# NoelShin/PixelPick

Hardware: AMD Instinct MI355X
Metric: train_step_throughput (higher is better)
Workload: dtype f32; 1 GPU; BASELINE configs[1]: Cityscapes 256x512, C=19, DeepLabv3+-MobileNetV2; train step per-GPU batch 4 with 20 labelled px/img + Adam; acquisition entropy top-k=20, B=256 images/launch/GPU, NCHW fp32 logits; global_batch=4

## Files before the change

### include/pixelpick_hip.h

```cpp
#ifndef PIXELPICK_HIP_H
#define PIXELPICK_HIP_H

#include <stddef.h>
#include <stdint.h>

#ifdef __cplusplus
extern "C" {
#endif

typedef void* pp_stream_t;

enum {
    PP_OK = 0,
    PP_ERR_BAD_ARG = -1,
    PP_ERR_BAD_K = -2,
    PP_ERR_WORKSPACE = -3,
    PP_ERR_UNSUPPORTED = -4,
    PP_ERR_LAUNCH = -5
};

enum { PP_ACQ_ENTROPY = 0, PP_ACQ_LEAST_CONFIDENCE = 1, PP_ACQ_MARGIN = 2 };
#define PP_ACQ_REFERENCE_ORDER 0x100

#define PP_ACQ_MAX_CLASSES 64
// ... 154 lines not shown

int64_t pp_conv2d_fwd_stats_rows(int B, int H, int W, int Cin, int Cout, int kh, int kw, int stride, int pad, int dil);
int pp_conv2d_fwd_stats(const float* x, int64_t ldx, int B, int H, int W, int Cin, const float* w, const float* bias,
                        int kh, int kw, int stride, int pad, int dil, float* y, int64_t ldy, int Cout, void* workspace,
                        size_t ws_bytes, float* stats, size_t stats_floats, pp_stream_t stream);
int pp_bn_train_fwd_partials(const float* x, int64_t ldx, int64_t M, int C, const float* stats, int64_t stat_rows, const float* gamma,
                             const float* beta, float eps, float momentum, float* running_mean, float* running_var, float* mean,
                             float* invstd, const float* residual, int64_t ldr, int act, float drop_p, uint64_t drop_seed,
                             const uint64_t* drop_seed_dev, float* y, int64_t ldy, pp_stream_t stream);

int pp_dwconv3x3_bn_train_fwd_fused(const float* in, int64_t ld_in, int B, int H, int W, int C, const float* w, int stride, int pad,
                                    int dil, float* x_out, int64_t ldx, const float* gamma, const float* beta, float eps,
                                    float momentum, float* running_mean, float* running_var, float* mean, float* invstd,
                                    const float* residual, int64_t ldr, int act, float* y, int64_t ldy, void* workspace,
                                    size_t ws_bytes, int32_t* sync, size_t sync_ints, pp_stream_t stream);

int pp_bn_bwd_fused(const float* x, int64_t ldx, const float* dy, int64_t lddy, const float* y_act, int64_t ldya, int act,
                    int64_t M, int C, const float* mean, const float* invstd, const float* gamma, float* dgamma,
                    float* dbeta, float* dx, int64_t lddx, float* dres, int64_t lddr, float grad_scale, const float* beta,
                    void* workspace, size_t ws_bytes, int32_t* sync, size_t sync_ints, pp_stream_t stream);

int pp_row_flags(const float* dy, int64_t lddy, int64_t M, int C, unsigned char* flags, pp_stream_t stream);
size_t pp_conv1x1_bwd_weight_sparse_workspace_bytes(int64_t M, int Cin, int Cout);
int pp_conv1x1_bwd_weight_sparse(const float* x, int64_t ldx, int64_t M, int Cin, const float* dy, int64_t lddy, int Cout,
                                 const unsigned char* row_flags, float* dw, float* dbias, void* workspace, size_t ws_bytes, pp_stream_t stream);
int pp_conv1x1_bwd_data_sparse(const float* dy, int64_t lddy, int64_t M, int Cout, const float* w, int Cin, const unsigned char* row_flags,
                             float* dx, int64_t lddx, pp_stream_t stream);
int pp_bn_bwd_fused_sparse(const float* x, int64_t ldx, const float* dy, int64_t lddy, const float* y_act, int64_t ldya, int act,
                         int64_t M, int C, const float* mean, const float* invstd, const float* gamma, float* dgamma,
                         float* dbeta, float* dx, int64_t lddx, float* dres, int64_t lddr, float grad_scale, const float* beta,
                         void* workspace, size_t ws_bytes, int32_t* sync, size_t sync_ints, const unsigned char* row_flags,
                         pp_stream_t stream);

int pp_bn_eval_affine(int C, const float* gamma, const float* beta, const float* running_mean, const float* running_var,
                      float eps, float* scale, float* shift, pp_stream_t stream);

int pp_scale_shift_act(const float* x, int64_t ldx, int64_t M, int C, const float* scale, const float* shift,
                       const float* residual, int64_t ldr, int act, float* y, int64_t ldy, pp_stream_t stream);

int pp_bn_bwd(const float* x, int64_t ldx, const float* dy, int64_t lddy, const float* y_act, int64_t ldya, int act,
              int64_t M, int C, const float* mean, const float* invstd, const float* gamma, float* dgamma, float* dbeta,
              float* dx, int64_t lddx, float* dres, int64_t lddr, void* workspace, size_t ws_bytes, pp_stream_t stream);

int pp_dwconv3x3_fwd(const float* x, int64_t ldx, int B, int H, int W, int C, const float* w, int stride, int pad, int dil,
                     float* y, int64_t ldy, pp_stream_t stream);

int pp_dwconv3x3_fwd_bn_act(const float* x, int64_t ldx, int B, int H, int W, int C, const float* w, int stride, int pad,
                            int dil, const float* gamma, const float* beta, const float* running_mean,
                            const float* running_var, float eps, const float* residual, int64_t ldr, int act, float* y,
                            int64_t ldy, pp_stream_t stream);
int pp_dwconv3x3_bwd_data(const float* dy, int64_t lddy, int B, int H, int W, int C, const float* w, int stride, int pad,
                          int dil, float* dx, int64_t lddx, pp_stream_t stream);
int pp_dwconv3x3_bwd_weight(const float* x, int64_t ldx, int B, int H, int W, int C, const float* dy, int64_t lddy,
                            int stride, int pad, int dil, float* dw, void* workspace, size_t ws_bytes, pp_stream_t stream);

size_t pp_groupnorm_workspace_bytes(int B, int64_t P, int C);
int pp_groupnorm_relu_fwd(const float* x, int64_t ldx, int B, int64_t P, int C, int G, const float* gamma, const float* beta,
                          float eps, int relu, float* y, int64_t ldy, float* mean, float* rstd, void* workspace,
                          size_t ws_bytes, pp_stream_t stream);
int pp_groupnorm_relu_bwd(const float* x, int64_t ldx, const float* dy, int64_t lddy, const float* y, int64_t ldy, int B,
                          int64_t P, int C, int G, const float* mean, const float* rstd, const float* gamma, float* dgamma,
                          float* dbeta, float* dx, int64_t lddx, void* workspace, size_t ws_bytes, pp_stream_t stream);

int pp_maxpool2d_fwd(const float* x, int64_t ldx, int B, int H, int W, int C, int ksize, int stride, int pad, float* y,
                     int64_t ldy, unsigned char* argmax, pp_stream_t stream);
int pp_maxpool2d_bwd(const float* dy, int64_t lddy, const unsigned char* argmax, int B, int H, int W, int C, int ksize, int stride,
// ... 90 lines not shown
```

### pixelpick_amd/_lib.py

```python
import ctypes
import os
import struct

import torch

_HERE = os.path.dirname(os.path.abspath(__file__))
LIB_PATH = os.path.join(_HERE, "libpixelpick_hip.so")
KNOBS_LIB_PATH = os.path.join(_HERE, "libpixelpick_hip_knobs.so")
_use_knobs = [os.environ.get("PIXELPICK_KNOBS_BUILD", "0") not in ("", "0")]


def use_knobs_build(on: bool = True):
    if _lib is not None and _use_knobs[0] != bool(on):
        raise PixelPickHipError("use_knobs_build() after the library was loaded")
    _use_knobs[0] = bool(on)


def knobs_build() -> bool:
    return _use_knobs[0]

_i64, _p, _int, _sz, _f = ctypes.c_int64, ctypes.c_void_p, ctypes.c_int, ctypes.c_size_t, ctypes.c_float
_u64 = ctypes.c_uint64

SIGNATURES = {
# ... 33 lines not shown
                                      _p, _i64, _int, _p, _i64, _int, _p, _sz, _p, _sz, _p]),
    "pp_conv2d_bwd_data_bn_bwd_ok": (_int, [_int] * 10),
    "pp_conv2d_bwd_data_bn_bwd_xchg_bytes": (_sz, [_int] * 10),
    "pp_conv2d_bwd_data_bn_bwd": (_int, [_p, _i64, _int, _int, _int, _int, _p, _int, _int, _int, _int, _int, _int, _int, _int, _p, _i64, _p, _p, _p, _p,
                                         _int, _p, _p, _p, _i64, _p, _i64, _p, _i64, _p, _sz, _p, _sz, _p]),
    "pp_x3_planes_bytes": (_sz, [_i64, _int]),
    "pp_x3_split": (_int, [_p, _i64, _i64, _int, _p, _sz, _p]),
    "pp_conv2d_x3_planes_bytes": (_sz, [_int] * 11),
    "pp_conv2d_fwd_pre": (_int, [_p, _i64, _int, _int, _int, _int, _p, _p, _int, _int, _int, _int, _int, _p, _i64, _int, _p, _sz, _p, _p]),
    "pp_conv2d_bwd_data_multi_workspace_bytes": (_sz, [_int] * 14),
    "pp_conv2d_bwd_data_multi": (_int, [_p, _i64, _int, _int, _int, _int, _int, _p, _int, _int, _p, _int, _int, _p, _int, _int, _p, _int, _int,
                                       _p, _i64, _int, _int, _p, _sz, _p]),
    "pp_conv2d_bwd_data_pre": (_int, [_p, _i64, _int, _int, _int, _int, _p, _int, _int, _int, _int, _int, _p, _i64, _int, _int, _int, _int, _p, _sz, _p, _p]),
    "pp_x3_weight_planes_bytes": (_sz, [_int, _int, _int, _int]),
    "pp_x3_split_weights": (_int, [_p, _int, _int, _int, _int, _p, _sz, _p]),
    "pp_conv2d_fwd_pre2": (_int, [_p, _i64, _int, _int, _int, _int, _p, _p, _int, _int, _int, _int, _int, _p, _i64, _int, _p, _sz, _p, _p, _p]),
    "pp_conv2d_bwd_data_pre2": (_int, [_p, _i64, _int, _int, _int, _int, _p, _int, _int, _int, _int, _int, _p, _i64, _int, _int, _int, _int, _p, _sz, _p, _p, _p]),
    "pp_conv2d_bwd_weight_pre": (_int, [_p, _i64, _int, _int, _int, _int, _p, _i64, _int, _int, _int, _int, _int, _int, _p, _p, _p, _sz, _p, _p, _p]),
    "pp_conv2d_bwd_weight_partials": (_int, [_p, _i64, _int, _int, _int, _int, _p, _i64, _int, _int, _int, _int, _int, _int, _p, _p, _p, _sz, _p, _p]),
    "pp_wgrad_reduce_batch": (_int, [_p, _int, _p]),
    "pp_colreduce_workspace_bytes": (_sz, [_i64, _int]),
    "pp_bn_train_fwd": (_int, [_p, _i64, _i64, _int, _p, _p, _f, _f, _p, _p, _p, _p, _p, _p, _p, _sz, _p]),
    "pp_bn_eval_affine": (_int, [_int, _p, _p, _p, _p, _f, _p, _p, _p]),
    "pp_scale_shift_act": (_int, [_p, _i64, _i64, _int, _p, _p, _p, _i64, _int, _p, _i64, _p]),
    "pp_bn_bwd": (_int, [_p, _i64, _p, _i64, _p, _i64, _int, _i64, _int, _p, _p, _p, _p, _p, _p, _i64, _p, _i64, _p, _sz, _p]),
    "pp_bn_fused_workspace_bytes": (_sz, [_i64, _int]),
    "pp_bn_fused_sync_ints": (_sz, [_int]),
    "pp_bn_fused_rows_cached": (_int, [_i64, _int]),
    "pp_bn_train_fwd_fused": (_int, [_p, _i64, _i64, _int, _p, _p, _f, _f, _p, _p, _p, _p, _p, _i64, _int, _f, _u64, _p, _p, _i64, _p, _sz, _p, _sz, _p]),
    "pp_dwconv3x3_bn_train_fwd_fused": (_int, [_p, _i64, _int, _int, _int, _int, _p, _int, _int, _int, _p, _i64, _p, _p, _f, _f, _p, _p, _p, _p,
                                               _p, _i64, _int, _p, _i64, _p, _sz, _p, _sz, _p]),
    "pp_bn_bwd_fused": (_int, [_p, _i64, _p, _i64, _p, _i64, _int, _i64, _int, _p, _p, _p, _p, _p, _p, _i64, _p, _i64, _f, _p, _p, _sz, _p, _sz, _p]),
    "pp_bn_bwd_fused_sparse": (_int, [_p, _i64, _p, _i64, _p, _i64, _int, _i64, _int, _p, _p, _p, _p, _p, _p, _i64, _p, _i64, _f, _p, _p, _sz, _p, _sz, _p, _p]),
    "pp_row_flags": (_int, [_p, _i64, _i64, _int, _p, _p]),
    "pp_conv1x1_bwd_weight_sparse_workspace_bytes": (_sz, [_i64, _int, _int]),
    "pp_conv1x1_bwd_weight_sparse": (_int, [_p, _i64, _i64, _int, _p, _i64, _int, _p, _p, _p, _p, _sz, _p]),
    "pp_conv1x1_bwd_data_sparse": (_int, [_p, _i64, _i64, _int, _p, _int, _p, _p, _i64, _p]),
    "pp_dwconv3x3_fwd": (_int, [_p, _i64, _int, _int, _int, _int, _p, _int, _int, _int, _p, _i64, _p]),
    "pp_dwconv3x3_bwd_data": (_int, [_p, _i64, _int, _int, _int, _int, _p, _int, _int, _int, _p, _i64, _p]),
    "pp_dwconv3x3_bwd_weight": (_int, [_p, _i64, _int, _int, _int, _int, _p, _i64, _int, _int, _int, _p, _p, _sz, _p]),
    "pp_dwconv3x3_bwd_weight_partials": (_int, [_p, _i64, _int, _int, _int, _int, _p, _i64, _int, _int, _int, _p, _p, _sz, _p, _p]),
    "pp_groupnorm_workspace_bytes": (_sz, [_int, _i64, _int]),
    "pp_groupnorm_relu_fwd": (_int, [_p, _i64, _int, _i64, _int, _int, _p, _p, _f, _int, _p, _i64, _p, _p, _p, _sz, _p]),
    "pp_groupnorm_relu_bwd": (_int, [_p, _i64, _p, _i64, _p, _i64, _int, _i64, _int, _int, _p, _p, _p, _p, _p, _p, _i64, _p, _sz, _p]),
    "pp_maxpool2d_fwd": (_int, [_p, _i64, _int, _int, _int, _int, _int, _int, _int, _p, _i64, _p, _p]),
    "pp_maxpool2d_bwd": (_int, [_p, _i64, _p, _int, _int, _int, _int, _int, _int, _int, _p, _i64, _p]),
    "pp_pad2d": (_int, [_p, _i64, _int, _int, _int, _int, _int, _int, _int, _int, _p, _i64, _p]),
    "pp_crop2d_add": (_int, [_p, _i64, _int, _int, _int, _int, _int, _int, _p, _i64, _p, _i64, _int, _int, _p]),
    "pp_bilinear_fwd": (_int, [_p, _i64, _int, _int, _int, _int, _p, _i64, _int, _int, _int, _f, _f, _int, _p]),
    "pp_bilinear_bwd_workspace_bytes": (_sz, [_int] * 4),
    "pp_bilinear_bwd": (_int, [_p, _i64, _int, _int, _int, _int, _p, _i64, _int, _int, _int, _f, _f, _int, _p, _sz, _p]),
    "pp_image_colsum": (_int, [_p, _i64, _int, _i64, _int, _f, _p, _i64, _p]),
    "pp_image_broadcast": (_int, [_p, _i64, _int, _i64, _int, _f, _p, _i64, _p]),
    "pp_dropout": (_int, [_p, _i64, _p, _i64, _i64, _int, _f, ctypes.c_uint64, _p, _p]),
    "pp_dropout2d": (_int, [_p, _i64, _p, _i64, _int, _i64, _int, _f, ctypes.c_uint64, _p, _p]),
    "pp_aug_resample_h": (_int, [_p, _int, _int, _p, _p, _int, _int, _p, _p]),
    "pp_aug_vcrop": (_int, [_p, _p, _p] + [_int] * 11 + [_p, _p]),
    "pp_aug_labels": (_int, [_p, _p, _int, _p, _p, _p, _p] + [_int] * 8 + [_p, _p, _p]),
    "pp_aug_jitter": (_int, [_p, _i64, _int, _f, _p, _p]),
    "pp_aug_blur": (_int, [_p, _int, _int, _p, _int, _p, _p]),
    "pp_aug_blur_q8": (_int, [_p, _int, _int, _p, _int, _p, _p]),
    "pp_aug_to_tensor": (_int, [_p, _i64, ctypes.POINTER(_f), ctypes.POINTER(_f), _p, _p]),
    "pp_sparse_ce_workspace_bytes": (_sz, []),
    "pp_sparse_ce_fwd_bwd": (_int, [_p, _int, _int, _i64, _i64, _i64, _p, _int, _p, _p, _p, _p, _p, _sz, _p]),
    "pp_sparse_ce_lowres_workspace_bytes": (_sz, []),
    "pp_sparse_ce_lowres_fwd_bwd": (_int, [_p, _i64] + [_int] * 7 + [_p, _int, _p, _p, _p, _p, _i64, _p, _sz, _p]),
# ... 347 lines not shown
```

### pixelpick_amd/csrc/conv_igemm.hip

```cpp
#include <atomic>
#include <type_traits>

#include "pp_common.h"
#include "bn_xchg.h"
#include "conv_types.h"

namespace pp {


static int g_conv_xcd_remap = 1;
static int g_conv_novec = 0;
static int g_conv_lds_pad = 0;
static int g_conv_variant = 0;

typedef float f32x16s __attribute__((ext_vector_type(16)));
constexpr int BK = 16;
struct __attribute__((packed, aligned(4))) StemF4 { float x, y, z, w; };
struct __attribute__((packed, aligned(4))) StemF3 { float x, y, z; };
struct __attribute__((packed, aligned(4))) StemF2 { float x, y; };


template <int TM, int TN, bool A_MK, bool B_NK, int PITCH_A, int PITCH_B, int BKT = BK>
__device__ __forceinline__ void mma_step(const float* As, const float* Bs, int a_row0, int b_col0, f32x16 (&acc)[TM][TN])
{
    const int lane = threadIdx.x & 63;
    const int l31 = lane & 31, h = lane >> 5;
    constexpr int NQ = BKT / 8;
    float a[NQ][TM][4], b[NQ][TN][4];
#pragma unroll
    for (int q = 0; q < NQ; ++q) {
        const int k0 = 8 * q + 4 * h;
#pragma unroll
        for (int tm = 0; tm < TM; ++tm) {
            const int r = a_row0 + tm * 32 + l31;
            if constexpr (A_MK) {
                const float4 v = *reinterpret_cast<const float4*>(As + r * PITCH_A + k0);
                a[q][tm][0] = v.x; a[q][tm][1] = v.y; a[q][tm][2] = v.z; a[q][tm][3] = v.w;
            } else {
// ... 2413 lines not shown
        for (; m + 28 < r1; m += 32) {
            float v[8];
#pragma unroll
            for (int u = 0; u < 8; ++u) v[u] = dy[(m + 4 * u) * ld + c];
#pragma unroll
            for (int u = 0; u < 8; ++u) q[u] += v[u];
        }
        for (; m < r1; m += 4) q[0] += dy[m * ld + c];
        s = ((q[0] + q[1]) + (q[2] + q[3])) + ((q[4] + q[5]) + (q[6] + q[7]));
    }
    sh[ry][threadIdx.x & 63] = s;
    __syncthreads();
    if (ry == 0 && c < C)
        part[(int64_t)blockIdx.y * C + c] = (sh[0][threadIdx.x] + sh[1][threadIdx.x]) + (sh[2][threadIdx.x] + sh[3][threadIdx.x]);
}

__global__ __launch_bounds__(256) void bias_grad_final_kernel(const float* part, int nblk, int C, float* dbias)
{
    __shared__ double sh[256];
    const int t = threadIdx.x, lane = t >> 3;
    const int c = blockIdx.x * 8 + (t & 7);
    double s = 0.0;
    if (c < C)
        for (int b = lane; b < nblk; b += 32) s += (double)part[(int64_t)b * C + c];
    sh[t] = s;
    __syncthreads();
    for (int off = 128; off >= 8; off >>= 1) {
        if (t < off) sh[t] += sh[t + off];
        __syncthreads();
    }
    if (t < 8 && c < C) dbias[c] = (float)sh[t];
}

__device__ __forceinline__ uint16_t f32_to_bf16_rne(float f)
{
    uint32_t u = __float_as_uint(f);
    if ((u & 0x7F800000u) == 0x7F800000u) return (uint16_t)(u >> 16);
    u += 0x7FFFu + ((u >> 16) & 1u);
    return (uint16_t)(u >> 16);
}
__device__ __forceinline__ float bf16_to_f32(uint16_t h) { return __uint_as_float((uint32_t)h << 16); }

__device__ __forceinline__ void x3_split1(float v, uint16_t& hi, uint16_t& mid, uint16_t& lo)
{
    hi = f32_to_bf16_rne(v);
    const float r1 = v - bf16_to_f32(hi);
    mid = f32_to_bf16_rne(r1);
    const float r2 = r1 - bf16_to_f32(mid);
    lo = f32_to_bf16_rne(r2);
}

__global__ __launch_bounds__(256) void x3_split_kernel(const float* x, int64_t ldx, int64_t rows, int C, uint16_t* out, int Kp, int64_t plane)
{
    const int nchunk = Kp / 16;
    const int64_t per_chunk = (rows + 1) * 2;
    const int64_t total = per_chunk * nchunk;
    for (int64_t e = (int64_t)blockIdx.x * 256 + threadIdx.x; e < total; e += (int64_t)gridDim.x * 256) {
        const int ch = (int)(e / per_chunk);
        const int64_t rem = e - (int64_t)ch * per_chunk;
        const int64_t r = rem >> 1;
        const int c0 = ch * 16 + (int)(rem & 1) * 8;
        uint16_t h[8], m[8], l[8];
#pragma unroll
        for (int j = 0; j < 8; ++j) { h[j] = m[j] = l[j] = 0; }
        if (r < rows) {
            if (c0 + 8 <= C && (ldx & 3) == 0) {
                const float4 v0 = *reinterpret_cast<const float4*>(x + r * ldx + c0), v1 = *reinterpret_cast<const float4*>(x + r * ldx + c0 + 4);
                const float v[8] = {v0.x, v0.y, v0.z, v0.w, v1.x, v1.y, v1.z, v1.w};
#pragma unroll
                for (int j = 0; j < 8; ++j) x3_split1(v[j], h[j], m[j], l[j]);
            } else {
#pragma unroll
                for (int j = 0; j < 8; ++j)
                    if (c0 + j < C) x3_split1(x[r * ldx + c0 + j], h[j], m[j], l[j]);
            }
        }
        uint4 ph, pm, pl;
        ph.x = h[0] | ((uint32_t)h[1] << 16); ph.y = h[2] | ((uint32_t)h[3] << 16); ph.z = h[4] | ((uint32_t)h[5] << 16); ph.w = h[6] | ((uint32_t)h[7] << 16);
        pm.x = m[0] | ((uint32_t)m[1] << 16); pm.y = m[2] | ((uint32_t)m[3] << 16); pm.z = m[4] | ((uint32_t)m[5] << 16); pm.w = m[6] | ((uint32_t)m[7] << 16);
        pl.x = l[0] | ((uint32_t)l[1] << 16); pl.y = l[2] | ((uint32_t)l[3] << 16); pl.z = l[4] | ((uint32_t)l[5] << 16); pl.w = l[6] | ((uint32_t)l[7] << 16);
        const int64_t o = e * 8;
        *reinterpret_cast<uint4*>(out + o) = ph;
        *reinterpret_cast<uint4*>(out + plane + o) = pm;
        *reinterpret_cast<uint4*>(out + 2 * plane + o) = pl;
    }
}

__global__ __launch_bounds__(256) void x3_split_w_kernel(const float* w, int taps, int Cin, int Cout, int transpose, uint16_t* out, int Kp,
                                                        int64_t plane)
{
    const int n_rows = transpose ? Cout : Cin, K = transpose ? Cin : Cout;
    const int nchunk = Kp / 16;
    const int64_t rows = (int64_t)taps * n_rows;
    const int64_t per_chunk = (rows + 1) * 2;
    const int64_t total = per_chunk * nchunk;
    for (int64_t e = (int64_t)blockIdx.x * 256 + threadIdx.x; e < total; e += (int64_t)gridDim.x * 256) {
        const int64_t ch2 = e / (rows + 1);
        const int64_t r = e - ch2 * (rows + 1);
        const int ch = (int)(ch2 >> 1);
        const int k0 = ch * 16 + (int)(ch2 & 1) * 8;
        uint16_t h[8], m[8], l[8];
#pragma unroll
        for (int j = 0; j < 8; ++j) {
            h[j] = m[j] = l[j] = 0;
            if (r < rows && k0 + j < K) {
                const int t = (int)(r / n_rows), n = (int)(r - (int64_t)t * n_rows);
                const float v = transpose ? w[((int64_t)t * Cin + (k0 + j)) * Cout + n] : w[((int64_t)t * Cin + n) * Cout + k0 + j];
                x3_split1(v, h[j], m[j], l[j]);
            }
        }
        const int64_t o = ((int64_t)ch * per_chunk + r * 2 + (ch2 & 1)) * 8;
        uint4 ph, pm, pl;
        ph.x = h[0] | ((uint32_t)h[1] << 16); ph.y = h[2] | ((uint32_t)h[3] << 16); ph.z = h[4] | ((uint32_t)h[5] << 16); ph.w = h[6] | ((uint32_t)h[7] << 16);
        pm.x = m[0] | ((uint32_t)m[1] << 16); pm.y = m[2] | ((uint32_t)m[3] << 16); pm.z = m[4] | ((uint32_t)m[5] << 16); pm.w = m[6] | ((uint32_t)m[7] << 16);
// ... 3 lines not shown
        *reinterpret_cast<uint4*>(out + 2 * plane + o) = pl;
    }
}

__device__ __forceinline__ void x3_glds16(uint32_t voff, const void* sbase_in, uint32_t lds_dst_in)
{
    const uint32_t lds_dst = __builtin_amdgcn_readfirstlane(lds_dst_in);
    const uint64_t sb = reinterpret_cast<uint64_t>(sbase_in);
    const uint64_t sbu = ((uint64_t)(uint32_t)__builtin_amdgcn_readfirstlane((uint32_t)(sb >> 32)) << 32) |
                         (uint32_t)__builtin_amdgcn_readfirstlane((uint32_t)sb);
    const void* sbase = reinterpret_cast<const void*>(sbu);
    unsigned keep;
    asm volatile("s_mov_b32 %0, m0\n\ts_mov_b32 m0, %3\n\ts_nop 0\n\tglobal_load_lds_dwordx4 %1, %2\n\ts_mov_b32 m0, %0"
                 : "=&s"(keep) : "v"(voff), "s"(sbase), "s"(lds_dst) : "memory");
}

__device__ __forceinline__ void x3_glds16x3(uint32_t voff, const void* s0, const void* s1, const void* s2, uint32_t lds_dst_in, uint32_t stride_in)
{
    const uint32_t d0 = __builtin_amdgcn_readfirstlane(lds_dst_in);
    const uint32_t st = __builtin_amdgcn_readfirstlane(stride_in);
    auto uni = [](const void* q) -> const void* {
        const uint64_t v = reinterpret_cast<uint64_t>(q);
        return reinterpret_cast<const void*>(((uint64_t)(uint32_t)__builtin_amdgcn_readfirstlane((uint32_t)(v >> 32)) << 32) |
                                             (uint32_t)__builtin_amdgcn_readfirstlane((uint32_t)v));
    };
    const void* b0 = uni(s0); const void* b1 = uni(s1); const void* b2 = uni(s2);
    unsigned keep, t;
    asm volatile("s_mov_b32 %0, m0\n\ts_mov_b32 m0, %6\n\ts_nop 0\n\tglobal_load_lds_dwordx4 %2, %3\n\t"
                 "s_add_u32 %1, %6, %7\n\ts_mov_b32 m0, %1\n\ts_nop 0\n\tglobal_load_lds_dwordx4 %2, %4\n\t"
                 "s_add_u32 %1, %1, %7\n\ts_mov_b32 m0, %1\n\ts_nop 0\n\tglobal_load_lds_dwordx4 %2, %5\n\ts_mov_b32 m0, %0"
                 : "=&s"(keep), "=&s"(t) : "v"(voff), "s"(b0), "s"(b1), "s"(b2), "s"(d0), "s"(st) : "memory", "scc");
}

template <int BM, int BN, int VAR = 0>
__global__ __launch_bounds__(BM * 2, (BM == 128 ? 2 : 2)) void conv_x3_kernel(ConvParams p, X3Operands o)
{
    constexpr int TM = 2, TN = BN / 64, WN = 2, NWAVE = BM / 32;
    constexpr int NSTAGE = VAR == 1 ? 3 : VAR == 2 ? 2 : (BM == 256 && BN == 128) ? 4 : (BM == 256 ? 5 : 3);
    constexpr bool PROD = VAR == 0 && BM == 256 && BN == 128;
    constexpr bool PAIR = PROD || VAR == 8 || VAR == 9;
    constexpr bool LATE_BEGIN = PROD || VAR == 9 || VAR == 10;
    constexpr int PRE = PAIR ? NSTAGE - 1 : NSTAGE;
    constexpr int A_BYTES = BM * 32, B_BYTES = BN * 32;
    constexpr int STAGE_BYTES = 3 * (A_BYTES + B_BYTES);
    constexpr int NBW = BN / 32;
    static_assert(NBW <= NWAVE, "B rows are loaded by the first BN/32 waves");
    __shared__ __attribute__((aligned(1024))) unsigned char smem[NSTAGE * STAGE_BYTES];
    struct Frags { bf16x8_t a[3][TM], b[3][TN]; };

    const int tid = threadIdx.x, lane = tid & 63, l31 = lane & 31, h = lane >> 5;
    const int wave = __builtin_amdgcn_readfirstlane(tid >> 6);
    const int wm = wave / WN, wn = wave % WN;
    int mt, nt;
    {
        const int ntn = p.n_tiles, nblk = gridDim.x, bid = blockIdx.x, per_xcd = nblk / 8;
        if (p.xcd_remap && per_xcd * 8 == nblk) {
            const int lin = (bid & 7) * per_xcd + (bid >> 3);
            mt = lin / ntn; nt = lin - mt * ntn;
        } else {
            mt = bid / ntn; nt = bid - mt * ntn;
        }
    }
    const int64_t m0 = (int64_t)mt * BM;
    const int n0 = o.col_base + nt * BN;
    const uint32_t lds0 = __builtin_amdgcn_readfirstlane((uint32_t)(uintptr_t)smem);

    const int lr = lane >> 1;
    const int lhalf = (lane & 1) ^ ((lr >> 3) & 1);
    uint32_t a_e0 = 0;
    unsigned a_vm = 0u;
    {
        const int64_t m = m0 + wave * 32 + lr;
        if (m < p.M) {
            const unsigned mu = (unsigned)m;
            const unsigned t = mu / (unsigned)p.Wo;
            const int ow = (int)(mu - t * (unsigned)p.Wo);
            const unsigned bb = t / (unsigned)p.Ho;
            const int oh = (int)(t - bb * (unsigned)p.Ho);
            const int ih0 = oh * p.stride, iw0 = ow * p.stride;
// ... 561 lines not shown
        const double t = (double)cdiv(tiles, cus) * tile_us;
        if (t < best_t) { best_t = t; best = f; }
    }
    return best;
}

template <bool BWD>
static int launch_conv_x3(ConvParams& p, const ConvPlan& pl, const X3Plan& x, int kh_kw, void* workspace, hipStream_t st, bool f32path)
{
    const uint16_t* ap = p.a_pre ? p.a_pre : reinterpret_cast<uint16_t*>(workspace);
    uint16_t* bp = reinterpret_cast<uint16_t*>(reinterpret_cast<char*>(workspace) + x.b_off);
    if (!p.a_pre && !f32path) {
        const int64_t ta = (x.rows_a + 1) * (x.Kp / 8);
        hipLaunchKernelGGL(x3_split_kernel, dim3((unsigned)std::min<int64_t>(cdiv(ta, 256), 4096)), dim3(256), 0, st, p.x, p.ldx, x.rows_a, p.Ck,
                           reinterpret_cast<uint16_t*>(workspace), x.Kp, x.a_plane);
        if (int rc = check_launch("x3_split_kernel")) return rc;
    }
    if (p.b_pre) {
        bp = const_cast<uint16_t*>(p.b_pre);
    } else {
        const int64_t tb = (x.b_rows + 1) * (x.Kp / 8);
        hipLaunchKernelGGL(x3_split_w_kernel, dim3((unsigned)std::min<int64_t>(cdiv(tb, 256), 4096)), dim3(256), 0, st, p.w, kh_kw, p.Cin, p.Cout,
                           BWD ? 0 : 1, bp, x.Kp, x.b_plane);
        if (int rc = check_launch("x3_split_w_kernel")) return rc;
    }
    X3Operands o{ap, bp, x.a_plane, x.b_plane, x.Kp, p.Cn, (uint32_t)(x.rows_a * 32), (uint32_t)(x.b_rows * 32),
                 (uint32_t)((x.rows_a + 1) * 32), (uint32_t)((x.b_rows + 1) * 32), 0};
    p.n_tiles = pl.n_tiles;
    p.splits = 1;
    p.ks_per_split = 0;
    p.part = nullptr;
    const int full128 = p.Cn / 128, rem = p.Cn - full128 * 128;
    const bool two = rem > 0 && rem <= 64 && full128 > 0 && !(g_conv_x3 & 4);
    bool n128_only = !two && (rem == 0 || rem > 64 || (g_conv_x3 & 4));
    const int64_t mt256 = cdiv(p.M, 256);
    if (f32path && n128_only && rem == 0 && cdiv(p.M, 128) * full128 < 200 && cdiv(p.M, 128) * full128 * 2 >= 128) n128_only = false;
    auto go = [&](bool n128, int ntile, int col_base) {
        const bool m256 = !(g_conv_x3 & 2) && mt256 * ntile >= 200;
        const int64_t mtiles = m256 ? mt256 : cdiv(p.M, 128);
        o.col_base = col_base;
        p.n_tiles = ntile;
        const dim3 grid((unsigned)(mtiles * ntile));
#ifdef PP_DEBUG_KNOBS
        if (f32path) {
            (void)launch_conv_x3f(p, o, m256, n128, grid.x, st);
            return;
        }
#endif
        if (m256) {
            if (n128) {
                switch (g_x3_var) {
#ifdef PP_DEBUG_KNOBS
                    case 1: hipLaunchKernelGGL((conv_x3_kernel<256, 128, 1>), grid, dim3(512), 0, st, p, o); break;
                    case 2: hipLaunchKernelGGL((conv_x3_kernel<256, 128, 2>), grid, dim3(512), 0, st, p, o); break;
                    case 3: hipLaunchKernelGGL((conv_x3_kernel<256, 128, 3>), grid, dim3(512), 0, st, p, o); break;
                    case 4: hipLaunchKernelGGL((conv_x3_kernel<256, 128, 4>), grid, dim3(512), 0, st, p, o); break;
                    case 5: hipLaunchKernelGGL((conv_x3_kernel<256, 128, 5>), grid, dim3(512), 0, st, p, o); break;
                    case 6: hipLaunchKernelGGL((conv_x3_kernel<256, 128, 6>), grid, dim3(512), 0, st, p, o); break;
                    case 7: hipLaunchKernelGGL((conv_x3_kernel<256, 128, 7>), grid, dim3(512), 0, st, p, o); break;
                    case 8: hipLaunchKernelGGL((conv_x3_kernel<256, 128, 8>), grid, dim3(512), 0, st, p, o); break;
                    case 9: hipLaunchKernelGGL((conv_x3_kernel<256, 128, 9>), grid, dim3(512), 0, st, p, o); break;
                    case 10: hipLaunchKernelGGL((conv_x3_kernel<256, 128, 10>), grid, dim3(512), 0, st, p, o); break;
                    case 11: hipLaunchKernelGGL((conv_x3_kernel<256, 128, 11>), grid, dim3(512), 0, st, p, o); break;
#endif
                    default: hipLaunchKernelGGL((conv_x3_kernel<256, 128>), grid, dim3(512), 0, st, p, o);
                }
// ... 1467 lines not shown
```

### pixelpick_amd/csrc/nn_ops.hip

```cpp
#include "pp_common.h"
#include "bn_xchg.h"

namespace pp {

constexpr int kT = 256;

__device__ __forceinline__ float act_fwd(float z, int act)
{
    if (act == 1) return fmaxf(z, 0.0f);
    if (act == 2) return fminf(fmaxf(z, 0.0f), 6.0f);
    return z;
}
__device__ __forceinline__ void decode_bhwq(int64_t e, int cq, int Wd, int Hd, int& q, int& w, int& h, int& b)
{
    if (e <= 0xFFFFFFFFll) {
        const unsigned u = (unsigned)e;
        const unsigned t = u / (unsigned)cq;
        q = (int)(u - t * (unsigned)cq);
        const unsigned t2 = t / (unsigned)Wd;
        w = (int)(t - t2 * (unsigned)Wd);
        const unsigned t3 = t2 / (unsigned)Hd;
        h = (int)(t2 - t3 * (unsigned)Hd);
        b = (int)t3;
    } else {
        q = (int)(e % cq);
        int64_t t = e / cq;
        w = (int)(t % Wd); t /= Wd;
        h = (int)(t % Hd);
        b = (int)(t / Hd);
    }
}

struct ColReduceGeom {
    int cq;
// ... 294 lines not shown
    sh[1][t] = s1;
    __syncthreads();
    for (int off = 128; off >= 1; off >>= 1) {
        if (rl < off && rl + off < nrl) {
            const float4 a = sh[0][t + off * bq], b = sh[1][t + off * bq];
            s0.x += a.x; s0.y += a.y; s0.z += a.z; s0.w += a.w;
            s1.x += b.x; s1.y += b.y; s1.z += b.z; s1.w += b.w;
            sh[0][t] = s0;
            sh[1][t] = s1;
        }
        __syncthreads();
    }
}

__device__ __forceinline__ void drop4(float4& o, uint64_t i0, uint64_t seed, float p, float inv_keep)
{
    o.x = (float)(hash_rng(seed, i0 + 0) >> 8) * (1.0f / 16777216.0f) >= p ? o.x * inv_keep : 0.0f;
    o.y = (float)(hash_rng(seed, i0 + 1) >> 8) * (1.0f / 16777216.0f) >= p ? o.y * inv_keep : 0.0f;
    o.z = (float)(hash_rng(seed, i0 + 2) >> 8) * (1.0f / 16777216.0f) >= p ? o.z * inv_keep : 0.0f;
    o.w = (float)(hash_rng(seed, i0 + 3) >> 8) * (1.0f / 16777216.0f) >= p ? o.w * inv_keep : 0.0f;
}

struct BnFwdArgs {
    const float* x; int64_t ldx; int64_t M; int C;
    const float* gamma; const float* beta; float eps; float momentum;
    float* running_mean; float* running_var; float* mean; float* invstd;
    const float* res; int64_t ldr; int act; float* y; int64_t ldy;
    xword* part; int* sync; BnFusedGeom g;
    float drop_p, drop_inv_keep; uint64_t drop_seed; const uint64_t* drop_seed_dev;
    const float* dw_in; int64_t dw_ld; const float* dw_w; float* x_out;
    int dw_H, dw_W, dw_Ho, dw_Wo, dw_stride, dw_pad, dw_dil;
    const float* stats; int stat_rows;
    unsigned long long* probe;
};
#define BN_STAMP(i) do { if (a.probe && threadIdx.x == 0) a.probe[(int64_t)blockIdx.x * 8 + (i)] = wall_clock64(); } while (0)

__device__ __forceinline__ float4 dw_point(const BnFwdArgs& a, int64_t row, int q, const float4* wreg)
{
    const unsigned ru = (unsigned)row;
    const unsigned t = ru / (unsigned)a.dw_Wo;
    const int ow = (int)(ru - t * (unsigned)a.dw_Wo);
    const unsigned b = t / (unsigned)a.dw_Ho;
    const int oh = (int)(t - b * (unsigned)a.dw_Ho);
    float4 acc = make_float4(0.f, 0.f, 0.f, 0.f);
#pragma unroll
    for (int th = 0; th < 3; ++th) {
        const int ih = oh * a.dw_stride - a.dw_pad + th * a.dw_dil;
        if ((unsigned)ih >= (unsigned)a.dw_H) continue;
#pragma unroll
        for (int tw = 0; tw < 3; ++tw) {
            const int iw = ow * a.dw_stride - a.dw_pad + tw * a.dw_dil;
            if ((unsigned)iw >= (unsigned)a.dw_W) continue;
            const float4 v = *reinterpret_cast<const float4*>(a.dw_in + (((int64_t)b * a.dw_H + ih) * a.dw_W + iw) * a.dw_ld + q * 4);
            const float4 ww = wreg[th * 3 + tw];
            acc.x = fmaf(v.x, ww.x, acc.x); acc.y = fmaf(v.y, ww.y, acc.y);
            acc.z = fmaf(v.z, ww.z, acc.z); acc.w = fmaf(v.w, ww.w, acc.w);
        }
    }
    return acc;
}

template <int MODE, int NC = 0>
__global__ __launch_bounds__(kT) void bn_fused_fwd_kernel(BnFwdArgs a)
{
    constexpr bool DW = MODE == 1;
    static_assert(NC == 0 || (MODE != 2 && NC % 4 == 0), "row cache: the kernels with a statistics pass");
    float4 keep[NC > 0 ? NC : 1];
    __shared__ unsigned sh_tag;
    __shared__ float4 sh[2][kT];
    __shared__ double shd[kT];
    __shared__ double tot[64];
    __shared__ float aff[2][32];
    const BnFusedGeom g = a.g;
    unsigned tag = 0, tag0 = 0;
    BN_STAMP(0);
    if constexpr (MODE != 2) tag0 = tag_issue(a.sync);
    const int t = threadIdx.x;
    const int strip = blockIdx.x % g.nstrips, chunk = blockIdx.x / g.nstrips;
    const int ql = t % g.bq, rl = t / g.bq;
    const int q = strip * g.bq + ql;
    const bool active = rl < g.nrl && q < g.cq;
    const int64_t r0 = (int64_t)chunk * g.rows_per_chunk;
    const int64_t r1 = r0 + g.rows_per_chunk < a.M ? r0 + g.rows_per_chunk : a.M;
    const float* xq = a.x + q * 4;
    const int nch = g.bq * 4, nout = nch * 2;
    if constexpr (MODE == 2) {
        const int nsub = kT / nout;
        const int o = t % nout, sub = t / nout;
        const int stat = o / nch, cl = o - stat * nch;
        const int c = strip * nch + cl;
        double s = 0.0;
        if (sub < nsub && c < a.C) {
            const float* p = a.stats + (int64_t)stat * a.C + c;
            int r = sub;
            for (; r + 3 * nsub < a.stat_rows; r += 4 * nsub) {
                const float v0 = p[(int64_t)r * 2 * a.C], v1 = p[(int64_t)(r + nsub) * 2 * a.C];
                const float v2 = p[(int64_t)(r + 2 * nsub) * 2 * a.C], v3 = p[(int64_t)(r + 3 * nsub) * 2 * a.C];
                s += ((double)v0 + (double)v1) + ((double)v2 + (double)v3);
            }
            for (; r < a.stat_rows; r += nsub) s += (double)p[(int64_t)r * 2 * a.C];
        }
        shd[t] = s;
        __syncthreads();
        if (t < nout) {
            double acc = shd[t];
            for (int k = 1; k < nsub; ++k) acc += shd[k * nout + t];
            tot[t] = acc;
        }
        __syncthreads();
    } else {
// ... 85 lines not shown
                a.invstd[c] = is;
                if (a.running_mean) {
                    const double unbiased = count > 1.0 ? var * count / (count - 1.0) : var;
                    a.running_mean[c] = (1.0f - a.momentum) * a.running_mean[c] + a.momentum * (float)mu;
                    a.running_var[c] = (1.0f - a.momentum) * a.running_var[c] + a.momentum * (float)unbiased;
                }
            }
        }
    }
    __syncthreads();
    if (!active) return;
    const float4 sc = *reinterpret_cast<const float4*>(&aff[0][ql * 4]);
    const float4 sf = *reinterpret_cast<const float4*>(&aff[1][ql * 4]);
    float* yq = a.y + q * 4;
    const float* rq = a.res ? a.res + q * 4 : nullptr;
    const int act = a.act;
    const bool drop = a.drop_p > 0.0f;
    uint64_t dseed = a.drop_seed;
    if (drop && a.drop_seed_dev) dseed += *a.drop_seed_dev * 0x9E3779B97F4A7C15ull;
    if constexpr (NC > 0) {
#pragma unroll
        for (int e = 0; e < NC; ++e) {
            const int64_t r = r0 + rl + (int64_t)e * g.nrl;
            if (r >= r1) break;
            const float4 va = keep[e];
            float4 oa;
            oa.x = fmaf(va.x, sc.x, sf.x); oa.y = fmaf(va.y, sc.y, sf.y); oa.z = fmaf(va.z, sc.z, sf.z); oa.w = fmaf(va.w, sc.w, sf.w);
            if (rq) {
                const float4 ra = *reinterpret_cast<const float4*>(rq + r * a.ldr);
                oa.x += ra.x; oa.y += ra.y; oa.z += ra.z; oa.w += ra.w;
            }
            oa.x = act_fwd(oa.x, act); oa.y = act_fwd(oa.y, act); oa.z = act_fwd(oa.z, act); oa.w = act_fwd(oa.w, act);
            if (drop) drop4(oa, (uint64_t)(r * g.cq + q) * 4, dseed, a.drop_p, a.drop_inv_keep);
            *reinterpret_cast<float4*>(yq + r * a.ldy) = oa;
        }
        BN_STAMP(5);
        return;
    }
    for (int64_t r = r0 + rl; r < r1; r += (int64_t)g.nrl * 4) {
        float4 v[4], rv[4];
#pragma unroll
        for (int j = 0; j < 4; ++j) {
            const int64_t rr = r + (int64_t)j * g.nrl;
            const int64_t rc = rr < r1 ? rr : r;
            v[j] = *reinterpret_cast<const float4*>(xq + rc * a.ldx);
            rv[j] = rq ? *reinterpret_cast<const float4*>(rq + rc * a.ldr) : make_float4(0.f, 0.f, 0.f, 0.f);
        }
#pragma unroll
        for (int j = 0; j < 4; ++j) {
            const int64_t rr = r + (int64_t)j * g.nrl;
            if (rr >= r1) break;
            float4 o;
            o.x = fmaf(v[j].x, sc.x, sf.x); o.y = fmaf(v[j].y, sc.y, sf.y); o.z = fmaf(v[j].z, sc.z, sf.z); o.w = fmaf(v[j].w, sc.w, sf.w);
            if (rq) { o.x += rv[j].x; o.y += rv[j].y; o.z += rv[j].z; o.w += rv[j].w; }
            o.x = act_fwd(o.x, act); o.y = act_fwd(o.y, act); o.z = act_fwd(o.z, act); o.w = act_fwd(o.w, act);
            if (drop) drop4(o, (uint64_t)(rr * g.cq + q) * 4, dseed, a.drop_p, a.drop_inv_keep);
            *reinterpret_cast<float4*>(yq + rr * a.ldy) = o;
        }
    }
    BN_STAMP(5);
}

struct BnBwdArgs {
    const float* x; int64_t ldx; const float* dy; int64_t lddy; const float* yact; int64_t ldya; int act;
    int64_t M; int C; const float* mean; const float* invstd; const float* gamma; float* dgamma; float* dbeta;
    float* dx; int64_t lddx; float* dres; int64_t lddr; xword* part; int* sync; BnFusedGeom g;
    float gscale;
    const float* beta_mask;
    const unsigned char* rowflag;
};

__device__ __attribute__((aligned(16))) float g_bn_zero4[4] = {0.f, 0.f, 0.f, 0.f};
template <int NC, bool SPARSE = false>
__global__ __launch_bounds__(kT) void bn_fused_bwd_kernel(BnBwdArgs a)
{
    static_assert(!SPARSE || NC == 0, "row flags: the uncached variant");
    __shared__ unsigned sh_tag;
    __shared__ float4 sh[2][kT];
    __shared__ double shd[kT];
    __shared__ double tot[64];
    __shared__ float red[2][32];
    static_assert(NC % 2 == 0, "row cache: pairs of rows");
    float4 keepx[NC > 0 ? NC : 1], keepu[NC > 0 ? NC : 1];
    const BnFusedGeom g = a.g;
    const unsigned tag0 = tag_issue(a.sync);
    const int t = threadIdx.x;
    const int strip = blockIdx.x % g.nstrips, chunk = blockIdx.x / g.nstrips;
    const int ql = t % g.bq, rl = t / g.bq;
    const int q = strip * g.bq + ql;
    const bool active = rl < g.nrl && q < g.cq;
    const int64_t r0 = (int64_t)chunk * g.rows_per_chunk;
    const int64_t r1 = r0 + g.rows_per_chunk < a.M ? r0 + g.rows_per_chunk : a.M;
    const float* xq = a.x + q * 4;
    const float* gq = a.dy + q * 4;
    const float* aq = a.yact ? a.yact + q * 4 : nullptr;
    const bool remask = aq == nullptr && a.beta_mask != nullptr && a.act != 0;
    const int act = (aq || remask) ? a.act : 0;
    float4 s0 = make_float4(0.f, 0.f, 0.f, 0.f), s1 = s0, mu = s0, is = s0, zsc = s0, zsf = s0;
    if (active) {
        mu = *reinterpret_cast<const float4*>(a.mean + q * 4);
        is = *reinterpret_cast<const float4*>(a.invstd + q * 4);
        if (remask) {
            const float4 gm = *reinterpret_cast<const float4*>(a.gamma + q * 4), be = *reinterpret_cast<const float4*>(a.beta_mask + q * 4);
            zsc = make_float4(gm.x * is.x, gm.y * is.y, gm.z * is.z, gm.w * is.w);
            zsf = make_float4(be.x - mu.x * zsc.x, be.y - mu.y * zsc.y, be.z - mu.z * zsc.z, be.w - mu.w * zsc.w);
        }
        auto red_load = [&](int64_t r, float4* v, float4* gg, float4* ya, float* w) {
#pragma unroll
            for (int j = 0; j < 2; ++j) {
                const int64_t rr = r + (int64_t)j * g.nrl;
                w[j] = rr < r1 ? 1.0f : 0.0f;
                const int64_t rc = rr < r1 ? rr : r1 - 1;
                v[j] = *reinterpret_cast<const float4*>(xq + rc * a.ldx);
                gg[j] = *reinterpret_cast<const float4*>(gq + rc * a.lddy);
                ya[j] = (act != 0 && !remask) ? *reinterpret_cast<const float4*>(aq + rc * a.ldya) : make_float4(0.f, 0.f, 0.f, 0.f);
            }
        };
        auto red_acc = [&](const float4* v, const float4* gg, float4* ya, const float* w, float4* vk, float4* uk) {
#pragma unroll
// ... 76 lines not shown
    }
    strip_combine(a.part, strip, g.R, nout, tag, shd, tot);
    launch_done(a.sync);
    if (t < nch) {
        const int c = strip * nch + t;
        const float db = (float)tot[t], dg = (float)tot[nch + t];
        red[0][t] = db;
        red[1][t] = dg;
        if (c < a.C && chunk == 0) {
            a.dbeta[c] = db;
            a.dgamma[c] = dg;
        }
    }
    __syncthreads();
    if (!active) return;
    const float inv_count = 1.0f / (float)a.M;
    const float4 db = *reinterpret_cast<const float4*>(&red[0][ql * 4]);
    const float4 dg = *reinterpret_cast<const float4*>(&red[1][ql * 4]);
    const float4 ga = *reinterpret_cast<const float4*>(a.gamma + q * 4);
    float* dxq = a.dx + q * 4;
    float* drq = a.dres ? a.dres + q * 4 : nullptr;
    if constexpr (NC > 0) {
#pragma unroll
        for (int e = 0; e < NC; ++e) {
            const int64_t r = r0 + rl + (int64_t)e * g.nrl;
            if (r >= r1) break;
            const float4 u = keepu[e], v = keepx[e];
            if (drq) *reinterpret_cast<float4*>(drq + r * a.lddr) = u;
            float4 o;
            o.x = bn_dx(u.x, v.x, mu.x, is.x, ga.x, db.x, dg.x, inv_count);
            o.y = bn_dx(u.y, v.y, mu.y, is.y, ga.y, db.y, dg.y, inv_count);
            o.z = bn_dx(u.z, v.z, mu.z, is.z, ga.z, db.z, dg.z, inv_count);
            o.w = bn_dx(u.w, v.w, mu.w, is.w, ga.w, db.w, dg.w, inv_count);
            *reinterpret_cast<float4*>(dxq + r * a.lddx) = o;
        }
        return;
    }
    constexpr int RW = SPARSE ? 8 : 4;
    unsigned char fnext[RW] = {};
    if constexpr (SPARSE) {
#pragma unroll
        for (int j = 0; j < RW; ++j) {
            const int64_t rr = r0 + rl + (int64_t)j * g.nrl;
            fnext[j] = rr < r1 ? a.rowflag[rr] : (unsigned char)0;
        }
    }
    for (int64_t r = r0 + rl; r < r1; r += (int64_t)g.nrl * RW) {
        float4 uu[RW], vv[RW], yy[RW];
        unsigned char fcur[RW];
#pragma unroll
        for (int j = 0; j < RW; ++j) fcur[j] = fnext[j];
#pragma unroll
        for (int j = 0; j < RW; ++j) {
            const int64_t rr = r + (int64_t)j * g.nrl;
            const int64_t rc = rr < r1 ? rr : r;
            if constexpr (SPARSE) {
                const bool fl = rr < r1 && fcur[j] != 0;
                {
                    const int64_t rn = rr + (int64_t)g.nrl * RW;
                    fnext[j] = rn < r1 ? a.rowflag[rn] : (unsigned char)0;
                }
                uu[j] = *reinterpret_cast<const float4*>(fl ? gq + rc * a.lddy : g_bn_zero4);
                yy[j] = (act != 0 && !remask) ? *reinterpret_cast<const float4*>(fl ? aq + rc * a.ldya : g_bn_zero4) : make_float4(0.f, 0.f, 0.f, 0.f);
            } else {
                uu[j] = *reinterpret_cast<const float4*>(gq + rc * a.lddy);
                yy[j] = (act != 0 && !remask) ? *reinterpret_cast<const float4*>(aq + rc * a.ldya) : make_float4(0.f, 0.f, 0.f, 0.f);
            }
            vv[j] = *reinterpret_cast<const float4*>(xq + rc * a.ldx);
        }
#pragma unroll
        for (int j = 0; j < RW; ++j) {
            const int64_t rr = r + (int64_t)j * g.nrl;
            if (rr >= r1) break;
            float4 u = uu[j];
            const float4 v = vv[j];
            if (act != 0) {
                const float4 ya = remask ? make_float4(fmaf(v.x, zsc.x, zsf.x), fmaf(v.y, zsc.y, zsf.y), fmaf(v.z, zsc.z, zsf.z),
                                                       fmaf(v.w, zsc.w, zsf.w))
                                         : yy[j];
                u.x *= act_mask(ya.x, act); u.y *= act_mask(ya.y, act); u.z *= act_mask(ya.z, act); u.w *= act_mask(ya.w, act);
            }
            u.x *= a.gscale; u.y *= a.gscale; u.z *= a.gscale; u.w *= a.gscale;
            if (drq) *reinterpret_cast<float4*>(drq + rr * a.lddr) = u;
            float4 o;
            o.x = bn_dx(u.x, v.x, mu.x, is.x, ga.x, db.x, dg.x, inv_count);
            o.y = bn_dx(u.y, v.y, mu.y, is.y, ga.y, db.y, dg.y, inv_count);
            o.z = bn_dx(u.z, v.z, mu.z, is.z, ga.z, db.z, dg.z, inv_count);
            o.w = bn_dx(u.w, v.w, mu.w, is.w, ga.w, db.w, dg.w, inv_count);
            *reinterpret_cast<float4*>(dxq + rr * a.lddx) = o;
        }
    }
}

static int bn_fused_capacity()
{
    static const int cap = [] {
        int dev = 0, cus = 0, a = 0, b = 0, c = 0;
        if (hipGetDevice(&dev) != hipSuccess) { (void)hipGetLastError(); return 0; }
        if (hipDeviceGetAttribute(&cus, hipDeviceAttributeMultiprocessorCount, dev) != hipSuccess) { (void)hipGetLastError(); return 0; }
        int d = 0, e = 0, f = 0, sp = 0;
        if (hipOccupancyMaxActiveBlocksPerMultiprocessor(&a, bn_fused_fwd_kernel<0, 0>, kT, 0) != hipSuccess ||
            hipOccupancyMaxActiveBlocksPerMultiprocessor(&b, bn_fused_fwd_kernel<1, 0>, kT, 0) != hipSuccess ||
            hipOccupancyMaxActiveBlocksPerMultiprocessor(&c, bn_fused_bwd_kernel<0>, kT, 0) != hipSuccess ||
            hipOccupancyMaxActiveBlocksPerMultiprocessor(&sp, (bn_fused_bwd_kernel<0, true>), kT, 0) != hipSuccess ||
            hipOccupancyMaxActiveBlocksPerMultiprocessor(&d, bn_fused_fwd_kernel<0, kBnRowCache>, kT, 0) != hipSuccess ||
            hipOccupancyMaxActiveBlocksPerMultiprocessor(&e, bn_fused_bwd_kernel<kBnRowCache>, kT, 0) != hipSuccess ||
            hipOccupancyMaxActiveBlocksPerMultiprocessor(&f, bn_fused_fwd_kernel<1, kBnRowCache>, kT, 0) != hipSuccess) {
            (void)hipGetLastError();
            return 0;
        }
        int per = a < b ? a : b;
        per = per < c ? per : c;
        per = per < d ? per : d;
        per = per < e ? per : e;
        per = per < f ? per : f;
        per = per < sp ? per : sp;
        return per * cus;
    }();
    return reserve_scaled(cap, bn_device_cus());
}

__global__ __launch_bounds__(kT) void dwconv_fwd_kernel(const float* x, int64_t ldx, int B, int H, int W, int cq,
                                                       const float* w, int stride, int pad, int dil, float* y,
                                                       int64_t ldy, int Ho, int Wo, Epilogue epi)
{
    const int C = cq * 4;
    const int64_t total = (int64_t)B * Ho * Wo * cq;
    for (int64_t e = (int64_t)blockIdx.x * kT + threadIdx.x; e < total; e += (int64_t)gridDim.x * kT) {
        int q, ow, oh, b;
        decode_bhwq(e, cq, Wo, Ho, q, ow, oh, b);
        float4 acc = make_float4(0.f, 0.f, 0.f, 0.f);
        float4 v[9];
#pragma unroll
        for (int th = 0; th < 3; ++th) {
            const int ih = oh * stride - pad + th * dil;
            const bool rok = (unsigned)ih < (unsigned)H;
#pragma unroll
            for (int tw = 0; tw < 3; ++tw) {
                const int iw = ow * stride - pad + tw * dil;
                const bool ok = rok && (unsigned)iw < (unsigned)W;
                const float4 t = *reinterpret_cast<const float4*>(x + (((int64_t)b * H + (ok ? ih : 0)) * W + (ok ? iw : 0)) * ldx + q * 4);
                v[th * 3 + tw] = ok ? t : make_float4(0.f, 0.f, 0.f, 0.f);
            }
        }
#pragma unroll
        for (int t = 0; t < 9; ++t) {
            const float4 ww = *reinterpret_cast<const float4*>(w + t * C + q * 4);
            acc.x = fmaf(v[t].x, ww.x, acc.x); acc.y = fmaf(v[t].y, ww.y, acc.y);
            acc.z = fmaf(v[t].z, ww.z, acc.z); acc.w = fmaf(v[t].w, ww.w, acc.w);
// ... 441 lines not shown
        int64_t t = e / cq;
        const int pw = (int)(t % Wp); t /= Wp;
        const int ph = (int)(t % Hp);
        const int b = (int)(t / Hp);
        const int ih = ph - pt, iw = pw - pl;
        float4 v = make_float4(0.f, 0.f, 0.f, 0.f);
        if ((unsigned)ih < (unsigned)H && (unsigned)iw < (unsigned)W)
            v = *reinterpret_cast<const float4*>(x + (((int64_t)b * H + ih) * W + iw) * ldx + q * 4);
        *reinterpret_cast<float4*>(y + (((int64_t)b * Hp + ph) * Wp + pw) * ldy + q * 4) = v;
    }
}

__global__ __launch_bounds__(kT) void crop_kernel(const float* xp, int64_t ldxp, int B, int Hp, int Wp, int cq, int pt, int pl,
                                                 const float* add, int64_t ldadd, float* y, int64_t ldy, int H, int W)
{
    const int64_t total = (int64_t)B * H * W * cq;
    for (int64_t e = (int64_t)blockIdx.x * kT + threadIdx.x; e < total; e += (int64_t)gridDim.x * kT) {
        const int q = (int)(e % cq);
        int64_t t = e / cq;
        const int iw = (int)(t % W); t /= W;
        const int ih = (int)(t % H);
        const int b = (int)(t / H);
        float4 v = *reinterpret_cast<const float4*>(xp + (((int64_t)b * Hp + ih + pt) * Wp + iw + pl) * ldxp + q * 4);
        const int64_t r = ((int64_t)b * H + ih) * W + iw;
        if (add) {
            const float4 a = *reinterpret_cast<const float4*>(add + r * ldadd + q * 4);
            v.x += a.x; v.y += a.y; v.z += a.z; v.w += a.w;
        }
        *reinterpret_cast<float4*>(y + r * ldy + q * 4) = v;
    }
}


template <bool OUT_NCHW>
__global__ __launch_bounds__(kT) void bilinear_fwd_kernel(const float* x, int64_t ldx, int B, int H, int W, int C,
                                                         float* y, int64_t ldy, int Ho, int Wo, float sh, float sw,
                                                         int align)
{
    if constexpr (!OUT_NCHW) {
        const int cq = C / 4;
        const int64_t total = (int64_t)B * Ho * Wo * cq;
        for (int64_t e = (int64_t)blockIdx.x * kT + threadIdx.x; e < total; e += (int64_t)gridDim.x * kT) {
            int q, ow, oh, b;
            if (total < (1ll << 31)) {
                const unsigned eu = (unsigned)e, t1 = eu / (unsigned)cq, t2 = t1 / (unsigned)Wo;
                q = (int)(eu - t1 * (unsigned)cq);
                ow = (int)(t1 - t2 * (unsigned)Wo);
                b = (int)(t2 / (unsigned)Ho);
                oh = (int)(t2 - (unsigned)b * (unsigned)Ho);
            } else {
                q = (int)(e % cq);
                int64_t t = e / cq;
                ow = (int)(t % Wo); t /= Wo;
                oh = (int)(t % Ho);
                b = (int)(t / Ho);
            }
            const Lerp lh = lerp_src(oh, H, sh, align), lw = lerp_src(ow, W, sw, align);
            const float* base = x + (int64_t)b * H * W * ldx + q * 4;
            const float4 v00 = *reinterpret_cast<const float4*>(base + ((int64_t)lh.i0 * W + lw.i0) * ldx);
            const float4 v01 = *reinterpret_cast<const float4*>(base + ((int64_t)lh.i0 * W + lw.i1) * ldx);
            const float4 v10 = *reinterpret_cast<const float4*>(base + ((int64_t)lh.i1 * W + lw.i0) * ldx);
            const float4 v11 = *reinterpret_cast<const float4*>(base + ((int64_t)lh.i1 * W + lw.i1) * ldx);
            float4 o;
            o.x = bilerp(lh.l0, lh.l1, lw.l0, lw.l1, v00.x, v01.x, v10.x, v11.x);
            o.y = bilerp(lh.l0, lh.l1, lw.l0, lw.l1, v00.y, v01.y, v10.y, v11.y);
            o.z = bilerp(lh.l0, lh.l1, lw.l0, lw.l1, v00.z, v01.z, v10.z, v11.z);
            o.w = bilerp(lh.l0, lh.l1, lw.l0, lw.l1, v00.w, v01.w, v10.w, v11.w);
            *reinterpret_cast<float4*>(y + (((int64_t)b * Ho + oh) * Wo + ow) * ldy + q * 4) = o;
        }
    } else {
        const int64_t total = (int64_t)B * C * Ho * Wo;
        for (int64_t e = (int64_t)blockIdx.x * kT + threadIdx.x; e < total; e += (int64_t)gridDim.x * kT) {
            const int ow = (int)(e % Wo);
            int64_t t = e / Wo;
            const int oh = (int)(t % Ho); t /= Ho;
            const int c = (int)(t % C);
            const int b = (int)(t / C);
            const Lerp lh = lerp_src(oh, H, sh, align), lw = lerp_src(ow, W, sw, align);
            const float* base = x + (int64_t)b * H * W * ldx + c;
            const float v00 = base[((int64_t)lh.i0 * W + lw.i0) * ldx], v01 = base[((int64_t)lh.i0 * W + lw.i1) * ldx];
            const float v10 = base[((int64_t)lh.i1 * W + lw.i0) * ldx], v11 = base[((int64_t)lh.i1 * W + lw.i1) * ldx];
            y[e] = bilerp(lh.l0, lh.l1, lw.l0, lw.l1, v00, v01, v10, v11);
        }
    }
}

__device__ __forceinline__ void out_window(int i, int in, int out, float scale, int align, int& lo, int& hi)
{
    float inv = scale > 0.0f ? 1.0f / scale : 0.0f;
    float a = ((float)i - 1.0f) * inv, b = ((float)i + 1.0f) * inv;
    if (!align) { a -= 0.5f; b += 0.5f; }
    lo = (int)floorf(a) - 1;
    hi = (int)ceilf(b) + 1;
    if (lo < 0) lo = 0;
    if (hi > out - 1) hi = out - 1;
    if (scale == 0.0f) { lo = 0; hi = out - 1; }
}

constexpr int kMaxWin = 24;
__global__ __launch_bounds__(kT) void bilinear_bwd4_kernel(const float* dy, int64_t lddy, int B, int Ho, int Wo, int cq,
                                                          float* dx, int64_t lddx, int H, int W, float sh, float sw, int align)
// ... 588 lines not shown

__global__ __launch_bounds__(kT) void nhwc_to_nchw_kernel(const float* x, int64_t ldx, int B, int C, int64_t HW, float* y)
{
    const int64_t total = (int64_t)B * C * HW;
    for (int64_t e = (int64_t)blockIdx.x * kT + threadIdx.x; e < total; e += (int64_t)gridDim.x * kT) {
        const int64_t pix = e % HW;
        const int64_t t = e / HW;
        const int c = (int)(t % C);
        const int64_t b = t / C;
        y[e] = x[(b * HW + pix) * ldx + c];
    }
}

static int g_bil_sep = 1;
static int g_dw_wgrad_x4 = 1, g_dw_wgrad_x4_blocks = 256;
static int g_dw_wgrad_cq_blk = 0, g_dw_wgrad_passes = 0;
static int g_dw_x4 = 1;
static int g_dw_s2 = 1;

static inline unsigned grid_for(int64_t total)
{
    int64_t b = cdiv(total, kT);
    if (b > 8192) b = 8192;
    if (b < 1) b = 1;
    return (unsigned)b;
}

static int need_c4(int C, const char* what)
{
    if (C < 4 || C % 4 != 0) return fail(PP_ERR_UNSUPPORTED, "%s: C=%d must be a positive multiple of 4", what, C);
    return PP_OK;
}

}

using namespace pp;

extern "C" {

#ifdef PP_DEBUG_KNOBS
void pp_debug_set_dw_variant(int v)
{
    g_dw_x4 = (v & 1) ? 0 : 1;
    g_dw_s2 = (v & 1048576) ? 0 : 1;
    g_bil_sep = (v & 256) ? 0 : 1;
    g_dw_wgrad_x4 = (v & 512) ? 0 : 1;
    { const int s4 = (v >> 10) & 7; g_dw_wgrad_x4_blocks = s4 == 1 ? 128 : s4 == 2 ? 512 : s4 == 3 ? 1024 : s4 == 4 ? 64 : 256; }
    { const int cb = (v >> 13) & 7; g_dw_wgrad_cq_blk = cb == 1 ? 8 : cb == 2 ? 16 : cb == 3 ? 32 : cb == 4 ? 64 : cb == 5 ? 128 : cb == 6 ? kT : 0; }
    { const int mp = (v >> 16) & 3; g_dw_wgrad_passes = mp == 1 ? 1 : mp == 2 ? 2 : mp == 3 ? 4 : 0; }
    const int sel = (v >> 1) & 7;
    g_dw_wgrad_blocks = sel == 1 ? 512 : sel == 2 ? 256 : sel == 3 ? 128 : sel == 4 ? 2048 : 1024;
}
#endif
#ifdef PP_DEBUG_KNOBS
void pp_debug_set_bn_target(int blocks) { g_bn_target_blocks = blocks > 0 ? (blocks > 1024 ? 1024 : blocks) : 0; }
#endif
#ifdef PP_DEBUG_KNOBS
void pp_debug_set_bn_bytes_per_block(int bytes)
{
    g_bn_bytes_per_block = bytes > 0 ? bytes : 0;
    g_bn_row_cache = bytes == -1 ? 0 : 1;
}
#endif
static thread_local unsigned long long* g_bn_probe = nullptr;
#ifdef PP_DEBUG_KNOBS
void pp_debug_set_bn_probe(void* device_buffer) { g_bn_probe = reinterpret_cast<unsigned long long*>(device_buffer); }
// ... 26 lines not shown
    if (int rc = check_launch("col_reduce_kernel<0>")) return rc;
    hipLaunchKernelGGL(bn_finalize_kernel, dim3((unsigned)cdiv(C, 8)), dim3(kT), 0, st, part, g.nblk_rows, C, (double)M,
                       gamma, beta, eps, momentum, running_mean, running_var, mean, invstd, scale, shift);
    return check_launch("bn_finalize_kernel");
}

size_t pp_bn_fused_workspace_bytes(int64_t M, int C)
{
    if (M < 1 || C < 4) return 256;
    BnFusedGeom g = bn_fused_geom(M, C);
    return align_up((size_t)g.nstrips * g.R * g.bq * 8 * 8, 256);
}

int pp_bn_fused_rows_cached(int64_t M, int C)
{
    if (M < 1 || C < 4 || C % 4) return 0;
    BnFusedGeom g = bn_fused_geom(M, C);
    return (g_bn_row_cache && g.rows_per_chunk <= (int64_t)g.nrl * kBnRowCache) ? 1 : 0;
}

size_t pp_bn_fused_sync_ints(int C) { (void)C; return 64; }

static int bn_fused_check(const char* what, int64_t M, int C, const BnFusedGeom& g, const void* workspace, size_t ws_bytes,
                          const int32_t* sync, size_t sync_ints)
{
    if (M < 1) return fail(PP_ERR_BAD_ARG, "%s: M < 1", what);
    if (!workspace || ws_bytes < (size_t)g.nstrips * g.R * g.bq * 8 * 8) return fail(PP_ERR_WORKSPACE, "%s: workspace", what);
    if ((reinterpret_cast<uintptr_t>(workspace) & 7) != 0) return fail(PP_ERR_BAD_ARG, "%s: workspace must be 8-byte aligned", what);
    if (!sync || sync_ints < 2) return fail(PP_ERR_WORKSPACE, "%s: sync array needs 2 ints", what);
    (void)C;
    return PP_OK;
}

int pp_bn_train_fwd_fused(const float* x, int64_t ldx, int64_t M, int C, const float* gamma, const float* beta, float eps,
                          float momentum, float* running_mean, float* running_var, float* mean, float* invstd,
                          const float* residual, int64_t ldr, int act, float drop_p, uint64_t drop_seed,
                          const uint64_t* drop_seed_dev, float* y, int64_t ldy, void* workspace,
                          size_t ws_bytes, int32_t* sync, size_t sync_ints, pp_stream_t stream)
{
    if (drop_p < 0.0f || drop_p >= 1.0f) return fail(PP_ERR_BAD_ARG, "bn_train_fwd_fused: dropout p=%f outside [0,1)", (double)drop_p);
    if (drop_p > 0.0f && act == 2) return fail(PP_ERR_UNSUPPORTED, "bn_train_fwd_fused: dropout after ReLU6 is not fusable");
    if (!x || !gamma || !beta || !mean || !invstd || !y) return fail(PP_ERR_BAD_ARG, "bn_train_fwd_fused: null");
    if (int rc = need_c4(C, "bn_train_fwd_fused")) return rc;
    if (ldx % 4 || ldy % 4 || (residual && ldr % 4)) return fail(PP_ERR_BAD_ARG, "bn_train_fwd_fused: ld must be multiples of 4");
    BnFusedGeom g = bn_fused_geom(M, C);
    if (int rc = bn_fused_check("bn_train_fwd_fused", M, C, g, workspace, ws_bytes, sync, sync_ints)) return rc;
    BnFwdArgs a{x, ldx, M, C, gamma, beta, eps, momentum, running_mean, running_var, mean, invstd, residual, ldr, act, y, ldy,
                reinterpret_cast<xword*>(workspace), sync, g, drop_p, 1.0f / (1.0f - drop_p), drop_seed, drop_seed_dev,
                nullptr, 0, nullptr, nullptr, 0, 0, 0, 0, 0, 0, 0, nullptr, 0, g_bn_probe};
    if (g_bn_row_cache && g.rows_per_chunk <= (int64_t)g.nrl * kBnRowCache)
        hipLaunchKernelGGL((bn_fused_fwd_kernel<0, kBnRowCache>), dim3((unsigned)(g.nstrips * g.R)), dim3(kT), 0, as_stream(stream), a);
    else
        hipLaunchKernelGGL((bn_fused_fwd_kernel<0, 0>), dim3((unsigned)(g.nstrips * g.R)), dim3(kT), 0, as_stream(stream), a);
    return check_launch("bn_fused_fwd_kernel");
}

int pp_bn_train_fwd_partials(const float* x, int64_t ldx, int64_t M, int C, const float* stats, int64_t stat_rows, const float* gamma,
                             const float* beta, float eps, float momentum, float* running_mean, float* running_var, float* mean,
                             float* invstd, const float* residual, int64_t ldr, int act, float drop_p, uint64_t drop_seed,
                             const uint64_t* drop_seed_dev, float* y, int64_t ldy, pp_stream_t stream)
{
    if (drop_p < 0.0f || drop_p >= 1.0f) return fail(PP_ERR_BAD_ARG, "bn_train_fwd_partials: dropout p=%f outside [0,1)", (double)drop_p);
    if (drop_p > 0.0f && act == 2) return fail(PP_ERR_UNSUPPORTED, "bn_train_fwd_partials: dropout after ReLU6 is not fusable");
    if (!x || !gamma || !beta || !mean || !invstd || !y || !stats) return fail(PP_ERR_BAD_ARG, "bn_train_fwd_partials: null");
    if (M < 1 || stat_rows < 1 || stat_rows > 0x7FFFFFFFll) return fail(PP_ERR_BAD_ARG, "bn_train_fwd_partials: M / stat_rows");
    if (int rc = need_c4(C, "bn_train_fwd_partials")) return rc;
    if (ldx % 4 || ldy % 4 || (residual && ldr % 4)) return fail(PP_ERR_BAD_ARG, "bn_train_fwd_partials: ld must be multiples of 4");
    BnFusedGeom g = bn_fused_geom(M, C);
    BnFwdArgs a{x, ldx, M, C, gamma, beta, eps, momentum, running_mean, running_var, mean, invstd, residual, ldr, act, y, ldy,
                nullptr, nullptr, g, drop_p, 1.0f / (1.0f - drop_p), drop_seed, drop_seed_dev,
                nullptr, 0, nullptr, nullptr, 0, 0, 0, 0, 0, 0, 0, stats, (int)stat_rows};
    hipLaunchKernelGGL((bn_fused_fwd_kernel<2, 0>), dim3((unsigned)(g.nstrips * g.R)), dim3(kT), 0, as_stream(stream), a);
    return check_launch("bn_fused_fwd_kernel<partials>");
}

int pp_dwconv3x3_bn_train_fwd_fused(const float* in, int64_t ld_in, int B, int H, int W, int C, const float* w, int stride, int pad,
                                    int dil, float* x_out, int64_t ldx, const float* gamma, const float* beta, float eps,
                                    float momentum, float* running_mean, float* running_var, float* mean, float* invstd,
                                    const float* residual, int64_t ldr, int act, float* y, int64_t ldy, void* workspace,
                                    size_t ws_bytes, int32_t* sync, size_t sync_ints, pp_stream_t stream)
{
    if (!in || !w || !x_out || !gamma || !beta || !mean || !invstd || !y) return fail(PP_ERR_BAD_ARG, "dwconv_bn_train_fwd_fused: null");
    if (int rc = need_c4(C, "dwconv_bn_train_fwd_fused")) return rc;
    if (ld_in % 4 || ldx % 4 || ldy % 4 || (residual && ldr % 4)) return fail(PP_ERR_BAD_ARG, "dwconv_bn_train_fwd_fused: ld must be multiples of 4");
    if (stride < 1 || dil < 1) return fail(PP_ERR_BAD_ARG, "dwconv_bn_train_fwd_fused: stride / dilation");
    const int Ho = (H + 2 * pad - 2 * dil - 1) / stride + 1, Wo = (W + 2 * pad - 2 * dil - 1) / stride + 1;
    if (Ho < 1 || Wo < 1) return fail(PP_ERR_BAD_ARG, "dwconv_bn_train_fwd_fused: empty output");
    const int64_t M = (int64_t)B * Ho * Wo;
    if (M > 0x7FFFFFFFll) return fail(PP_ERR_UNSUPPORTED, "dwconv_bn_train_fwd_fused: more than 2^31 output pixels");
    BnFusedGeom g = bn_fused_geom(M, C);
    if (int rc = bn_fused_check("dwconv_bn_train_fwd_fused", M, C, g, workspace, ws_bytes, sync, sync_ints)) return rc;
    BnFwdArgs a{x_out, ldx, M, C, gamma, beta, eps, momentum, running_mean, running_var, mean, invstd, residual, ldr, act, y, ldy,
                reinterpret_cast<xword*>(workspace), sync, g, 0.0f, 1.0f, 0ull, nullptr,
                in, ld_in, w, x_out, H, W, Ho, Wo, stride, pad, dil, nullptr, 0};
    if (g_bn_row_cache && g.rows_per_chunk <= (int64_t)g.nrl * kBnRowCache)
        hipLaunchKernelGGL((bn_fused_fwd_kernel<1, kBnRowCache>), dim3((unsigned)(g.nstrips * g.R)), dim3(kT), 0, as_stream(stream), a);
    else
        hipLaunchKernelGGL((bn_fused_fwd_kernel<1, 0>), dim3((unsigned)(g.nstrips * g.R)), dim3(kT), 0, as_stream(stream), a);
    return check_launch("bn_fused_fwd_kernel<dw>");
}

static int bn_bwd_fused_impl(const float* x, int64_t ldx, const float* dy, int64_t lddy, const float* y_act, int64_t ldya, int act,
                             int64_t M, int C, const float* mean, const float* invstd, const float* gamma, float* dgamma,
                             float* dbeta, float* dx, int64_t lddx, float* dres, int64_t lddr, float grad_scale, const float* beta,
                             void* workspace, size_t ws_bytes, int32_t* sync, size_t sync_ints, pp_stream_t stream,
                             const unsigned char* row_flags);

int pp_bn_bwd_fused(const float* x, int64_t ldx, const float* dy, int64_t lddy, const float* y_act, int64_t ldya, int act,
                    int64_t M, int C, const float* mean, const float* invstd, const float* gamma, float* dgamma,
                    float* dbeta, float* dx, int64_t lddx, float* dres, int64_t lddr, float grad_scale, const float* beta,
                    void* workspace, size_t ws_bytes, int32_t* sync, size_t sync_ints, pp_stream_t stream)
{
    return bn_bwd_fused_impl(x, ldx, dy, lddy, y_act, ldya, act, M, C, mean, invstd, gamma, dgamma, dbeta, dx, lddx, dres, lddr, grad_scale,
                             beta, workspace, ws_bytes, sync, sync_ints, stream, nullptr);
}

int pp_bn_bwd_fused_sparse(const float* x, int64_t ldx, const float* dy, int64_t lddy, const float* y_act, int64_t ldya, int act,
                         int64_t M, int C, const float* mean, const float* invstd, const float* gamma, float* dgamma,
                         float* dbeta, float* dx, int64_t lddx, float* dres, int64_t lddr, float grad_scale, const float* beta,
                         void* workspace, size_t ws_bytes, int32_t* sync, size_t sync_ints, const unsigned char* row_flags,
                         pp_stream_t stream)
{
    return bn_bwd_fused_impl(x, ldx, dy, lddy, y_act, ldya, act, M, C, mean, invstd, gamma, dgamma, dbeta, dx, lddx, dres, lddr, grad_scale,
                             beta, workspace, ws_bytes, sync, sync_ints, stream, row_flags);
}

__global__ __launch_bounds__(256) void row_flags_kernel(const float* dy, int64_t ld, int64_t M, int C, unsigned char* flags)
{
    const int64_t r = (int64_t)blockIdx.x * 256 + threadIdx.x;
    if (r >= M) return;
    const float* p = dy + r * ld;
    bool nz = false;
    for (int c = 0; c < C; ++c) nz = nz || (p[c] != 0.0f);
    flags[r] = nz ? 1 : 0;
}

int pp_row_flags(const float* dy, int64_t lddy, int64_t M, int C, unsigned char* flags, pp_stream_t stream)
{
    if (!dy || !flags || M < 1 || C < 1) return fail(PP_ERR_BAD_ARG, "row_flags: bad argument");
    hipLaunchKernelGGL(row_flags_kernel, dim3((unsigned)cdiv(M, 256)), dim3(256), 0, as_stream(stream), dy, lddy, M, C, flags);
    return check_launch("row_flags_kernel");
}

__global__ __launch_bounds__(256) void conv1x1_bwd_data_rows_kernel(const float* dy, int64_t lddy, int64_t M, int Cout, const float* w, int Cin,
                                                                     const unsigned char* flags, float* dx, int64_t lddx)
{
    __shared__ unsigned char fl[16];
    const int t = threadIdx.x;
    const int64_t r0 = (int64_t)blockIdx.x * 16;
    const int cq = Cin / 4;
    if (t < 16) fl[t] = (r0 + t < M) ? flags[r0 + t] : (unsigned char)2;
    __syncthreads();
    for (int e = t; e < 16 * cq; e += 256) {
        const int rr = e / cq, q = e - rr * cq;
        if (fl[rr] == 0) *reinterpret_cast<float4*>(dx + (r0 + rr) * lddx + q * 4) = make_float4(0.f, 0.f, 0.f, 0.f);
    }
    for (int rr = 0; rr < 16; ++rr) {
// ... 87 lines not shown

size_t pp_conv1x1_bwd_weight_sparse_workspace_bytes(int64_t M, int Cin, int Cout)
{
    if (M < 1 || Cin < 1 || Cout < 1 || (int64_t)Cin * Cout + Cout > 256 * kSwAcc) return 0;
    const int64_t G = cdiv(M, kSwRows);
    return align_up((size_t)G * ((size_t)Cin * Cout + Cout) * 4, 256) + align_up((size_t)G * 4, 256);
}

int pp_conv1x1_bwd_weight_sparse(const float* x, int64_t ldx, int64_t M, int Cin, const float* dy, int64_t lddy, int Cout,
                                 const unsigned char* row_flags, float* dw, float* dbias, void* workspace, size_t ws_bytes, pp_stream_t stream)
{
    if (!x || !dy || !row_flags || !dw || M < 1 || Cin < 1 || Cout < 1) return fail(PP_ERR_BAD_ARG, "conv1x1_bwd_weight_sparse: bad argument");
    const size_t need = pp_conv1x1_bwd_weight_sparse_workspace_bytes(M, Cin, Cout);
    if (need == 0) return fail(PP_ERR_UNSUPPORTED, "conv1x1_bwd_weight_sparse: Cin * Cout + Cout = %lld > %d", (long long)Cin * Cout + Cout, 256 * kSwAcc);
    if (!workspace || ws_bytes < need) return fail(PP_ERR_WORKSPACE, "conv1x1_bwd_weight_sparse: workspace %zu B < required %zu B", ws_bytes, need);
    const int64_t G = cdiv(M, kSwRows);
    if (G > 0x7FFFFFFF) return fail(PP_ERR_UNSUPPORTED, "conv1x1_bwd_weight_sparse: too many rows");
    const int cn = Cin * Cout, E = cn + (dbias ? Cout : 0);
    float* part = reinterpret_cast<float*>(workspace);
    int* cnt = reinterpret_cast<int*>(reinterpret_cast<char*>(workspace) + align_up((size_t)G * ((size_t)cn + Cout) * 4, 256));
    hipStream_t st = as_stream(stream);
    hipLaunchKernelGGL(conv1x1_wgrad_rows_partial_kernel, dim3((unsigned)G), dim3(256), 0, st, x, ldx, dy, lddy, M, Cin, Cout, row_flags,
                       dbias ? 1 : 0, part, cnt);
    if (int rc = check_launch("conv1x1_wgrad_rows_partial_kernel")) return rc;
    hipLaunchKernelGGL(conv1x1_wgrad_rows_reduce_kernel, dim3((unsigned)cdiv(E, 256)), dim3(256), 0, st, (const float*)part, (const int*)cnt, (int)G, E, cn,
                       dw, dbias);
    return check_launch("conv1x1_wgrad_rows_reduce_kernel");
}

static int bn_bwd_fused_impl(const float* x, int64_t ldx, const float* dy, int64_t lddy, const float* y_act, int64_t ldya, int act,
                             int64_t M, int C, const float* mean, const float* invstd, const float* gamma, float* dgamma,
                             float* dbeta, float* dx, int64_t lddx, float* dres, int64_t lddr, float grad_scale, const float* beta,
                             void* workspace, size_t ws_bytes, int32_t* sync, size_t sync_ints, pp_stream_t stream,
                             const unsigned char* row_flags)
{
    if (!x || !dy || !mean || !invstd || !gamma || !dgamma || !dbeta || !dx) return fail(PP_ERR_BAD_ARG, "bn_bwd_fused: null");
    if (act != 0 && !y_act && !beta) return fail(PP_ERR_BAD_ARG, "bn_bwd_fused: the mask needs the activation output or beta");
    if (!y_act && act != 0 && (dres || grad_scale != 1.0f))
        return fail(PP_ERR_BAD_ARG, "bn_bwd_fused: the mask can only be recomputed from x without residual / dropout");
    if (int rc = need_c4(C, "bn_bwd_fused")) return rc;
    if (ldx % 4 || lddy % 4 || lddx % 4 || (y_act && ldya % 4) || (dres && lddr % 4))
        return fail(PP_ERR_BAD_ARG, "bn_bwd_fused: ld must be multiples of 4");
    BnFusedGeom g = bn_fused_geom(M, C);
    if (int rc = bn_fused_check("bn_bwd_fused", M, C, g, workspace, ws_bytes, sync, sync_ints)) return rc;
    BnBwdArgs a{x, ldx, dy, lddy, y_act, ldya, act, M, C, mean, invstd, gamma, dgamma, dbeta, dx, lddx, dres, lddr,
                reinterpret_cast<xword*>(workspace), sync, g, grad_scale, y_act ? nullptr : beta, row_flags};
    if (g_bn_row_cache && g.rows_per_chunk <= (int64_t)g.nrl * kBnRowCache)
        hipLaunchKernelGGL(bn_fused_bwd_kernel<kBnRowCache>, dim3((unsigned)(g.nstrips * g.R)), dim3(kT), 0, as_stream(stream), a);
    else if (row_flags)
        hipLaunchKernelGGL((bn_fused_bwd_kernel<0, true>), dim3((unsigned)(g.nstrips * g.R)), dim3(kT), 0, as_stream(stream), a);
    else
        hipLaunchKernelGGL(bn_fused_bwd_kernel<0>, dim3((unsigned)(g.nstrips * g.R)), dim3(kT), 0, as_stream(stream), a);
    return check_launch("bn_fused_bwd_kernel");
}

int pp_bn_eval_affine(int C, const float* gamma, const float* beta, const float* running_mean, const float* running_var,
                      float eps, float* scale, float* shift, pp_stream_t stream)
{
    if (!gamma || !beta || !running_mean || !running_var || !scale || !shift) return fail(PP_ERR_BAD_ARG, "bn_eval_affine: null");
    hipLaunchKernelGGL(bn_eval_affine_kernel, dim3((unsigned)cdiv(C, kT)), dim3(kT), 0, as_stream(stream), C, gamma, beta,
                       running_mean, running_var, eps, scale, shift);
    return check_launch("bn_eval_affine_kernel");
}

int pp_scale_shift_act(const float* x, int64_t ldx, int64_t M, int C, const float* scale, const float* shift,
                       const float* residual, int64_t ldr, int act, float* y, int64_t ldy, pp_stream_t stream)
{
    if (!x || !scale || !shift || !y) return fail(PP_ERR_BAD_ARG, "scale_shift_act: null");
    if (int rc = need_c4(C, "scale_shift_act")) return rc;
    if (ldx % 4 || ldy % 4 || (residual && ldr % 4)) return fail(PP_ERR_BAD_ARG, "scale_shift_act: ld must be multiples of 4");
    hipLaunchKernelGGL(bn_apply_kernel, dim3(grid_for(M * (C / 4))), dim3(kT), 0, as_stream(stream), x, ldx, scale, shift,
                       residual, ldr, act, y, ldy, M, C / 4);
    return check_launch("bn_apply_kernel");
}

int pp_bn_bwd(const float* x, int64_t ldx, const float* dy, int64_t lddy, const float* y_act, int64_t ldya, int act,
              int64_t M, int C, const float* mean, const float* invstd, const float* gamma, float* dgamma, float* dbeta,
              float* dx, int64_t lddx, float* dres, int64_t lddr, void* workspace, size_t ws_bytes, pp_stream_t stream)
{
// ... 266 lines not shown
        float4 acc = make_float4(0.f, 0.f, 0.f, 0.f);
        for (int oh = lo; oh <= hi; ++oh) {
            const Lerp l = lerp_src(oh, H, sh, align);
            const float wgt = (l.i0 == ih ? l.l0 : 0.0f) + (l.i1 == ih ? l.l1 : 0.0f);
            if (wgt != 0.0f) {
                const float4 v = *reinterpret_cast<const float4*>(src + (int64_t)oh * W * cq * 4);
                acc.x = fmaf(wgt, v.x, acc.x); acc.y = fmaf(wgt, v.y, acc.y); acc.z = fmaf(wgt, v.z, acc.z); acc.w = fmaf(wgt, v.w, acc.w);
            }
        }
        *reinterpret_cast<float4*>(dx + (((int64_t)b * H + ih) * W + iw) * lddx + q * 4) = acc;
    }
}

static void bil_scales(int H, int W, int Ho, int Wo, int align, float scale_h, float scale_w, float& sh, float& sw)
{
    if (align) {
        sh = Ho > 1 ? (float)(H - 1) / (float)(Ho - 1) : 0.0f;
        sw = Wo > 1 ? (float)(W - 1) / (float)(Wo - 1) : 0.0f;
    } else {
        sh = scale_h > 0.0f ? 1.0f / scale_h : (float)H / (float)Ho;
        sw = scale_w > 0.0f ? 1.0f / scale_w : (float)W / (float)Wo;
    }
}

int pp_bilinear_fwd(const float* x, int64_t ldx, int B, int H, int W, int C, float* y, int64_t ldy, int Ho, int Wo,
                    int align_corners, float scale_h, float scale_w, int out_nchw, pp_stream_t stream)
{
    if (!x || !y) return fail(PP_ERR_BAD_ARG, "bilinear fwd: null");
    float sh, sw;
    bil_scales(H, W, Ho, Wo, align_corners, scale_h, scale_w, sh, sw);
    hipStream_t st = as_stream(stream);
    if (out_nchw) {
        hipLaunchKernelGGL((bilinear_fwd_kernel<true>), dim3(grid_for((int64_t)B * C * Ho * Wo)), dim3(kT), 0, st, x, ldx, B, H,
                           W, C, y, ldy, Ho, Wo, sh, sw, align_corners);
    } else {
        if (int rc = need_c4(C, "bilinear fwd (NHWC out)")) return rc;
        hipLaunchKernelGGL((bilinear_fwd_kernel<false>), dim3(grid_for((int64_t)B * Ho * Wo * (C / 4))), dim3(kT), 0, st, x, ldx,
                           B, H, W, C, y, ldy, Ho, Wo, sh, sw, align_corners);
    }
    return check_launch("bilinear_fwd_kernel");
}

size_t pp_bilinear_bwd_workspace_bytes(int B, int Ho, int W, int C)
{
    if (B < 1 || Ho < 1 || W < 1 || C < 1) return 0;
    return align_up((size_t)B * Ho * W * C * 4, 256);
}

int pp_bilinear_bwd(const float* dy, int64_t lddy, int B, int Ho, int Wo, int C, float* dx, int64_t lddx, int H, int W,
                    int align_corners, float scale_h, float scale_w, int dy_nchw, void* workspace, size_t ws_bytes,
                    pp_stream_t stream)
{
    if (!dy || !dx) return fail(PP_ERR_BAD_ARG, "bilinear bwd: null");
    float sh, sw;
    bil_scales(H, W, Ho, Wo, align_corners, scale_h, scale_w, sh, sw);
    hipStream_t st = as_stream(stream);
    const bool win_ok = sh > 0.0f && sw > 0.0f && (int)(2.0f / sw) + 6 <= kMaxWin;
    const bool up2_special = !align_corners && Ho == 2 * H && Wo == 2 * W && H >= 2 && W >= 2 &&
                             (scale_h == 0.0f || scale_h == 2.0f) && (scale_w == 0.0f || scale_w == 2.0f);
    if (!dy_nchw && C % 4 == 0 && lddy % 4 == 0 && lddx % 4 == 0 && sh > 0.0f && sw > 0.0f && Ho >= 3 * H && Wo >= 3 * W &&
        !up2_special && workspace && ws_bytes >= pp_bilinear_bwd_workspace_bytes(B, Ho, W, C) && g_bil_sep) {
        float* tmp = reinterpret_cast<float*>(workspace);
        const int cq = C / 4;
        hipLaunchKernelGGL(bilinear_bwd_sepw_kernel, dim3(grid_for((int64_t)B * Ho * W * cq)), dim3(kT), 0, st, dy, lddy, B, Ho, Wo, cq,
                           tmp, W, sw, align_corners);
        if (int rc = check_launch("bilinear_bwd_sepw_kernel")) return rc;
        hipLaunchKernelGGL(bilinear_bwd_seph_kernel, dim3(grid_for((int64_t)B * H * W * cq)), dim3(kT), 0, st, tmp, B, Ho, W, cq, dx,
                           lddx, H, sh, align_corners);
        return check_launch("bilinear_bwd_seph_kernel");
    }
    if (dy_nchw && win_ok) {
        hipLaunchKernelGGL(bilinear_bwd_planes_kernel, dim3(grid_for((int64_t)B * H * W * C)), dim3(kT), 0, st, dy, B, Ho, Wo, C,
                           dx, lddx, H, W, sh, sw, align_corners);
// ... 192 lines not shown
```

### pixelpick_amd/csrc/plan.hip

```cpp
#include "pp_common.h"

#include <cstring>
#include <type_traits>
#include <utility>
#include <vector>

namespace pp {
namespace {

template <typename T>
inline T unpack_slot(uint64_t s)
{
    if constexpr (std::is_same_v<T, float>) {
        float f;
        uint32_t lo = (uint32_t)s;
        memcpy(&f, &lo, 4);
        return f;
    } else if constexpr (std::is_same_v<T, double>) {
        double d;
        memcpy(&d, &s, 8);
        return d;
    } else if constexpr (std::is_pointer_v<T>) {
        return reinterpret_cast<T>(static_cast<uintptr_t>(s));
    } else {
// ... 30 lines not shown
    PP_PLAN_ENTRY(pp_acq_lowres_score_topk),
    PP_PLAN_ENTRY(pp_acq_lowres_score_at),
    PP_PLAN_ENTRY(pp_conv2d_fwd),
    PP_PLAN_ENTRY(pp_conv2d_fwd_stats),
    PP_PLAN_ENTRY(pp_bn_train_fwd_partials),
    PP_PLAN_ENTRY(pp_conv2d_fwd_bn_act),
    PP_PLAN_ENTRY(pp_dwconv3x3_fwd_bn_act),
    PP_PLAN_ENTRY(pp_bn_finalize_partials),
    PP_PLAN_ENTRY(pp_dwconv3x3_fwd_fused),
    PP_PLAN_ENTRY(pp_dwconv3x3_bwd_weight_affine_in),
    PP_PLAN_ENTRY(pp_conv2d_fwd_affine_in),
    PP_PLAN_ENTRY(pp_conv2d_bwd_data),
    PP_PLAN_ENTRY(pp_conv2d_bwd_weight),
    PP_PLAN_ENTRY(pp_conv2d_fwd_bn_train),
    PP_PLAN_ENTRY(pp_conv2d_bwd_data_bn_bwd),
    PP_PLAN_ENTRY(pp_x3_split),
    PP_PLAN_ENTRY(pp_conv2d_fwd_pre),
    PP_PLAN_ENTRY(pp_conv2d_bwd_data_pre),
    PP_PLAN_ENTRY(pp_conv2d_bwd_data_multi),
    PP_PLAN_ENTRY(pp_conv2d_fwd_pre2),
    PP_PLAN_ENTRY(pp_conv2d_bwd_data_pre2),
    PP_PLAN_ENTRY(pp_x3_split_weights),
    PP_PLAN_ENTRY(pp_conv2d_bwd_weight_pre),
    PP_PLAN_ENTRY(pp_conv2d_bwd_weight_partials),
    PP_PLAN_ENTRY(pp_wgrad_reduce_batch),
    PP_PLAN_ENTRY(pp_bn_train_fwd),
    PP_PLAN_ENTRY(pp_bn_eval_affine),
    PP_PLAN_ENTRY(pp_scale_shift_act),
    PP_PLAN_ENTRY(pp_bn_bwd),
    PP_PLAN_ENTRY(pp_bn_train_fwd_fused),
    PP_PLAN_ENTRY(pp_dwconv3x3_bn_train_fwd_fused),
    PP_PLAN_ENTRY(pp_bn_bwd_fused),
    PP_PLAN_ENTRY(pp_bn_bwd_fused_sparse),
    PP_PLAN_ENTRY(pp_row_flags),
    PP_PLAN_ENTRY(pp_conv1x1_bwd_weight_sparse),
    PP_PLAN_ENTRY(pp_conv1x1_bwd_data_sparse),
    PP_PLAN_ENTRY(pp_dwconv3x3_fwd),
    PP_PLAN_ENTRY(pp_dwconv3x3_bwd_data),
    PP_PLAN_ENTRY(pp_dwconv3x3_bwd_weight),
    PP_PLAN_ENTRY(pp_dwconv3x3_bwd_weight_partials),
    PP_PLAN_ENTRY(pp_groupnorm_relu_fwd),
    PP_PLAN_ENTRY(pp_groupnorm_relu_bwd),
    PP_PLAN_ENTRY(pp_maxpool2d_fwd),
    PP_PLAN_ENTRY(pp_maxpool2d_bwd),
    PP_PLAN_ENTRY(pp_pad2d),
    PP_PLAN_ENTRY(pp_crop2d_add),
    PP_PLAN_ENTRY(pp_bilinear_fwd),
    PP_PLAN_ENTRY(pp_bilinear_bwd),
    PP_PLAN_ENTRY(pp_image_colsum),
    PP_PLAN_ENTRY(pp_image_broadcast),
    PP_PLAN_ENTRY(pp_dropout),
    PP_PLAN_ENTRY(pp_dropout2d),
    PP_PLAN_ENTRY(pp_aug_resample_h),
    PP_PLAN_ENTRY(pp_aug_vcrop),
    PP_PLAN_ENTRY(pp_aug_labels),
    PP_PLAN_ENTRY(pp_aug_jitter),
    PP_PLAN_ENTRY(pp_aug_blur),
    PP_PLAN_ENTRY(pp_aug_blur_q8),
    PP_PLAN_ENTRY(pp_aug_to_tensor),
    PP_PLAN_ENTRY(pp_sparse_ce_fwd_bwd),
    PP_PLAN_ENTRY(pp_sparse_ce_lowres_fwd_bwd),
    PP_PLAN_ENTRY(pp_confusion_matrix_update),
    PP_PLAN_ENTRY(pp_adam_step_flat),
    PP_PLAN_ENTRY(pp_sgd_step_flat),
    PP_PLAN_ENTRY(pp_add2d),
    PP_PLAN_ENTRY(pp_nhwc_to_nchw),
    PP_PLAN_ENTRY(pp_nchw_to_nhwc),
};

const Entry* find_entry(const void* fn)
{
    for (const Entry& e : kEntries)
        if (e.fn == fn) return &e;
    return nullptr;
}

enum OpKind : int { kCall = 0, kEventRecord = 1, kStreamWait = 2, kHostBreak = 3 };

struct Op {
    int kind;
// ... 129 lines not shown
```

### pixelpick_amd/engine.py

```python
import contextlib
import math
import ctypes
import os
import weakref
from typing import List, Optional, Sequence

import torch

from . import _lib

ACT_NONE, ACT_RELU, ACT_RELU6 = 0, 1, 2


class Var:
    __slots__ = ("_t", "grad", "needs_grad", "_pending", "_lazy", "_bn_bwd_ctx", "_closed", "_grad_dst")

    def __init__(self, t: Optional[torch.Tensor], needs_grad: bool = True):
        self._t = t
        self.grad: Optional[torch.Tensor] = None
        self.needs_grad = needs_grad
        self._pending = None
        self._lazy = None
        self._bn_bwd_ctx = None
        self._closed = False
        self._grad_dst = None

    @property
    def t(self) -> torch.Tensor:
        if self._pending is not None:
            _launch_deferred(self, None)
        if self._t is None and self._lazy is not None:
            self._t = _materialise(self._lazy)
        return self._t

    @t.setter
    def t(self, value):
        self._t = value


def shape_of(v: "Var"):
    if v._pending is None:
        if v._t is None and v._lazy is not None:
            return tuple(v._lazy[0].shape)
        return tuple(v._t.shape)
    kind, x, w, _, stride, pad, dil = v._pending
    B, H, W, C = shape_of(x)
    kh, kw = (w.shape[0], w.shape[1]) if kind == "conv" else (3, 3)
    return (B, out_size(H, kh, stride, pad, dil), out_size(W, kw, stride, pad, dil), w.shape[3] if kind == "conv" else C)


_FUSE_EVAL = os.environ.get("PIXELPICK_FUSE_EVAL", "1") != "0"
_FUSE_DW_BN = os.environ.get("PIXELPICK_FUSE_DW_BN", "0")
_FUSE_DW_BN = {"0": False, "1": True}.get(_FUSE_DW_BN, _FUSE_DW_BN)
_ROWS_CACHED = {}


def _dw_bn_fusable(M: int, C: int) -> bool:
    if _FUSE_DW_BN != "auto":
# ... 332 lines not shown
        raise ValueError("channel axis must be contiguous")
    if W > 1:
        ld = t.stride(2)
    elif H > 1:
        ld = t.stride(1)
    elif B > 1:
        ld = t.stride(0)
    else:
        ld = C
    if (W > 1 and H > 1 and t.stride(1) != W * ld) or (B > 1 and (H > 1 or W > 1) and t.stride(0) != H * W * ld):
        raise ValueError(f"tensor is not a pixel-strided NHWC view: shape {tuple(t.shape)} strides {t.stride()}")
    return B, H, W, C, ld


_SCRATCH = {}
_SCRATCH_RETIRED = []
_WS_BYTES = {}


_X3_SHARE = os.environ.get("PIXELPICK_X3_SHARE", "1") != "0"


def _x3_planes(which: int, B, H, W, Cin, Cout, kh, kw, stride, pad, dil) -> int:
    return _wsbytes("pp_conv2d_x3_planes_bytes", which, B, H, W, Cin, Cout, kh, kw, stride, pad, dil) if _X3_SHARE else 0


def _x3_split(t: torch.Tensor, ld: int, rows: int, C: int) -> torch.Tensor:
    nb = _wsbytes("pp_x3_planes_bytes", rows, C)
    planes = torch.empty(nb, dtype=torch.uint8, device=t.device)
    _lib.check(_lib.lib().pp_x3_split(t.data_ptr(), ld, rows, C, planes.data_ptr(), nb, _stream()), "pp_x3_split")
    return planes


_BATCH_REDUCE = os.environ.get("PIXELPICK_BATCH_REDUCE", "0") != "0"
_ARENA_BYTES = int(os.environ.get("PIXELPICK_REDUCE_ARENA_MB", "768")) << 20
_FLUSH_BYTES = int(os.environ.get("PIXELPICK_REDUCE_FLUSH_MB", "768")) << 20
_ARENAS = {}
_JOB_POOL = (_lib.ReduceJob * 512)()


def _arena(device) -> torch.Tensor:
    key = (device.type, device.index)
    a = _ARENAS.get(key)
    if a is None:
        a = _ARENAS[key] = torch.empty(_ARENA_BYTES, dtype=torch.uint8, device=device)
    return a


def _ws(nbytes: int, device) -> torch.Tensor:
    key = (device.type, device.index, _role[0])
    buf = _SCRATCH.get(key)
    if buf is None or buf.numel() < nbytes:
        if buf is not None:
            _SCRATCH_RETIRED.append(buf)
        buf = torch.empty(max(int(nbytes), 2 * (buf.numel() if buf is not None else 0), 8 << 20), dtype=torch.uint8, device=device)
        _SCRATCH[key] = buf
    return buf


def _wsbytes(fn_name: str, *args) -> int:
    key = (fn_name,) + args
    _memo_epoch()
    n = _WS_BYTES.get(key)
    if n is None:
        n = int(getattr(_lib.lib(), fn_name)(*args))
        _WS_BYTES[key] = n
# ... 277 lines not shown
        x = self.x
        if not x.needs_grad:
            return
        if getattr(x, "_closed", False):
            raise RuntimeError("ConvBwdGroup: the input's gradient was already consumed by a fused BatchNorm backward")
        B, H, W, Cin = shape_of(x)
        dev = self.dbuf.device
        acc_into = x.grad if (x.grad is not None and getattr(x.grad, "_pp_owned", False) and x.grad.is_contiguous()
                              and tuple(x.grad.shape) == (B, H, W, Cin)) else None
        dx = acc_into if acc_into is not None else torch.empty((B, H, W, Cin), dtype=torch.float32, device=dev)
        ws = _ws(self.ws_bytes, dev)
        args = []
        for w, k, d in self.specs:
            args += [w.data_ptr(), k, d]
        args += [None, 0, 0] * (4 - self.n)
        rc = _lib.lib().pp_conv2d_bwd_data_multi(self.dbuf.data_ptr(), self.n * self.Cout, B, H, W, self.Cout, self.n, *args, dx.data_ptr(), Cin, Cin,
                                                 1 if acc_into is not None else 0, ws.data_ptr(), ws.numel(), _stream())
        _lib.check(rc, "pp_conv2d_bwd_data_multi")
        tape._keepalive.append(self.dbuf)
        if acc_into is None:
            dx._pp_owned = True
            _acc(x, dx)


def conv2d(tape: Tape, x: Var, w: torch.Tensor, bias: Optional[torch.Tensor], stride=1, pad=0, dil=1,
           dst: Optional[torch.Tensor] = None, bwd_group=None) -> Var:
    B, H, W, Cin = shape_of(x)
    kh, kw, wcin, Cout = w.shape
    assert wcin == Cin, f"conv2d: Cin {Cin} vs weight {tuple(w.shape)}"
    if _FUSE_EVAL and not tape.enabled and dst is None:
        out = Var(None, needs_grad=False)
        out._pending = ("conv", x, w, bias, stride, pad, dil)
        return out
    if (tape.enabled and dst is None and (_CONV_BN_STATS or _BN_ON_LOAD or
                                           (_CONV_BN_FUSE and bias is None and _conv_bn_fusable(B, H, W, Cin, Cout, kh, kw, stride, pad, dil)))):
        out = Var(None)
        out._pending = ("conv", x, w, bias, stride, pad, dil)
        if bwd_group is not None:
            out._grad_dst = bwd_group[0].slice(bwd_group[1])
        tape.record(_conv2d_bwd, (x, w, bias, stride, pad, dil, None, bwd_group), out)
        return out
    _, _, _, _, ldx = _geom(x.t)
    Ho, Wo = out_size(H, kh, stride, pad, dil), out_size(W, kw, stride, pad, dil)
    y = dst if dst is not None else torch.empty((B, Ho, Wo, Cout), dtype=torch.float32, device=x.t.device)
    _, _, _, _, ldy = _geom(y)
    ws, wsn = _conv_ws(False, x.t.device, B, H, W, Cin, Cout, kh, kw, stride, pad, dil)
    xp = None
    if (tape.enabled and w.requires_grad and _x3_planes(0, B, H, W, Cin, Cout, kh, kw, stride, pad, dil)
            and _x3_planes(2, B, H, W, Cin, Cout, kh, kw, stride, pad, dil)):
        xp = _x3_split(x.t, ldx, B * H * W, Cin)
    if xp is not None or (tape.enabled and w.requires_grad and _x3_planes(3, B, H, W, Cin, Cout, kh, kw, stride, pad, dil)):
        wp = _weight_planes(w, 1)
        _register_weight_planes(w, 1)
        rc = _lib.lib().pp_conv2d_fwd_pre2(x.t.data_ptr(), ldx, B, H, W, Cin, w.data_ptr(), bias.data_ptr() if bias is not None else None,
                                           kh, kw, stride, pad, dil, y.data_ptr(), ldy, Cout, ws, wsn, xp.data_ptr() if xp is not None else None, wp, _stream())
    else:
        rc = _lib.lib().pp_conv2d_fwd(x.t.data_ptr(), ldx, B, H, W, Cin, w.data_ptr(), bias.data_ptr() if bias is not None else None,
                                      kh, kw, stride, pad, dil, y.data_ptr(), ldy, Cout, ws, wsn, _stream())
    _lib.check(rc, "pp_conv2d_fwd")
    out = Var(y)
    if bwd_group is not None and tape.enabled:
        out._grad_dst = bwd_group[0].slice(bwd_group[1])
    tape.record(_conv2d_bwd, (x, w, bias, stride, pad, dil, xp, bwd_group), out)
    return out


def _conv2d_bwd(tape: Tape, dy: torch.Tensor, x: Var, w, bias, stride, pad, dil, xp=None, bwd_group=None):
    L = _lib.lib()
    lazy_in = x._lazy if (x._t is None and x._lazy is not None) else None
    B, H, W, Cin, ldx = _geom(lazy_in[0] if lazy_in is not None else x.t)
    if lazy_in is not None:
        ldx = Cin
    _, Ho, Wo, Cout, lddy = _geom(dy)
    kh, kw = w.shape[0], w.shape[1]
    dev = dy.device
    dyp = None
    if (w.requires_grad and x.needs_grad and lazy_in is None and _x3_planes(1, B, H, W, Cin, Cout, kh, kw, stride, pad, dil)
            and _x3_planes(2, B, H, W, Cin, Cout, kh, kw, stride, pad, dil)):
        dyp = _x3_split(dy, lddy, B * Ho * Wo, Cout)
    big = _BIG_WGRAD_MAIN and 2.0 * B * Ho * Wo * Cin * Cout * kh * kw >= _BIG_WGRAD_FLOP

    def _issue_wgrad():
        dw = tape.grad_buffer_for(w)
        db = tape.grad_buffer_for(bias) if (bias is not None and bias.requires_grad) else None
        with (_NULL_CTX if big else tape.side_stream_for(lazy_in[0] if lazy_in is not None else x.t, dy, dw, db)):
            if lazy_in is not None:
                tape._keepalive.append(x.t)
            nws = _wsbytes("pp_conv2d_bwd_weight_workspace_bytes", B, H, W, Cin, Cout, kh, kw, stride, pad, dil)
            slot = tape.defer_slot(nws, dev) if (not big and db is None) else None
            flags = getattr(dy, "_pp_rowflags", None) if (_SPARSE_ROWS and _SPARSE_WGRAD) else None
            nsp = (_wsbytes("pp_conv1x1_bwd_weight_sparse_workspace_bytes", B * H * W, Cin, Cout)
                   if (flags is not None and kh == 1 and kw == 1 and stride == 1 and pad == 0 and lazy_in is None and xp is None and dyp is None
                       and flags.numel() == B * H * W) else 0)
            if nsp:
                ws = _ws(nsp, dev)
                rc = L.pp_conv1x1_bwd_weight_sparse(x.t.data_ptr(), ldx, B * H * W, Cin, dy.data_ptr(), lddy, Cout, flags.data_ptr(),
                                                    dw.data_ptr(), db.data_ptr() if db is not None else None, ws.data_ptr(), ws.numel(), _stream())
                tape._keepalive.append(flags)
            elif slot is not None:
                job, wptr, _ = slot
                rc = L.pp_conv2d_bwd_weight_partials(x.t.data_ptr(), ldx, B, H, W, Cin, dy.data_ptr(), lddy, Cout, kh, kw, stride, pad, dil,
                                                     dw.data_ptr(), None, wptr, nws, ctypes.addressof(job), _stream())
                tape.defer_commit(job)
            elif xp is not None or dyp is not None:
                ws = _ws(nws, dev)
                tape._keepalive.extend(t for t in (xp, dyp) if t is not None)
                rc = L.pp_conv2d_bwd_weight_pre(x.t.data_ptr(), ldx, B, H, W, Cin, dy.data_ptr(), lddy, Cout, kh, kw, stride, pad, dil,
                                                dw.data_ptr(), db.data_ptr() if db is not None else None, ws.data_ptr(), ws.numel(),
                                                xp.data_ptr() if xp is not None else None, dyp.data_ptr() if dyp is not None else None, _stream())
            else:
                ws = _ws(nws, dev)
                rc = L.pp_conv2d_bwd_weight(x.t.data_ptr(), ldx, B, H, W, Cin, dy.data_ptr(), lddy, Cout, kh, kw, stride, pad, dil,
# ... 291 lines not shown
                                             invstd.data_ptr(), rptr, ldr, act, float(dropout_p), dseed,
                                             sd.data_ptr() if sd is not None else None, y.data_ptr(), ldy, _stream())
    _lib.check(rc, "pp_bn_train_fwd_partials")
    out = Var(y)
    tape.record(_bn_bwd, (x, gamma, beta, mean, invstd, act, residual, out, 1.0 / (1.0 - dropout_p)), out)
    return out


def _bn_on_load(tape: Tape, x: Var, gamma, beta, running_mean, running_var, act, eps, momentum):
    if x._pending[0] == "conv":
        got = _launch_conv_stats(x, max_rows=1 << 30)
    else:
        got = _launch_dw_fused(x, True)
    if got is None:
        return None
    stats, rows = got
    B, H, W, C, _ = _geom(x._t)
    dev = x._t.device
    mean, invstd, scale, shift = (torch.empty(C, dtype=torch.float32, device=dev) for _ in range(4))
    rc = _lib.lib().pp_bn_finalize_partials(stats.data_ptr(), rows, B * H * W, C, gamma.data_ptr(), beta.data_ptr(), eps, momentum,
                                            running_mean.data_ptr() if running_mean is not None else None,
                                            running_var.data_ptr() if running_var is not None else None, mean.data_ptr(),
                                            invstd.data_ptr(), scale.data_ptr(), shift.data_ptr(), _stream())
    _lib.check(rc, "pp_bn_finalize_partials")
    out = Var(None)
    out._lazy = (x._t, scale, shift, act)
    tape.record(_bn_bwd, (x, gamma, beta, mean, invstd, act, None, out, 1.0), out)
    return out


def batch_norm_act(tape: Tape, x: Var, gamma, beta, running_mean, running_var, training: bool, act: int = ACT_NONE,
                   residual: Optional[Var] = None, eps: float = 1e-5, momentum: float = 0.1,
                   dst: Optional[torch.Tensor] = None, dropout_p: float = 0.0, lazy_ok: bool = False, single_consumer: bool = False,
                   consumers: int = 0) -> Var:
    if (lazy_ok and _BN_ON_LOAD and training and tape.enabled and x._pending is not None and residual is None and dropout_p == 0.0
            and dst is None and shape_of(x)[3] % 4 == 0 and 4 * math.prod(shape_of(x)) >= _BN_ON_LOAD_MIN_BYTES):
        out = _bn_on_load(tape, x, gamma, beta, running_mean, running_var, act, eps, momentum)
        if out is not None:
            return out
    if dropout_p > 0.0 and not (training and _BN_FUSED and act != ACT_RELU6 and dst is None and _bn_exchange_ok(x.t.device)):
        y = batch_norm_act(tape, x, gamma, beta, running_mean, running_var, training, act, residual, eps, momentum, dst)
        return dropout(tape, y, dropout_p, True)
    if not training and x._pending is not None and not tape.enabled:
        _launch_deferred(x, (gamma, beta, running_mean, running_var, eps, act, residual, dst))
        return Var(x._t, needs_grad=False)
    L = _lib.lib()
    if training and x._pending is not None and x._pending[0] == "conv" and tape.enabled and _CONV_BN_FUSE and dropout_p == 0.0:
        ncons = consumers if consumers > 0 else (1 if (lazy_ok or single_consumer) else 0)
        out = _conv_bn_train_fused(tape, x, gamma, beta, running_mean, running_var, act, residual, eps, momentum, dst,
                                   ncons if (dst is None and (residual is None or act == ACT_NONE)) else 0)
        if out is not None:
            return out
    if training and x._pending is not None and x._pending[0] == "conv" and tape.enabled and _CONV_BN_STATS:
        out = _conv_bn_train_partials(tape, x, gamma, beta, running_mean, running_var, act, residual, eps, momentum, dst, dropout_p)
        if out is not None:
            return out
    if (training and x._pending is not None and x._pending[0] == "dw" and tape.enabled and dropout_p == 0.0 and _BN_FUSED
            and _FUSE_DW_BN and _dw_bn_fusable(*_dw_out_rows(x._pending[1], *x._pending[4:7])) and _bn_exchange_ok(x._pending[1].t.device)):
        fused = _dw_bn_train_fused(tape, x, gamma, beta, running_mean, running_var, act, residual, eps, momentum, dst)
        if fused is not None:
            return fused
    B, H, W, C, ldx = _geom(x.t)
    M = B * H * W
    dev = x.t.device
    if training and _BN_FUSED and M <= _BN_FUSED_MAXM and C <= 65536 and _bn_exchange_ok(dev):
        mean = torch.empty(C, dtype=torch.float32, device=dev)
        invstd = torch.empty(C, dtype=torch.float32, device=dev)
        y = dst if dst is not None else torch.empty((B, H, W, C), dtype=torch.float32, device=dev)
        _, _, _, _, ldy = _geom(y)
        rptr, ldr = (None, 0)
        if residual is not None:
            _, _, _, _, ldr = _geom(residual.t)
            rptr = residual.t.data_ptr()
        sync, ws = _bn_exchange(dev)
        dseed, sd = 0, None
        if dropout_p > 0.0:
            _dropout_counter[0] += 1
            dseed = (_dropout_counter[0] * 0x9E3779B97F4A7C15) & 0xFFFFFFFFFFFFFFFF
            sd = _dropout_seed_dev[0]
        rc = L.pp_bn_train_fwd_fused(x.t.data_ptr(), ldx, M, C, gamma.data_ptr(), beta.data_ptr(), eps, momentum,
                                     running_mean.data_ptr() if running_mean is not None else None,
                                     running_var.data_ptr() if running_var is not None else None,
                                     mean.data_ptr(), invstd.data_ptr(), rptr, ldr, act, float(dropout_p), dseed,
                                     sd.data_ptr() if sd is not None else None, y.data_ptr(), ldy,
                                     ws.data_ptr(), ws.numel(), sync.data_ptr(), sync.numel(), _stream())
        _lib.check(rc, "pp_bn_train_fwd_fused")
        out = Var(y)
        tape.record(_bn_bwd, (x, gamma, beta, mean, invstd, act, residual, out, 1.0 / (1.0 - dropout_p)), out)
        ncons = consumers if consumers > 0 else (1 if (lazy_ok or single_consumer) else 0)
        if ncons and dropout_p == 0.0 and dst is None and (residual is None or act == ACT_NONE):
            out._bn_bwd_ctx = (x, gamma, beta, mean, invstd, act, residual, ncons)
        return out
    scale = torch.empty(C, dtype=torch.float32, device=dev)
    shift = torch.empty(C, dtype=torch.float32, device=dev)
    mean = invstd = None
    if training:
        mean = torch.empty(C, dtype=torch.float32, device=dev)
        invstd = torch.empty(C, dtype=torch.float32, device=dev)
        ws = _ws(_wsbytes("pp_colreduce_workspace_bytes", M, C), dev)
        rc = L.pp_bn_train_fwd(x.t.data_ptr(), ldx, M, C, gamma.data_ptr(), beta.data_ptr(), eps, momentum,
                               running_mean.data_ptr() if running_mean is not None else None,
                               running_var.data_ptr() if running_var is not None else None,
                               mean.data_ptr(), invstd.data_ptr(), scale.data_ptr(), shift.data_ptr(),
                               ws.data_ptr(), ws.numel(), _stream())
        _lib.check(rc, "pp_bn_train_fwd")
    else:
        rc = L.pp_bn_eval_affine(C, gamma.data_ptr(), beta.data_ptr(), running_mean.data_ptr(), running_var.data_ptr(), eps,
                                 scale.data_ptr(), shift.data_ptr(), _stream())
        _lib.check(rc, "pp_bn_eval_affine")
    y = dst if dst is not None else torch.empty((B, H, W, C), dtype=torch.float32, device=dev)
    _, _, _, _, ldy = _geom(y)
    rptr, ldr = (None, 0)
    if residual is not None:
        _, _, _, _, ldr = _geom(residual.t)
        rptr = residual.t.data_ptr()
    rc = L.pp_scale_shift_act(x.t.data_ptr(), ldx, M, C, scale.data_ptr(), shift.data_ptr(), rptr, ldr, act, y.data_ptr(), ldy, _stream())
    _lib.check(rc, "pp_scale_shift_act")
    out = Var(y)
    if training:
        tape.record(_bn_bwd, (x, gamma, beta, mean, invstd, act, residual, out, 1.0), out)
    else:
        tape.record(_bn_eval_bwd, (x, scale, act, residual, out), out)
    return out


def _bn_bwd(tape: Tape, dy, x: Var, gamma, beta, mean, invstd, act, residual, out: Var, gscale: float = 1.0):
    L = _lib.lib()
    B, H, W, C, ldx = _geom(x.t)
    M = B * H * W
    _, _, _, _, lddy = _geom(dy)
    lazy_out = out._t is None and out._lazy is not None
    ldya = 0 if lazy_out else _geom(out.t)[4]
    dev = dy.device
    dgamma = tape.grad_buffer_for(gamma)
    dbeta = tape.grad_buffer_for(beta)
    gd = x._grad_dst if x.grad is None else None
    if gd is not None and not (tuple(gd.shape) == (B, H, W, C) and gd.stride(3) == 1 and gd.stride(2) % 4 == 0 and gd.data_ptr() % 16 == 0
                               and gd.stride(1) == W * gd.stride(2) and gd.stride(0) == H * gd.stride(1)):
        gd = None
    dx = gd if gd is not None else torch.empty((B, H, W, C), dtype=torch.float32, device=dev)
    lddx = dx.stride(2)
    dres = torch.empty((B, H, W, C), dtype=torch.float32, device=dev) if (residual is not None and residual.needs_grad) else None
    if _BN_FUSED and M <= _BN_FUSED_MAXM and C <= 65536 and _bn_exchange_ok(dev):
        sync, ws = _bn_exchange(dev)
        remask = (act != ACT_NONE and residual is None and gscale == 1.0) or lazy_out
        flags = getattr(dy, "_pp_rowflags", None) if _SPARSE_ROWS else None
        if flags is not None and flags.numel() == M:
            rc = L.pp_bn_bwd_fused_sparse(x.t.data_ptr(), ldx, dy.data_ptr(), lddy, None if remask else out.t.data_ptr(), ldya, act, M, C,
                                        mean.data_ptr(), invstd.data_ptr(), gamma.data_ptr(), dgamma.data_ptr(), dbeta.data_ptr(),
                                        dx.data_ptr(), lddx, dres.data_ptr() if dres is not None else None, C, float(gscale),
                                        beta.data_ptr(), ws.data_ptr(), ws.numel(), sync.data_ptr(), sync.numel(), flags.data_ptr(), _stream())
            tape._keepalive.append(flags)
        else:
            rc = L.pp_bn_bwd_fused(x.t.data_ptr(), ldx, dy.data_ptr(), lddy, None if remask else out.t.data_ptr(), ldya, act, M, C,
                                   mean.data_ptr(), invstd.data_ptr(), gamma.data_ptr(), dgamma.data_ptr(), dbeta.data_ptr(),
                                   dx.data_ptr(), lddx, dres.data_ptr() if dres is not None else None, C, float(gscale),
                                   beta.data_ptr(), ws.data_ptr(), ws.numel(), sync.data_ptr(), sync.numel(), _stream())
        _lib.check(rc, "pp_bn_bwd_fused")
    else:
        assert gscale == 1.0, "a fused dropout is only created together with the single-launch BatchNorm"
        ws = _ws(_wsbytes("pp_colreduce_workspace_bytes", M, C), dev)
        rc = L.pp_bn_bwd(x.t.data_ptr(), ldx, dy.data_ptr(), lddy, out.t.data_ptr(), ldya, act, M, C, mean.data_ptr(), invstd.data_ptr(),
                         gamma.data_ptr(), dgamma.data_ptr(), dbeta.data_ptr(), dx.data_ptr(), lddx,
                         dres.data_ptr() if dres is not None else None, C, ws.data_ptr(), ws.numel(), _stream())
        _lib.check(rc, "pp_bn_bwd")
    if gamma.requires_grad:
        tape.set_param_grad(gamma, dgamma)
    if beta.requires_grad:
        tape.set_param_grad(beta, dbeta)
    _acc(x, dx)
    if dres is not None:
        dres._pp_owned = True
        _acc(residual, dres)


def _bn_eval_bwd(tape: Tape, dy, x: Var, scale, act, residual, out: Var):
    raise RuntimeError("backward through eval-mode BatchNorm is not part of the PixelPick path "
                       "(query.py:148-158 and model.py:176-190 run eval under no_grad)")


def pad2d(tape: Tape, x: Var, pad_beg: int, pad_end: int) -> Var:
    B, H, W, C, ldx = _geom(x.t)
    Hp, Wp = H + pad_beg + pad_end, W + pad_beg + pad_end
    y = torch.empty((B, Hp, Wp, C), dtype=torch.float32, device=x.t.device)
    rc = _lib.lib().pp_pad2d(x.t.data_ptr(), ldx, B, H, W, C, pad_beg, pad_beg, Hp, Wp, y.data_ptr(), C, _stream())
    _lib.check(rc, "pp_pad2d")
    out = Var(y)
    tape.record(_pad_bwd, (x, pad_beg), out)
    return out


def _pad_bwd(tape: Tape, dy, x: Var, pad_beg):
    if not x.needs_grad:
        return
    B, H, W, C, _ = _geom(x.t)
    _, Hp, Wp, _, lddy = _geom(dy)
    dx = torch.empty((B, H, W, C), dtype=torch.float32, device=dy.device)
    add_ptr, ldadd = (None, 0)
    if x.grad is not None:
        _, _, _, _, ldadd = _geom(x.grad)
        add_ptr = x.grad.data_ptr()
    rc = _lib.lib().pp_crop2d_add(dy.data_ptr(), lddy, B, Hp, Wp, C, pad_beg, pad_beg, add_ptr, ldadd, dx.data_ptr(), C, H, W, _stream())
    _lib.check(rc, "pp_crop2d_add")
    x.grad = dx


def bilinear(tape: Tape, x: Var, size, align_corners: bool, scale_factor: float = 0.0, out_nchw: bool = False,
             dst: Optional[torch.Tensor] = None) -> Var:
    B, H, W, C, ldx = _geom(x.t)
    Ho, Wo = int(size[0]), int(size[1])
    dev = x.t.device
    if out_nchw:
        y = torch.empty((B, C, Ho, Wo), dtype=torch.float32, device=dev)
        ldy = 0
    else:
        y = dst if dst is not None else torch.empty((B, Ho, Wo, C), dtype=torch.float32, device=dev)
        _, _, _, _, ldy = _geom(y)
    rc = _lib.lib().pp_bilinear_fwd(x.t.data_ptr(), ldx, B, H, W, C, y.data_ptr(), ldy, Ho, Wo, int(align_corners),
                                    float(scale_factor), float(scale_factor), int(out_nchw), _stream())
    _lib.check(rc, "pp_bilinear_fwd")
    out = Var(y)
    tape.record(_bilinear_bwd, (x, (Ho, Wo), align_corners, scale_factor, out_nchw), out)
    return out


def _bilinear_bwd(tape: Tape, dy, x: Var, size, align_corners, scale_factor, out_nchw):
    if not x.needs_grad:
        return
    B, H, W, C, _ = _geom(x.t)
    Ho, Wo = size
    if out_nchw:
        dy = dy.contiguous()
        lddy = 0
    else:
        _, _, _, _, lddy = _geom(dy)
    dx = torch.empty((B, H, W, C), dtype=torch.float32, device=dy.device)
    ws_ptr, ws_n = None, 0
    if not out_nchw and Ho >= 3 * H and Wo >= 3 * W:
        ws = _ws(_wsbytes("pp_bilinear_bwd_workspace_bytes", B, Ho, W, C), dy.device)
        ws_ptr, ws_n = ws.data_ptr(), ws.numel()
    rc = _lib.lib().pp_bilinear_bwd(dy.data_ptr(), lddy, B, Ho, Wo, C, dx.data_ptr(), C, H, W, int(align_corners),
                                    float(scale_factor), float(scale_factor), int(out_nchw), ws_ptr, ws_n, _stream())
    _lib.check(rc, "pp_bilinear_bwd")
    _acc(x, dx)


def global_avg_pool(tape: Tape, x: Var) -> Var:
    B, H, W, C, ldx = _geom(x.t)
    y = torch.empty((B, 1, 1, C), dtype=torch.float32, device=x.t.device)
    rc = _lib.lib().pp_image_colsum(x.t.data_ptr(), ldx, B, H * W, C, 1.0 / (H * W), y.data_ptr(), C, _stream())
    _lib.check(rc, "pp_image_colsum")
    out = Var(y)
    tape.record(_gap_bwd, (x,), out)
    return out
# ... 146 lines not shown
    _lib.check(rc, "pp_dropout")
    _acc(x, dx)


def dropout2d(tape: Tape, x: Var, p: float, training: bool) -> Var:
    if not training or p <= 0.0:
        return x
    B, H, W, C, ldx = _geom(x.t)
    _dropout_counter[0] += 1
    seed = (_dropout_counter[0] * 0x9E3779B97F4A7C15) & 0xFFFFFFFFFFFFFFFF
    y = torch.empty((B, H, W, C), dtype=torch.float32, device=x.t.device)
    sd = _dropout_seed_dev[0]
    rc = _lib.lib().pp_dropout2d(x.t.data_ptr(), ldx, y.data_ptr(), C, B, H * W, C, float(p), seed,
                                 sd.data_ptr() if sd is not None else None, _stream())
    _lib.check(rc, "pp_dropout2d")
    out = Var(y, needs_grad=x.needs_grad)
    tape.record(_dropout2d_bwd, (x, p, seed), out)
    return out


def _dropout2d_bwd(tape: Tape, dy, x: Var, p, seed):
    if not x.needs_grad:
        return
    B, H, W, C, _ = _geom(x.t)
    _, _, _, _, lddy = _geom(dy)
    dx = torch.empty((B, H, W, C), dtype=torch.float32, device=dy.device)
    sd = _dropout_seed_dev[0]
    rc = _lib.lib().pp_dropout2d(dy.data_ptr(), lddy, dx.data_ptr(), C, B, H * W, C, float(p), seed,
                                 sd.data_ptr() if sd is not None else None, _stream())
    _lib.check(rc, "pp_dropout2d")
    _acc(x, dx)


def concat_alias(tape: Tape, buf: torch.Tensor, parts: Sequence[Var]) -> Var:
    off = 0
    for p in parts:
        c = p.t.shape[3]
        assert p.t.data_ptr() == buf[..., off:off + c].data_ptr(), "concat_alias: part not produced in place"
        off += c
    assert off == buf.shape[3]
    out = Var(buf)
    tape.record(_concat_bwd, (tuple(parts),), out)
    return out


def _concat_bwd(tape: Tape, dy, parts):
    off = 0
    for p in parts:
        c = p.t.shape[3]
        _acc(p, dy[..., off:off + c])
        off += c


def cross_entropy_nchw(logits: torch.Tensor, target: torch.Tensor, ignore_index: int, want_grad: bool = True, sparse: bool = True):
    assert logits.is_cuda and logits.dtype == torch.float32 and logits.dim() == 4
    B, C, H, W = logits.shape
    assert logits.stride(3) == 1 and logits.stride(2) == W, "logits planes must be contiguous"
    target = target.to(logits.device, torch.int64).contiguous()
    L = _lib.lib()
    dev = logits.device
    loss = torch.empty(1, dtype=torch.float32, device=dev)
    count = torch.empty(1, dtype=torch.float32, device=dev)
    dl = torch.empty((B, C, H, W), dtype=torch.float32, device=dev) if want_grad else None
    ws = _ws(_wsbytes("pp_sparse_ce_workspace_bytes"), dev)
    rc = L.pp_sparse_ce_fwd_bwd(logits.data_ptr(), B, C, H * W, logits.stride(0), logits.stride(1), target.data_ptr(),
                                int(ignore_index), loss.data_ptr(), count.data_ptr(), None,
                                dl.data_ptr() if dl is not None else None, ws.data_ptr(), ws.numel(), _stream())
    _lib.check(rc, "pp_sparse_ce_fwd_bwd")
    if dl is not None and sparse:
        dl._pp_sparse_rows = True
    return loss, dl


def cross_entropy_lowres(low: torch.Tensor, size, target: torch.Tensor, ignore_index: int, align_corners: bool = True,
# ... 23 lines not shown
```

### pixelpick_amd/networks/backbones/resnet_backbone.py

```python
import math
from collections import OrderedDict
from functools import partial

import torch
import torch.nn as nn

from ... import engine as E
from ..layers import BatchNorm2d, Conv2d, ReLU


class Bottleneck(nn.Module):
    expansion = 4

    def __init__(self, inplanes, planes, stride=1, downsample=None):
        super().__init__()
        self.conv1 = Conv2d(inplanes, planes, 1, bias=False)
        self.bn1 = BatchNorm2d(planes)
        self.conv2 = Conv2d(planes, planes, 3, stride=stride, padding=1, bias=False)
        self.bn2 = BatchNorm2d(planes)
        self.conv3 = Conv2d(planes, planes * 4, 1, bias=False)
        self.bn3 = BatchNorm2d(planes * 4)
        self.relu = ReLU(inplace=True)
        self.downsample = downsample
        self.stride = stride

    def run(self, tape, x):
        out = self.bn1.run(tape, self.conv1.run(tape, x), E.ACT_RELU)
        out = self.bn2.run(tape, self.conv2.run(tape, out), E.ACT_RELU)
        residual = x
        if self.downsample is not None:
            residual = self.downsample[1].run(tape, self.downsample[0].run(tape, x))
        return self.bn3.run(tape, self.conv3.run(tape, out), E.ACT_RELU, residual=residual)


class ResNet(nn.Module):

    def __init__(self, block, layers, width_multiplier=1.0):
        super().__init__()
        self.inplanes = int(64 * width_multiplier)
        self.prefix = nn.Sequential(OrderedDict([
            ('conv1', Conv2d(3, self.inplanes, 7, stride=2, padding=3, bias=False)),
            ('bn1', BatchNorm2d(self.inplanes)),
            ('relu', ReLU(inplace=False))]))
        self.maxpool = nn.Identity()
        self.layer1 = self._make_layer(block, int(64 * width_multiplier), layers[0])
        self.layer2 = self._make_layer(block, int(128 * width_multiplier), layers[1], stride=2)
        self.layer3 = self._make_layer(block, int(256 * width_multiplier), layers[2], stride=2)
        self.layer4 = self._make_layer(block, int(512 * width_multiplier), layers[3], stride=2)
        for m in self.modules():
            if isinstance(m, Conv2d):
                n = m.kernel_size * m.kernel_size * m.out_channels
                with torch.no_grad():
                    m.weight.normal_(0, math.sqrt(2. / n))

    def _make_layer(self, block, planes, blocks, stride=1):
        downsample = None
        if stride != 1 or self.inplanes != planes * block.expansion:
            downsample = nn.Sequential(Conv2d(self.inplanes, planes * block.expansion, 1, stride=stride, bias=False),
                                       BatchNorm2d(planes * block.expansion))
        layers = [block(self.inplanes, planes, stride, downsample)]
        self.inplanes = planes * block.expansion
# ... 79 lines not shown
```

### pixelpick_amd/networks/decoders.py

```python
import math

import torch
import torch.nn as nn

from .. import engine as E
from .layers import BatchNorm2d, Conv2d, Dropout, ReLU


class GroupNorm(nn.Module):

    def __init__(self, num_groups, num_channels, eps=1e-5):
        super().__init__()
        self.num_groups, self.num_channels, self.eps = num_groups, num_channels, eps
        self.weight = nn.Parameter(torch.ones(num_channels))
        self.bias = nn.Parameter(torch.zeros(num_channels))

    def run(self, tape, x, relu=True):
        return E.group_norm_relu(tape, x, self.weight, self.bias, self.num_groups, relu, self.eps)

    def forward(self, x):
        raise RuntimeError("pixelpick_amd layers execute through run(tape, x)")


class UpsampleBlock(nn.Module):
# ... 53 lines not shown

    def run(self, tape, feats, lowres=False):
        c2, c3, c4, c5 = feats
        c5 = self.lat_layer_0.run(tape, c5)
        c4 = self.lat_layer_1.run(tape, c4)
        c3 = self.lat_layer_2.run(tape, c3)
        c2 = self.lat_layer_3.run(tape, c2)
        p5 = c5
        p4 = self._upsample_add(tape, p5, c4)
        p3 = self._upsample_add(tape, p4, c3)
        p2 = self._upsample_add(tape, p3, c2)
        p5 = self._seq(tape, self.upsample_blocks_0, p5, not lowres)
        p4 = self._seq(tape, self.upsample_blocks_1, p4, not lowres)
        p3 = self._seq(tape, self.upsample_blocks_2, p3, not lowres)
        p2 = self._seq(tape, self.upsample_blocks_3, p2, not lowres)
        emb = E.add(tape, E.add(tape, E.add(tape, p2, p3), p4), p5)
        if lowres:
            return {"emb": None, "pred": self.classifier.run(tape, emb)}
        return {"emb": emb, "pred": self.classifier.run(tape, emb)}


class SegmentHead(nn.Module):
    def __init__(self, args, openset=False):
        super().__init__()
        self.segment_head = nn.Sequential(Conv2d(304, 256, kernel_size=3, stride=1, padding=1, bias=False),
                                          BatchNorm2d(256), ReLU(), Dropout(0.5),
                                          Conv2d(256, 256, kernel_size=3, stride=1, padding=1, bias=False),
                                          BatchNorm2d(256), ReLU(), Dropout(args.mc_dropout_p))
        self.classifier = Conv2d(256, args.n_classes, 1)
        self.n_classes = args.n_classes

    def run(self, tape, x):
        s = self.segment_head
        h = s[1].run(tape, s[0].run(tape, x), E.ACT_RELU, dropout=s[3])
        emb = s[5].run(tape, s[4].run(tape, h), E.ACT_RELU, dropout=s[7])
        pred = self.classifier.run(tape, emb)
        return {"emb": emb, "pred": pred}
```

### pixelpick_amd/networks/deeplab.py

```python
import torch
import torch.nn as nn

from .. import engine as E
from .aspp import ASPP
from .decoders import SegmentHead
from .layers import BatchNorm2d, Conv2d, Dropout, ReLU
from .mobilenet_v2 import MobileNetV2


class _LazyOutputs(dict):

    def __init__(self, pred, emb_low, size):
        super().__init__(pred=pred)
        self._emb_low, self._size = emb_low, size

    def _emb(self):
        if not dict.__contains__(self, "emb"):
            v = E.bilinear(E.Tape(False), E.Var(self._emb_low), self._size, True, 0.0, out_nchw=True)
            dict.__setitem__(self, "emb", v.t)
        return dict.__getitem__(self, "emb")

    def __getitem__(self, k):
        return self._emb() if k == "emb" else dict.__getitem__(self, k)

# ... 46 lines not shown
        self.seg_head = SegmentHead(args)
        self.return_features = False
        self.return_attention = False
        self._last_emb_low = None

    def turn_on_dropout(self):
        for m in self.modules():
            if isinstance(m, Dropout):
                m.train()

    def turn_off_dropout(self):
        for m in self.modules():
            if isinstance(m, Dropout):
                m.eval()

    def set_return_features(self, return_features):
        self.return_features = return_features

    def set_return_attention(self, return_attention):
        self.return_attention = return_attention

    def _run(self, tape, inputs, upsample=True):
        B, _, H, W = inputs.shape
        x = E.nchw_to_nhwc(inputs)
        if self._resnet:
            feats = self.backbone.run(tape, x)
            high, low = feats[3], feats[0]
        else:
            high, low = self.backbone.run(tape, x)
        tape.mark("encoder_done")
        a = self.aspp.run(tape, high)
        _, Hl, Wl, _ = low.t.shape
        cat_buf = torch.empty((B, Hl, Wl, 304), dtype=torch.float32, device=inputs.device)
        up = E.bilinear(tape, a, (Hl, Wl), True, 0.0, dst=cat_buf[..., 0:256])
        llc = self.low_level_conv
        low_ = llc[1].run(tape, llc[0].run(tape, low), E.ACT_RELU, dst=cat_buf[..., 256:304])
        cat = E.concat_alias(tape, cat_buf, [up, low_])
        outs = self.seg_head.run(tape, cat)
        if not upsample:
            return outs["pred"], outs["emb"]
        pred = E.bilinear(tape, outs["pred"], (H, W), True, 0.0, out_nchw=True)
        return pred, outs["emb"]

    def forward_lowres(self, inputs):
        if not inputs.is_cuda:
            raise RuntimeError("pixelpick_amd.DeepLab runs on the GPU only (no CPU fallback)")
        pred_v, _ = self._run(E.Tape(enabled=False), inputs.to(torch.float32), upsample=False)
        return pred_v.t, tuple(inputs.shape[2:])

    def forward(self, inputs):
        if not inputs.is_cuda:
            raise RuntimeError("pixelpick_amd.DeepLab runs on the GPU only (no CPU fallback); move the model and "
                               "inputs to cuda")
        inputs = inputs.to(torch.float32)
        params = [p for p in self.parameters()]
        if torch.is_grad_enabled() and any(p.requires_grad for p in params):
            pred = _NetFunction.apply(inputs, self, *params)
            emb_low = self._last_emb_low
        else:
            pred_v, emb_v = self._run(E.Tape(enabled=False), inputs)
            pred, emb_low = pred_v.t, emb_v.t
        return _LazyOutputs(pred, emb_low, tuple(inputs.shape[2:]))
```

### pixelpick_amd/networks/layers.py

```python
import math

import torch
import torch.nn as nn

from .. import _lib
from .. import engine as E


def _bump_nbt(d):
    d["_nbt_pending"] += 1


def _kaiming_normal_oihw(cout, cin_per_group, kh, kw, nonlinearity_gain=math.sqrt(2.0)):
    fan_in = cin_per_group * kh * kw
    std = nonlinearity_gain / math.sqrt(fan_in)
    return torch.randn(cout, cin_per_group, kh, kw) * std


class Conv2d(nn.Module):

    def __init__(self, in_channels, out_channels, kernel_size, stride=1, padding=0, dilation=1, groups=1, bias=True):
        super().__init__()
        assert groups in (1, in_channels), "only dense and depthwise convolutions occur in the reference"
        self.in_channels, self.out_channels = in_channels, out_channels
# ... 57 lines not shown
        return E.conv_accepts_lazy_input(B, H, W, C, self.out_channels, k, k, self.stride, self.padding + extra_pad, self.dilation)

    def run(self, tape, x, dst=None, extra_pad: int = 0, bwd_group=None):
        if self.depthwise:
            return E.dwconv3x3(tape, x, self.weight, self.stride, self.padding + extra_pad, self.dilation)
        return E.conv2d(tape, x, self.weight, self.bias, self.stride, self.padding + extra_pad, self.dilation, dst=dst, bwd_group=bwd_group)

    def forward(self, x):
        raise RuntimeError("pixelpick_amd layers execute through run(tape, x); call the network's forward()")

    def extra_repr(self):
        return (f"{self.in_channels}, {self.out_channels}, kernel_size={self.kernel_size}, stride={self.stride}, "
                f"padding={self.padding}, dilation={self.dilation}, groups={self.groups}, bias={self.bias is not None}")


class BatchNorm2d(nn.Module):

    def __init__(self, num_features, eps=1e-5, momentum=0.1):
        super().__init__()
        self.num_features, self.eps, self.momentum = num_features, eps, momentum
        self.weight = nn.Parameter(torch.ones(num_features))
        self.bias = nn.Parameter(torch.zeros(num_features))
        self.register_buffer("running_mean", torch.zeros(num_features))
        self.register_buffer("running_var", torch.ones(num_features))
        self.register_buffer("num_batches_tracked", torch.tensor(0, dtype=torch.long))
        self._nbt_pending = 0

    def _save_to_state_dict(self, destination, prefix, keep_vars):
        if self._nbt_pending:
            self.num_batches_tracked += self._nbt_pending
            self._nbt_pending = 0
        super()._save_to_state_dict(destination, prefix, keep_vars)

    def run(self, tape, x, act=E.ACT_NONE, residual=None, dst=None, dropout=None, lazy_ok=False, single_consumer=False, consumers=0):
        training = self.training
        if training:
            B, H, W, _ = E.shape_of(x)
            if B * H * W <= 1:
                raise ValueError(f"Expected more than 1 value per channel when training, got input size {tuple(x.t.shape)}")
            _lib.plan_note_host(_bump_nbt, self.__dict__)
        drop_p = dropout.p if (dropout is not None and dropout.training and dropout.p > 0.0) else 0.0
        return E.batch_norm_act(tape, x, self.weight, self.bias, self.running_mean, self.running_var, training, act,
                                residual, self.eps, self.momentum, dst=dst, dropout_p=drop_p, lazy_ok=lazy_ok,
                                single_consumer=single_consumer, consumers=consumers)

    def forward(self, x):
        raise RuntimeError("pixelpick_amd layers execute through run(tape, x)")

    def extra_repr(self):
        return f"{self.num_features}, eps={self.eps}, momentum={self.momentum}"


class _Placeholder(nn.Module):

    def forward(self, x):
        return x


class ReLU(_Placeholder):
    def __init__(self, inplace=False):
        super().__init__()


class ReLU6(_Placeholder):
    def __init__(self, inplace=False):
        super().__init__()


class Dropout2d(nn.Module):

    def __init__(self, p=0.5):
        super().__init__()
        self.p = p

    def run(self, tape, x):
        return E.dropout2d(tape, x, self.p, self.training)

    def forward(self, x):
        return x

    def extra_repr(self):
        return f"p={self.p}"

# ... 16 lines not shown
```

Measured before the change: 748.9 images/s.

## Write bf16x3 conv operand planes directly from BN and bilinear producers

Adds plane-writing variants of the fused BN forward/backward and bilinear kernels. They emit the hi/mid/lo bf16 split operand planes the x3 conv consumes, and skip the fp32 output when it is not needed. This is meant to remove the separate x3_split pass and the fp32 round trip before the decoder convs. It also adds a 256x160 single-tile conv_x3 launch for channel counts like 304. The cost is more kernel template variants, occupancy checks that now also include the plane kernels, and extra plumbing through the decoder and backbone.

```diff
diff --git a/include/pixelpick_hip.h b/include/pixelpick_hip.h
--- a/include/pixelpick_hip.h
+++ b/include/pixelpick_hip.h
@@ -210,6 +210,26 @@
                          void* workspace, size_t ws_bytes, int32_t* sync, size_t sync_ints, const unsigned char* row_flags,
                          pp_stream_t stream);
 
+int pp_bn_train_fwd_fused_planes(const float* x, int64_t ldx, int64_t M, int C, const float* gamma, const float* beta, float eps,
+                                 float momentum, float* running_mean, float* running_var, float* mean, float* invstd,
+                                 const float* residual, int64_t ldr, int act, float drop_p, uint64_t drop_seed,
+                                 const uint64_t* drop_seed_dev, float* y, int64_t ldy, void* workspace,
+                                 size_t ws_bytes, int32_t* sync, size_t sync_ints, void* planes, size_t planes_bytes, int Kp, int c0,
+                                 int store_f32, pp_stream_t stream);
+int pp_bn_bwd_fused_planes(const float* x, int64_t ldx, const float* dy, int64_t lddy, const float* y_act, int64_t ldya, int act,
+                           int64_t M, int C, const float* mean, const float* invstd, const float* gamma, float* dgamma,
+                           float* dbeta, float* dx, int64_t lddx, float* dres, int64_t lddr, float grad_scale, const float* beta,
+                           void* workspace, size_t ws_bytes, int32_t* sync, size_t sync_ints, void* planes, size_t planes_bytes, int Kp,
+                           int c0, int store_f32, pp_stream_t stream);
+int pp_bn_bwd_fused_sparse_planes(const float* x, int64_t ldx, const float* dy, int64_t lddy, const float* y_act, int64_t ldya, int act,
+                                  int64_t M, int C, const float* mean, const float* invstd, const float* gamma, float* dgamma,
+                                  float* dbeta, float* dx, int64_t lddx, float* dres, int64_t lddr, float grad_scale, const float* beta,
+                                  void* workspace, size_t ws_bytes, int32_t* sync, size_t sync_ints, const unsigned char* row_flags,
+                                  void* planes, size_t planes_bytes, int Kp, int c0, int store_f32, pp_stream_t stream);
+int pp_bilinear_fwd_planes(const float* x, int64_t ldx, int B, int H, int W, int C, float* y, int64_t ldy, int Ho, int Wo,
+                           int align_corners, float scale_h, float scale_w, void* planes, size_t planes_bytes, int Kp, int c0,
+                           int store_f32, pp_stream_t stream);
+
 int pp_bn_eval_affine(int C, const float* gamma, const float* beta, const float* running_mean, const float* running_var,
                       float eps, float* scale, float* shift, pp_stream_t stream);
 
diff --git a/pixelpick_amd/_lib.py b/pixelpick_amd/_lib.py
--- a/pixelpick_amd/_lib.py
+++ b/pixelpick_amd/_lib.py
@@ -89,6 +89,13 @@
                                                _p, _i64, _int, _p, _i64, _p, _sz, _p, _sz, _p]),
     "pp_bn_bwd_fused": (_int, [_p, _i64, _p, _i64, _p, _i64, _int, _i64, _int, _p, _p, _p, _p, _p, _p, _i64, _p, _i64, _f, _p, _p, _sz, _p, _sz, _p]),
     "pp_bn_bwd_fused_sparse": (_int, [_p, _i64, _p, _i64, _p, _i64, _int, _i64, _int, _p, _p, _p, _p, _p, _p, _i64, _p, _i64, _f, _p, _p, _sz, _p, _sz, _p, _p]),
+    "pp_bn_train_fwd_fused_planes": (_int, [_p, _i64, _i64, _int, _p, _p, _f, _f, _p, _p, _p, _p, _p, _i64, _int, _f, _u64, _p, _p, _i64, _p, _sz, _p, _sz,
+                                            _p, _sz, _int, _int, _int, _p]),
+    "pp_bn_bwd_fused_planes": (_int, [_p, _i64, _p, _i64, _p, _i64, _int, _i64, _int, _p, _p, _p, _p, _p, _p, _i64, _p, _i64, _f, _p, _p, _sz, _p, _sz,
+                                      _p, _sz, _int, _int, _int, _p]),
+    "pp_bn_bwd_fused_sparse_planes": (_int, [_p, _i64, _p, _i64, _p, _i64, _int, _i64, _int, _p, _p, _p, _p, _p, _p, _i64, _p, _i64, _f, _p, _p, _sz, _p, _sz,
+                                             _p, _p, _sz, _int, _int, _int, _p]),
+    "pp_bilinear_fwd_planes": (_int, [_p, _i64, _int, _int, _int, _int, _p, _i64, _int, _int, _int, _f, _f, _p, _sz, _int, _int, _int, _p]),
     "pp_row_flags": (_int, [_p, _i64, _i64, _int, _p, _p]),
     "pp_conv1x1_bwd_weight_sparse_workspace_bytes": (_sz, [_i64, _int, _int]),
     "pp_conv1x1_bwd_weight_sparse": (_int, [_p, _i64, _i64, _int, _p, _i64, _int, _p, _p, _p, _p, _sz, _p]),
diff --git a/pixelpick_amd/csrc/conv_igemm.hip b/pixelpick_amd/csrc/conv_igemm.hip
--- a/pixelpick_amd/csrc/conv_igemm.hip
+++ b/pixelpick_amd/csrc/conv_igemm.hip
@@ -4,6 +4,7 @@
 #include "pp_common.h"
 #include "bn_xchg.h"
 #include "conv_types.h"
+#include "x3_planes.h"
 
 namespace pp {
 
@@ -2483,23 +2484,6 @@
     if (t < 8 && c < C) dbias[c] = (float)sh[t];
 }
 
-__device__ __forceinline__ uint16_t f32_to_bf16_rne(float f)
-{
-    uint32_t u = __float_as_uint(f);
-    if ((u & 0x7F800000u) == 0x7F800000u) return (uint16_t)(u >> 16);
-    u += 0x7FFFu + ((u >> 16) & 1u);
-    return (uint16_t)(u >> 16);
-}
-__device__ __forceinline__ float bf16_to_f32(uint16_t h) { return __uint_as_float((uint32_t)h << 16); }
-
-__device__ __forceinline__ void x3_split1(float v, uint16_t& hi, uint16_t& mid, uint16_t& lo)
-{
-    hi = f32_to_bf16_rne(v);
-    const float r1 = v - bf16_to_f32(hi);
-    mid = f32_to_bf16_rne(r1);
-    const float r2 = r1 - bf16_to_f32(mid);
-    lo = f32_to_bf16_rne(r2);
-}
 
 __global__ __launch_bounds__(256) void x3_split_kernel(const float* x, int64_t ldx, int64_t rows, int C, uint16_t* out, int Kp, int64_t plane)
 {
@@ -2530,7 +2514,7 @@
         ph.x = h[0] | ((uint32_t)h[1] << 16); ph.y = h[2] | ((uint32_t)h[3] << 16); ph.z = h[4] | ((uint32_t)h[5] << 16); ph.w = h[6] | ((uint32_t)h[7] << 16);
         pm.x = m[0] | ((uint32_t)m[1] << 16); pm.y = m[2] | ((uint32_t)m[3] << 16); pm.z = m[4] | ((uint32_t)m[5] << 16); pm.w = m[6] | ((uint32_t)m[7] << 16);
         pl.x = l[0] | ((uint32_t)l[1] << 16); pl.y = l[2] | ((uint32_t)l[3] << 16); pl.z = l[4] | ((uint32_t)l[5] << 16); pl.w = l[6] | ((uint32_t)l[7] << 16);
-        const int64_t o = e * 8;
+        const int64_t o = x3_plane_off(rows, r, c0);
         *reinterpret_cast<uint4*>(out + o) = ph;
         *reinterpret_cast<uint4*>(out + plane + o) = pm;
         *reinterpret_cast<uint4*>(out + 2 * plane + o) = pl;
@@ -2600,12 +2584,13 @@
                  : "=&s"(keep), "=&s"(t) : "v"(voff), "s"(b0), "s"(b1), "s"(b2), "s"(d0), "s"(st) : "memory", "scc");
 }
 
-template <int BM, int BN, int VAR = 0>
+template <int BM, int BN, int VAR = 0, int TMW = 2, int WNW = 2>
 __global__ __launch_bounds__(BM * 2, (BM == 128 ? 2 : 2)) void conv_x3_kernel(ConvParams p, X3Operands o)
 {
-    constexpr int TM = 2, TN = BN / 64, WN = 2, NWAVE = BM / 32;
-    constexpr int NSTAGE = VAR == 1 ? 3 : VAR == 2 ? 2 : (BM == 256 && BN == 128) ? 4 : (BM == 256 ? 5 : 3);
-    constexpr bool PROD = VAR == 0 && BM == 256 && BN == 128;
+    constexpr int TM = TMW, WN = WNW, TN = BN / (32 * WN), NWAVE = BM / 32;
+    static_assert((BM / (32 * TM)) * WN == NWAVE && TN * 32 * WN == BN, "every wave DMAs 32 A rows: BM / 32 waves");
+    constexpr int NSTAGE = VAR == 1 ? 3 : VAR == 2 ? 2 : (BM == 256 && BN >= 128) ? 4 : (BM == 256 ? 5 : 3);
+    constexpr bool PROD = VAR == 0 && BM == 256 && BN >= 128;
     constexpr bool PAIR = PROD || VAR == 8 || VAR == 9;
     constexpr bool LATE_BEGIN = PROD || VAR == 9 || VAR == 10;
     constexpr int PRE = PAIR ? NSTAGE - 1 : NSTAGE;
@@ -2613,6 +2598,7 @@
     constexpr int STAGE_BYTES = 3 * (A_BYTES + B_BYTES);
     constexpr int NBW = BN / 32;
     static_assert(NBW <= NWAVE, "B rows are loaded by the first BN/32 waves");
+    static_assert(NSTAGE * STAGE_BYTES + 32 * 2 * 4 <= 160 * 1024, "ring + tap table in 160 KiB of LDS");
     __shared__ __attribute__((aligned(1024))) unsigned char smem[NSTAGE * STAGE_BYTES];
     struct Frags { bf16x8_t a[3][TM], b[3][TN]; };
 
@@ -3240,6 +3226,14 @@
     p.part = nullptr;
     const int full128 = p.Cn / 128, rem = p.Cn - full128 * 128;
     const bool two = rem > 0 && rem <= 64 && full128 > 0 && !(g_conv_x3 & 4);
+    const bool one160 = two && !(g_conv_x3 & 16) && !(g_conv_x3 & 2) && !f32path && g_x3_var == 0 && !p.stats &&
+                        (rem <= 32 || 2 * 160 >= p.Cn) && cdiv(p.M, 256) * cdiv(p.Cn, 160) >= 200;
+    if (one160) {
+        o.col_base = 0;
+        p.n_tiles = (int)cdiv(p.Cn, 160);
+        hipLaunchKernelGGL((conv_x3_kernel<256, 160, 0, 1, 1>), dim3((unsigned)(cdiv(p.M, 256) * p.n_tiles)), dim3(512), 0, st, p, o);
+        return check_launch("conv_x3_kernel");
+    }
     bool n128_only = !two && (rem == 0 || rem > 64 || (g_conv_x3 & 4));
     const int64_t mt256 = cdiv(p.M, 256);
     if (f32path && n128_only && rem == 0 && cdiv(p.M, 128) * full128 < 200 && cdiv(p.M, 128) * full128 * 2 >= 128) n128_only = false;
diff --git a/pixelpick_amd/csrc/nn_ops.hip b/pixelpick_amd/csrc/nn_ops.hip
--- a/pixelpick_amd/csrc/nn_ops.hip
+++ b/pixelpick_amd/csrc/nn_ops.hip
@@ -1,5 +1,6 @@
 #include "pp_common.h"
 #include "bn_xchg.h"
+#include "x3_planes.h"
 
 namespace pp {
 
@@ -360,6 +361,7 @@
     int dw_H, dw_W, dw_Ho, dw_Wo, dw_stride, dw_pad, dw_dil;
     const float* stats; int stat_rows;
     unsigned long long* probe;
+    X3PlanesOut xp;
 };
 #define BN_STAMP(i) do { if (a.probe && threadIdx.x == 0) a.probe[(int64_t)blockIdx.x * 8 + (i)] = wall_clock64(); } while (0)
 
@@ -388,7 +390,7 @@
     return acc;
 }
 
-template <int MODE, int NC = 0>
+template <int MODE, int NC = 0, bool PLANES = false>
 __global__ __launch_bounds__(kT) void bn_fused_fwd_kernel(BnFwdArgs a)
 {
     constexpr bool DW = MODE == 1;
@@ -404,6 +406,9 @@
     BN_STAMP(0);
     if constexpr (MODE != 2) tag0 = tag_issue(a.sync);
     const int t = threadIdx.x;
+    if constexpr (PLANES) {
+        if (blockIdx.x == 0) x3_store_zero_row(a.xp, a.C, t, kT);
+    }
     const int strip = blockIdx.x % g.nstrips, chunk = blockIdx.x / g.nstrips;
     const int ql = t % g.bq, rl = t / g.bq;
     const int q = strip * g.bq + ql;
@@ -555,6 +560,10 @@
             }
             oa.x = act_fwd(oa.x, act); oa.y = act_fwd(oa.y, act); oa.z = act_fwd(oa.z, act); oa.w = act_fwd(oa.w, act);
             if (drop) drop4(oa, (uint64_t)(r * g.cq + q) * 4, dseed, a.drop_p, a.drop_inv_keep);
+            if constexpr (PLANES) {
+                x3_store4(a.xp, r, q * 4, a.C, oa);
+                if (a.xp.store_f32) *reinterpret_cast<float4*>(yq + r * a.ldy) = oa;
+            } else
             *reinterpret_cast<float4*>(yq + r * a.ldy) = oa;
         }
         BN_STAMP(5);
@@ -578,6 +587,10 @@
             if (rq) { o.x += rv[j].x; o.y += rv[j].y; o.z += rv[j].z; o.w += rv[j].w; }
             o.x = act_fwd(o.x, act); o.y = act_fwd(o.y, act); o.z = act_fwd(o.z, act); o.w = act_fwd(o.w, act);
             if (drop) drop4(o, (uint64_t)(rr * g.cq + q) * 4, dseed, a.drop_p, a.drop_inv_keep);
+            if constexpr (PLANES) {
+                x3_store4(a.xp, rr, q * 4, a.C, o);
+                if (a.xp.store_f32) *reinterpret_cast<float4*>(yq + rr * a.ldy) = o;
+            } else
             *reinterpret_cast<float4*>(yq + rr * a.ldy) = o;
         }
     }
@@ -591,10 +604,11 @@
     float gscale;
     const float* beta_mask;
     const unsigned char* rowflag;
+    X3PlanesOut xp;
 };
 
 __device__ __attribute__((aligned(16))) float g_bn_zero4[4] = {0.f, 0.f, 0.f, 0.f};
-template <int NC, bool SPARSE = false>
+template <int NC, bool SPARSE = false, bool PLANES = false>
 __global__ __launch_bounds__(kT) void bn_fused_bwd_kernel(BnBwdArgs a)
 {
     static_assert(!SPARSE || NC == 0, "row flags: the uncached variant");
@@ -608,6 +622,9 @@
     const BnFusedGeom g = a.g;
     const unsigned tag0 = tag_issue(a.sync);
     const int t = threadIdx.x;
+    if constexpr (PLANES) {
+        if (blockIdx.x == 0) x3_store_zero_row(a.xp, a.C, t, kT);
+    }
     const int strip = blockIdx.x % g.nstrips, chunk = blockIdx.x / g.nstrips;
     const int ql = t % g.bq, rl = t / g.bq;
     const int q = strip * g.bq + ql;
@@ -750,6 +767,10 @@
             o.y = bn_dx(u.y, v.y, mu.y, is.y, ga.y, db.y, dg.y, inv_count);
             o.z = bn_dx(u.z, v.z, mu.z, is.z, ga.z, db.z, dg.z, inv_count);
             o.w = bn_dx(u.w, v.w, mu.w, is.w, ga.w, db.w, dg.w, inv_count);
+            if constexpr (PLANES) {
+                x3_store4(a.xp, r, q * 4, a.C, o);
+                if (a.xp.store_f32) *reinterpret_cast<float4*>(dxq + r * a.lddx) = o;
+            } else
             *reinterpret_cast<float4*>(dxq + r * a.lddx) = o;
         }
         return;
@@ -805,6 +826,10 @@
             o.y = bn_dx(u.y, v.y, mu.y, is.y, ga.y, db.y, dg.y, inv_count);
             o.z = bn_dx(u.z, v.z, mu.z, is.z, ga.z, db.z, dg.z, inv_count);
             o.w = bn_dx(u.w, v.w, mu.w, is.w, ga.w, db.w, dg.w, inv_count);
+            if constexpr (PLANES) {
+                x3_store4(a.xp, rr, q * 4, a.C, o);
+                if (a.xp.store_f32) *reinterpret_cast<float4*>(dxq + rr * a.lddx) = o;
+            } else
             *reinterpret_cast<float4*>(dxq + rr * a.lddx) = o;
         }
     }
@@ -827,12 +852,22 @@
             (void)hipGetLastError();
             return 0;
         }
+        int pl[5] = {0, 0, 0, 0, 0};
+        if (hipOccupancyMaxActiveBlocksPerMultiprocessor(&pl[0], (bn_fused_fwd_kernel<0, 0, true>), kT, 0) != hipSuccess ||
+            hipOccupancyMaxActiveBlocksPerMultiprocessor(&pl[1], (bn_fused_fwd_kernel<0, kBnRowCache, true>), kT, 0) != hipSuccess ||
+            hipOccupancyMaxActiveBlocksPerMultiprocessor(&pl[2], (bn_fused_bwd_kernel<0, false, true>), kT, 0) != hipSuccess ||
+            hipOccupancyMaxActiveBlocksPerMultiprocessor(&pl[3], (bn_fused_bwd_kernel<0, true, true>), kT, 0) != hipSuccess ||
+            hipOccupancyMaxActiveBlocksPerMultiprocessor(&pl[4], (bn_fused_bwd_kernel<kBnRowCache, false, true>), kT, 0) != hipSuccess) {
+            (void)hipGetLastError();
+            return 0;
+        }
         int per = a < b ? a : b;
         per = per < c ? per : c;
         per = per < d ? per : d;
         per = per < e ? per : e;
         per = per < f ? per : f;
         per = per < sp ? per : sp;
+        for (int v : pl) per = per < v ? per : v;
         return per * cus;
     }();
     return reserve_scaled(cap, bn_device_cus());
@@ -1340,12 +1375,16 @@
 }
 
 
-template <bool OUT_NCHW>
+template <bool OUT_NCHW, bool PLANES = false>
 __global__ __launch_bounds__(kT) void bilinear_fwd_kernel(const float* x, int64_t ldx, int B, int H, int W, int C,
                                                          float* y, int64_t ldy, int Ho, int Wo, float sh, float sw,
-                                                         int align)
-{
+                                                         int align, X3PlanesOut xp)
+{
+    static_assert(!(OUT_NCHW && PLANES), "operand planes are channels-last");
     if constexpr (!OUT_NCHW) {
+        if constexpr (PLANES) {
+            if (blockIdx.x == 0) x3_store_zero_row(xp, C, threadIdx.x, kT);
+        }
         const int cq = C / 4;
         const int64_t total = (int64_t)B * Ho * Wo * cq;
         for (int64_t e = (int64_t)blockIdx.x * kT + threadIdx.x; e < total; e += (int64_t)gridDim.x * kT) {
@@ -1374,7 +1413,12 @@
             o.y = bilerp(lh.l0, lh.l1, lw.l0, lw.l1, v00.y, v01.y, v10.y, v11.y);
             o.z = bilerp(lh.l0, lh.l1, lw.l0, lw.l1, v00.z, v01.z, v10.z, v11.z);
             o.w = bilerp(lh.l0, lh.l1, lw.l0, lw.l1, v00.w, v01.w, v10.w, v11.w);
-            *reinterpret_cast<float4*>(y + (((int64_t)b * Ho + oh) * Wo + ow) * ldy + q * 4) = o;
+            const int64_t row = ((int64_t)b * Ho + oh) * Wo + ow;
+            if constexpr (PLANES) {
+                x3_store4(xp, row, q * 4, C, o);
+                if (xp.store_f32) *reinterpret_cast<float4*>(y + row * ldy + q * 4) = o;
+            } else
+            *reinterpret_cast<float4*>(y + row * ldy + q * 4) = o;
         }
     } else {
         const int64_t total = (int64_t)B * C * Ho * Wo;
@@ -2029,6 +2073,22 @@
     return PP_OK;
 }
 
+static int x3_planes_arg(const char* what, void* planes, size_t planes_bytes, int64_t rows, int C, int Kp, int c0, int store_f32,
+                         const void* f32, X3PlanesOut& o)
+{
+    if (!planes) return fail(PP_ERR_BAD_ARG, "%s: planes is NULL", what);
+    if (rows < 1 || C < 4 || C % 4 != 0) return fail(PP_ERR_BAD_ARG, "%s: rows=%lld C=%d", what, (long long)rows, C);
+    if (Kp < 16 || Kp % 16 != 0 || c0 < 0 || c0 % 16 != 0 || (int64_t)c0 + C > Kp)
+        return fail(PP_ERR_BAD_ARG, "%s: Kp=%d and c0=%d must be multiples of 16 with c0 + C <= Kp", what, Kp, c0);
+    if (reinterpret_cast<uintptr_t>(planes) & 255) return fail(PP_ERR_BAD_ARG, "%s: planes must be 256-byte aligned", what);
+    if (store_f32 && !f32) return fail(PP_ERR_BAD_ARG, "%s: the fp32 output is NULL but store_f32 is set", what);
+    const int64_t plane = (rows + 1) * Kp;
+    if (plane * 2 >= (1ll << 32) - 4096) return fail(PP_ERR_UNSUPPORTED, "%s: plane of %lld bytes", what, (long long)(plane * 2));
+    if (planes_bytes < pp_x3_planes_bytes(rows, Kp)) return fail(PP_ERR_WORKSPACE, "%s: planes buffer", what);
+    o = X3PlanesOut{reinterpret_cast<uint16_t*>(planes), plane, rows, c0, store_f32 ? 1 : 0};
+    return PP_OK;
+}
+
 }
 
 using namespace pp;
@@ -2121,27 +2181,57 @@
     return PP_OK;
 }
 
-int pp_bn_train_fwd_fused(const float* x, int64_t ldx, int64_t M, int C, const float* gamma, const float* beta, float eps,
-                          float momentum, float* running_mean, float* running_var, float* mean, float* invstd,
-                          const float* residual, int64_t ldr, int act, float drop_p, uint64_t drop_seed,
-                          const uint64_t* drop_seed_dev, float* y, int64_t ldy, void* workspace,
-                          size_t ws_bytes, int32_t* sync, size_t sync_ints, pp_stream_t stream)
+static int bn_train_fwd_fused_impl(const float* x, int64_t ldx, int64_t M, int C, const float* gamma, const float* beta, float eps,
+                                   float momentum, float* running_mean, float* running_var, float* mean, float* invstd,
+                                   const float* residual, int64_t ldr, int act, float drop_p, uint64_t drop_seed,
+                                   const uint64_t* drop_seed_dev, float* y, int64_t ldy, void* workspace,
+                                   size_t ws_bytes, int32_t* sync, size_t sync_ints, pp_stream_t stream, const X3PlanesOut* planes)
 {
     if (drop_p < 0.0f || drop_p >= 1.0f) return fail(PP_ERR_BAD_ARG, "bn_train_fwd_fused: dropout p=%f outside [0,1)", (double)drop_p);
     if (drop_p > 0.0f && act == 2) return fail(PP_ERR_UNSUPPORTED, "bn_train_fwd_fused: dropout after ReLU6 is not fusable");
-    if (!x || !gamma || !beta || !mean || !invstd || !y) return fail(PP_ERR_BAD_ARG, "bn_train_fwd_fused: null");
+    if (!x || !gamma || !beta || !mean || !invstd || (!y && !planes)) return fail(PP_ERR_BAD_ARG, "bn_train_fwd_fused: null");
     if (int rc = need_c4(C, "bn_train_fwd_fused")) return rc;
     if (ldx % 4 || ldy % 4 || (residual && ldr % 4)) return fail(PP_ERR_BAD_ARG, "bn_train_fwd_fused: ld must be multiples of 4");
     BnFusedGeom g = bn_fused_geom(M, C);
     if (int rc = bn_fused_check("bn_train_fwd_fused", M, C, g, workspace, ws_bytes, sync, sync_ints)) return rc;
     BnFwdArgs a{x, ldx, M, C, gamma, beta, eps, momentum, running_mean, running_var, mean, invstd, residual, ldr, act, y, ldy,
                 reinterpret_cast<xword*>(workspace), sync, g, drop_p, 1.0f / (1.0f - drop_p), drop_seed, drop_seed_dev,
-                nullptr, 0, nullptr, nullptr, 0, 0, 0, 0, 0, 0, 0, nullptr, 0, g_bn_probe};
-    if (g_bn_row_cache && g.rows_per_chunk <= (int64_t)g.nrl * kBnRowCache)
-        hipLaunchKernelGGL((bn_fused_fwd_kernel<0, kBnRowCache>), dim3((unsigned)(g.nstrips * g.R)), dim3(kT), 0, as_stream(stream), a);
+                nullptr, 0, nullptr, nullptr, 0, 0, 0, 0, 0, 0, 0, nullptr, 0, g_bn_probe, planes ? *planes : X3PlanesOut{}};
+    const bool cached = g_bn_row_cache && g.rows_per_chunk <= (int64_t)g.nrl * kBnRowCache;
+    const dim3 grid((unsigned)(g.nstrips * g.R));
+    if (planes) {
+        if (cached) hipLaunchKernelGGL((bn_fused_fwd_kernel<0, kBnRowCache, true>), grid, dim3(kT), 0, as_stream(stream), a);
+        else        hipLaunchKernelGGL((bn_fused_fwd_kernel<0, 0, true>), grid, dim3(kT), 0, as_stream(stream), a);
+        return check_launch("bn_fused_fwd_kernel<planes>");
+    }
+    if (cached)
+        hipLaunchKernelGGL((bn_fused_fwd_kernel<0, kBnRowCache>), grid, dim3(kT), 0, as_stream(stream), a);
     else
-        hipLaunchKernelGGL((bn_fused_fwd_kernel<0, 0>), dim3((unsigned)(g.nstrips * g.R)), dim3(kT), 0, as_stream(stream), a);
+        hipLaunchKernelGGL((bn_fused_fwd_kernel<0, 0>), grid, dim3(kT), 0, as_stream(stream), a);
     return check_launch("bn_fused_fwd_kernel");
+}
+
+int pp_bn_train_fwd_fused(const float* x, int64_t ldx, int64_t M, int C, const float* gamma, const float* beta, float eps,
+                          float momentum, float* running_mean, float* running_var, float* mean, float* invstd,
+                          const float* residual, int64_t ldr, int act, float drop_p, uint64_t drop_seed,
+                          const uint64_t* drop_seed_dev, float* y, int64_t ldy, void* workspace,
+                          size_t ws_bytes, int32_t* sync, size_t sync_ints, pp_stream_t stream)
+{
+    return bn_train_fwd_fused_impl(x, ldx, M, C, gamma, beta, eps, momentum, running_mean, running_var, mean, invstd, residual, ldr, act,
+                                   drop_p, drop_seed, drop_seed_dev, y, ldy, workspace, ws_bytes, sync, sync_ints, stream, nullptr);
+}
+
+int pp_bn_train_fwd_fused_planes(const float* x, int64_t ldx, int64_t M, int C, const float* gamma, const float* beta, float eps,
+                                 float momentum, float* running_mean, float* running_var, float* mean, float* invstd,
+                                 const float* residual, int64_t ldr, int act, float drop_p, uint64_t drop_seed,
+                                 const uint64_t* drop_seed_dev, float* y, int64_t ldy, void* workspace,
+                                 size_t ws_bytes, int32_t* sync, size_t sync_ints, void* planes, size_t planes_bytes, int Kp, int c0,
+                                 int store_f32, pp_stream_t stream)
+{
+    X3PlanesOut o{};
+    if (int rc = x3_planes_arg("bn_train_fwd_fused_planes", planes, planes_bytes, M, C, Kp, c0, store_f32, y, o)) return rc;
+    return bn_train_fwd_fused_impl(x, ldx, M, C, gamma, beta, eps, momentum, running_mean, running_var, mean, invstd, residual, ldr, act,
+                                   drop_p, drop_seed, drop_seed_dev, y, ldy, workspace, ws_bytes, sync, sync_ints, stream, &o);
 }
 
 int pp_bn_train_fwd_partials(const float* x, int64_t ldx, int64_t M, int C, const float* stats, int64_t stat_rows, const float* gamma,
@@ -2193,7 +2283,7 @@
                              int64_t M, int C, const float* mean, const float* invstd, const float* gamma, float* dgamma,
                              float* dbeta, float* dx, int64_t lddx, float* dres, int64_t lddr, float grad_scale, const float* beta,
                              void* workspace, size_t ws_bytes, int32_t* sync, size_t sync_ints, pp_stream_t stream,
-                             const unsigned char* row_flags);
+                             const unsigned char* row_flags, const X3PlanesOut* planes = nullptr);
 
 int pp_bn_bwd_fused(const float* x, int64_t ldx, const float* dy, int64_t lddy, const float* y_act, int64_t ldya, int act,
                     int64_t M, int C, const float* mean, const float* invstd, const float* gamma, float* dgamma,
@@ -2212,6 +2302,30 @@
 {
     return bn_bwd_fused_impl(x, ldx, dy, lddy, y_act, ldya, act, M, C, mean, invstd, gamma, dgamma, dbeta, dx, lddx, dres, lddr, grad_scale,
                              beta, workspace, ws_bytes, sync, sync_ints, stream, row_flags);
+}
+
+int pp_bn_bwd_fused_planes(const float* x, int64_t ldx, const float* dy, int64_t lddy, const float* y_act, int64_t ldya, int act,
+                           int64_t M, int C, const float* mean, const float* invstd, const float* gamma, float* dgamma,
+                           float* dbeta, float* dx, int64_t lddx, float* dres, int64_t lddr, float grad_scale, const float* beta,
+                           void* workspace, size_t ws_bytes, int32_t* sync, size_t sync_ints, void* planes, size_t planes_bytes, int Kp,
+                           int c0, int store_f32, pp_stream_t stream)
+{
+    X3PlanesOut o{};
+    if (int rc = x3_planes_arg("bn_bwd_fused_planes", planes, planes_bytes, M, C, Kp, c0, store_f32, dx, o)) return rc;
+    return bn_bwd_fused_impl(x, ldx, dy, lddy, y_act, ldya, act, M, C, mean, invstd, gamma, dgamma, dbeta, dx, lddx, dres, lddr, grad_scale,
+                             beta, workspace, ws_bytes, sync, sync_ints, stream, nullptr, &o);
+}
+
+int pp_bn_bwd_fused_sparse_planes(const float* x, int64_t ldx, const float* dy, int64_t lddy, const float* y_act, int64_t ldya, int act,
+                                  int64_t M, int C, const float* mean, const float* invstd, const float* gamma, float* dgamma,
+                                  float* dbeta, float* dx, int64_t lddx, float* dres, int64_t lddr, float grad_scale, const float* beta,
+                                  void* workspace, size_t ws_bytes, int32_t* sync, size_t sync_ints, const unsigned char* row_flags,
+                                  void* planes, size_t planes_bytes, int Kp, int c0, int store_f32, pp_stream_t stream)
+{
+    X3PlanesOut o{};
+    if (int rc = x3_planes_arg("bn_bwd_fused_sparse_planes", planes, planes_bytes, M, C, Kp, c0, store_f32, dx, o)) return rc;
+    return bn_bwd_fused_impl(x, ldx, dy, lddy, y_act, ldya, act, M, C, mean, invstd, gamma, dgamma, dbeta, dx, lddx, dres, lddr, grad_scale,
+                             beta, workspace, ws_bytes, sync, sync_ints, stream, row_flags, &o);
 }
 
 __global__ __launch_bounds__(256) void row_flags_kernel(const float* dy, int64_t ld, int64_t M, int C, unsigned char* flags)
@@ -2365,9 +2479,9 @@
                              int64_t M, int C, const float* mean, const float* invstd, const float* gamma, float* dgamma,
                              float* dbeta, float* dx, int64_t lddx, float* dres, int64_t lddr, float grad_scale, const float* beta,
                              void* workspace, size_t ws_bytes, int32_t* sync, size_t sync_ints, pp_stream_t stream,
-                             const unsigned char* row_flags)
-{
-    if (!x || !dy || !mean || !invstd || !gamma || !dgamma || !dbeta || !dx) return fail(PP_ERR_BAD_ARG, "bn_bwd_fused: null");
+                             const unsigned char* row_flags, const X3PlanesOut* planes)
+{
+    if (!x || !dy || !mean || !invstd || !gamma || !dgamma || !dbeta || (!dx && !planes)) return fail(PP_ERR_BAD_ARG, "bn_bwd_fused: null");
     if (act != 0 && !y_act && !beta) return fail(PP_ERR_BAD_ARG, "bn_bwd_fused: the mask needs the activation output or beta");
     if (!y_act && act != 0 && (dres || grad_scale != 1.0f))
         return fail(PP_ERR_BAD_ARG, "bn_bwd_fused: the mask can only be recomputed from x without residual / dropout");
@@ -2377,7 +2491,17 @@
     BnFusedGeom g = bn_fused_geom(M, C);
     if (int rc = bn_fused_check("bn_bwd_fused", M, C, g, workspace, ws_bytes, sync, sync_ints)) return rc;
     BnBwdArgs a{x, ldx, dy, lddy, y_act, ldya, act, M, C, mean, invstd, gamma, dgamma, dbeta, dx, lddx, dres, lddr,
-                reinterpret_cast<xword*>(workspace), sync, g, grad_scale, y_act ? nullptr : beta, row_flags};
+                reinterpret_cast<xword*>(workspace), sync, g, grad_scale, y_act ? nullptr : beta, row_flags, planes ? *planes : X3PlanesOut{}};
+    if (planes) {
+        const dim3 grid((unsigned)(g.nstrips * g.R));
+        if (g_bn_row_cache && g.rows_per_chunk <= (int64_t)g.nrl * kBnRowCache)
+            hipLaunchKernelGGL((bn_fused_bwd_kernel<kBnRowCache, false, true>), grid, dim3(kT), 0, as_stream(stream), a);
+        else if (row_flags)
+            hipLaunchKernelGGL((bn_fused_bwd_kernel<0, true, true>), grid, dim3(kT), 0, as_stream(stream), a);
+        else
+            hipLaunchKernelGGL((bn_fused_bwd_kernel<0, false, true>), grid, dim3(kT), 0, as_stream(stream), a);
+        return check_launch("bn_fused_bwd_kernel<planes>");
+    }
     if (g_bn_row_cache && g.rows_per_chunk <= (int64_t)g.nrl * kBnRowCache)
         hipLaunchKernelGGL(bn_fused_bwd_kernel<kBnRowCache>, dim3((unsigned)(g.nstrips * g.R)), dim3(kT), 0, as_stream(stream), a);
     else if (row_flags)
@@ -2710,13 +2834,29 @@
     hipStream_t st = as_stream(stream);
     if (out_nchw) {
         hipLaunchKernelGGL((bilinear_fwd_kernel<true>), dim3(grid_for((int64_t)B * C * Ho * Wo)), dim3(kT), 0, st, x, ldx, B, H,
-                           W, C, y, ldy, Ho, Wo, sh, sw, align_corners);
+                           W, C, y, ldy, Ho, Wo, sh, sw, align_corners, X3PlanesOut{});
     } else {
         if (int rc = need_c4(C, "bilinear fwd (NHWC out)")) return rc;
         hipLaunchKernelGGL((bilinear_fwd_kernel<false>), dim3(grid_for((int64_t)B * Ho * Wo * (C / 4))), dim3(kT), 0, st, x, ldx,
-                           B, H, W, C, y, ldy, Ho, Wo, sh, sw, align_corners);
+                           B, H, W, C, y, ldy, Ho, Wo, sh, sw, align_corners, X3PlanesOut{});
     }
     return check_launch("bilinear_fwd_kernel");
+}
+
+int pp_bilinear_fwd_planes(const float* x, int64_t ldx, int B, int H, int W, int C, float* y, int64_t ldy, int Ho, int Wo,
+                           int align_corners, float scale_h, float scale_w, void* planes, size_t planes_bytes, int Kp, int c0,
+                           int store_f32, pp_stream_t stream)
+{
+    if (!x) return fail(PP_ERR_BAD_ARG, "bilinear fwd (planes): null");
+    if (B < 1 || H < 1 || W < 1 || Ho < 1 || Wo < 1 || ldx % 4 != 0 || (store_f32 && ldy % 4 != 0))
+        return fail(PP_ERR_BAD_ARG, "bilinear fwd (planes): bad shape / ld");
+    X3PlanesOut o{};
+    if (int rc = x3_planes_arg("bilinear_fwd_planes", planes, planes_bytes, (int64_t)B * Ho * Wo, C, Kp, c0, store_f32, y, o)) return rc;
+    float sh, sw;
+    bil_scales(H, W, Ho, Wo, align_corners, scale_h, scale_w, sh, sw);
+    hipLaunchKernelGGL((bilinear_fwd_kernel<false, true>), dim3(grid_for((int64_t)B * Ho * Wo * (C / 4))), dim3(kT), 0, as_stream(stream), x, ldx,
+                       B, H, W, C, y, ldy, Ho, Wo, sh, sw, align_corners, o);
+    return check_launch("bilinear_fwd_kernel<planes>");
 }
 
 size_t pp_bilinear_bwd_workspace_bytes(int B, int Ho, int W, int C)
diff --git a/pixelpick_amd/csrc/plan.hip b/pixelpick_amd/csrc/plan.hip
--- a/pixelpick_amd/csrc/plan.hip
+++ b/pixelpick_amd/csrc/plan.hip
@@ -86,6 +86,9 @@
     PP_PLAN_ENTRY(pp_dwconv3x3_bn_train_fwd_fused),
     PP_PLAN_ENTRY(pp_bn_bwd_fused),
     PP_PLAN_ENTRY(pp_bn_bwd_fused_sparse),
+    PP_PLAN_ENTRY(pp_bn_train_fwd_fused_planes),
+    PP_PLAN_ENTRY(pp_bn_bwd_fused_planes),
+    PP_PLAN_ENTRY(pp_bn_bwd_fused_sparse_planes),
     PP_PLAN_ENTRY(pp_row_flags),
     PP_PLAN_ENTRY(pp_conv1x1_bwd_weight_sparse),
     PP_PLAN_ENTRY(pp_conv1x1_bwd_data_sparse),
@@ -100,6 +103,7 @@
     PP_PLAN_ENTRY(pp_pad2d),
     PP_PLAN_ENTRY(pp_crop2d_add),
     PP_PLAN_ENTRY(pp_bilinear_fwd),
+    PP_PLAN_ENTRY(pp_bilinear_fwd_planes),
     PP_PLAN_ENTRY(pp_bilinear_bwd),
     PP_PLAN_ENTRY(pp_image_colsum),
     PP_PLAN_ENTRY(pp_image_broadcast),
diff --git a/pixelpick_amd/csrc/x3_planes.h b/pixelpick_amd/csrc/x3_planes.h
--- /dev/null
+++ b/pixelpick_amd/csrc/x3_planes.h
@@ -0,0 +1,65 @@
+#pragma once
+#include "pp_common.h"
+
+namespace pp {
+
+__device__ __forceinline__ uint16_t f32_to_bf16_rne(float f)
+{
+    uint32_t u = __float_as_uint(f);
+    if ((u & 0x7F800000u) == 0x7F800000u) return (uint16_t)(u >> 16);
+    u += 0x7FFFu + ((u >> 16) & 1u);
+    return (uint16_t)(u >> 16);
+}
+__device__ __forceinline__ float bf16_to_f32(uint16_t h) { return __uint_as_float((uint32_t)h << 16); }
+
+__device__ __forceinline__ void x3_split1(float v, uint16_t& hi, uint16_t& mid, uint16_t& lo)
+{
+    hi = f32_to_bf16_rne(v);
+    const float r1 = v - bf16_to_f32(hi);
+    mid = f32_to_bf16_rne(r1);
+    const float r2 = r1 - bf16_to_f32(mid);
+    lo = f32_to_bf16_rne(r2);
+}
+
+__device__ __forceinline__ int64_t x3_plane_off(int64_t rows, int64_t r, int c) { return ((int64_t)(c >> 4) * (rows + 1) + r) * 16 + (c & 15); }
+
+struct X3PlanesOut {
+    uint16_t* planes;
+    int64_t plane;
+    int64_t rows;
+    int c0;
+    int store_f32;
+};
+
+__device__ __forceinline__ void x3_store_quad(const X3PlanesOut& o, int64_t off, uint2 h, uint2 m, uint2 l)
+{
+    *reinterpret_cast<uint2*>(o.planes + off) = h;
+    *reinterpret_cast<uint2*>(o.planes + o.plane + off) = m;
+    *reinterpret_cast<uint2*>(o.planes + 2 * o.plane + off) = l;
+}
+
+__device__ __forceinline__ void x3_store4(const X3PlanesOut& o, int64_t r, int c, int C, float4 v)
+{
+    uint16_t h[4], m[4], l[4];
+    x3_split1(v.x, h[0], m[0], l[0]);
+    x3_split1(v.y, h[1], m[1], l[1]);
+    x3_split1(v.z, h[2], m[2], l[2]);
+    x3_split1(v.w, h[3], m[3], l[3]);
+    const int cg = o.c0 + c;
+    x3_store_quad(o, x3_plane_off(o.rows, r, cg), make_uint2(h[0] | ((uint32_t)h[1] << 16), h[2] | ((uint32_t)h[3] << 16)),
+                  make_uint2(m[0] | ((uint32_t)m[1] << 16), m[2] | ((uint32_t)m[3] << 16)),
+                  make_uint2(l[0] | ((uint32_t)l[1] << 16), l[2] | ((uint32_t)l[3] << 16)));
+    if (c + 4 == C) {
+        const uint2 z = make_uint2(0u, 0u);
+        for (int cz = cg + 4; (cz & 15) != 0; cz += 4) x3_store_quad(o, x3_plane_off(o.rows, r, cz), z, z, z);
+    }
+}
+
+__device__ __forceinline__ void x3_store_zero_row(const X3PlanesOut& o, int C, int tid, int nthreads)
+{
+    const uint2 z = make_uint2(0u, 0u);
+    const int q1 = ((o.c0 + C + 15) & ~15) >> 2;
+    for (int q = (o.c0 >> 2) + tid; q < q1; q += nthreads) x3_store_quad(o, x3_plane_off(o.rows, o.rows, q * 4), z, z, z);
+}
+
+}
diff --git a/pixelpick_amd/engine.py b/pixelpick_amd/engine.py
--- a/pixelpick_amd/engine.py
+++ b/pixelpick_amd/engine.py
@@ -13,7 +13,7 @@
 
 
 class Var:
-    __slots__ = ("_t", "grad", "needs_grad", "_pending", "_lazy", "_bn_bwd_ctx", "_closed", "_grad_dst")
+    __slots__ = ("_t", "grad", "needs_grad", "_pending", "_lazy", "_bn_bwd_ctx", "_closed", "_grad_dst", "_x3p", "_dy_planes")
 
     def __init__(self, t: Optional[torch.Tensor], needs_grad: bool = True):
         self._t = t
@@ -24,6 +24,8 @@
         self._bn_bwd_ctx = None
         self._closed = False
         self._grad_dst = None
+        self._x3p = None
+        self._dy_planes = None
 
     @property
     def t(self) -> torch.Tensor:
@@ -422,6 +424,51 @@
     return planes
 
 
+def _producer_planes() -> bool:
+    return _X3_SHARE and _CONV_BN_FUSE_BWD and os.environ.get("PIXELPICK_X3_PRODUCER_PLANES", "1") != "0"
+
+
+def producer_planes_on(tape) -> bool:
+    return bool(tape.enabled and _producer_planes())
+
+
+class X3Planes:
+    __slots__ = ("t", "rows", "C", "Kp", "nbytes", "filled")
+
+    def __init__(self, rows: int, C: int, device):
+        self.rows, self.C, self.Kp = rows, C, -(-C // 16) * 16
+        self.nbytes = _wsbytes("pp_x3_planes_bytes", rows, C)
+        self.t = torch.empty(self.nbytes, dtype=torch.uint8, device=device)
+        self.filled = 0
+
+    def complete(self) -> bool:
+        return self.filled == self.C
+
+    def accepts(self, rows: int, C: int, c0: int) -> bool:
+        return rows == self.rows and C % 4 == 0 and c0 % 16 == 0 and 0 <= c0 and c0 + C <= self.C
+
+
+def _conv_deferred(B, H, W, Cin, Cout, kh, kw, stride, pad, dil, bias) -> bool:
+    return bool(_CONV_BN_STATS or _BN_ON_LOAD or (_CONV_BN_FUSE and bias is None and _conv_bn_fusable(B, H, W, Cin, Cout, kh, kw, stride, pad, dil)))
+
+
+def _conv_reads_x_planes(tape, w, B, H, W, Cin, Cout, kh, kw, stride, pad, dil) -> bool:
+    return bool(tape.enabled and w.requires_grad and _x3_planes(0, B, H, W, Cin, Cout, kh, kw, stride, pad, dil)
+                and _x3_planes(2, B, H, W, Cin, Cout, kh, kw, stride, pad, dil))
+
+
+def x3_input_planes(tape, shape, w: torch.Tensor, bias, stride=1, pad=0, dil=1, device=None) -> Optional[X3Planes]:
+    B, H, W, Cin = shape
+    kh, kw, wcin, Cout = w.shape
+    if not _producer_planes() or wcin != Cin or Cin % 4:
+        return None
+    if _conv_deferred(B, H, W, Cin, Cout, kh, kw, stride, pad, dil, bias):
+        return None
+    if not _conv_reads_x_planes(tape, w, B, H, W, Cin, Cout, kh, kw, stride, pad, dil):
+        return None
+    return X3Planes(B * H * W, Cin, device if device is not None else w.device)
+
+
 _BATCH_REDUCE = os.environ.get("PIXELPICK_BATCH_REDUCE", "0") != "0"
 _ARENA_BYTES = int(os.environ.get("PIXELPICK_REDUCE_ARENA_MB", "768")) << 20
 _FLUSH_BYTES = int(os.environ.get("PIXELPICK_REDUCE_FLUSH_MB", "768")) << 20
@@ -765,12 +812,13 @@
         out = Var(None, needs_grad=False)
         out._pending = ("conv", x, w, bias, stride, pad, dil)
         return out
-    if (tape.enabled and dst is None and (_CONV_BN_STATS or _BN_ON_LOAD or
-                                           (_CONV_BN_FUSE and bias is None and _conv_bn_fusable(B, H, W, Cin, Cout, kh, kw, stride, pad, dil)))):
+    if tape.enabled and dst is None and _conv_deferred(B, H, W, Cin, Cout, kh, kw, stride, pad, dil, bias):
         out = Var(None)
         out._pending = ("conv", x, w, bias, stride, pad, dil)
         if bwd_group is not None:
             out._grad_dst = bwd_group[0].slice(bwd_group[1])
+        else:
+            _want_dy_planes(out, x, w, bias, B, H, W, Cin, Cout, kh, kw, stride, pad, dil)
         tape.record(_conv2d_bwd, (x, w, bias, stride, pad, dil, None, bwd_group), out)
         return out
     _, _, _, _, ldx = _geom(x.t)
@@ -779,9 +827,14 @@
     _, _, _, _, ldy = _geom(y)
     ws, wsn = _conv_ws(False, x.t.device, B, H, W, Cin, Cout, kh, kw, stride, pad, dil)
     xp = None
-    if (tape.enabled and w.requires_grad and _x3_planes(0, B, H, W, Cin, Cout, kh, kw, stride, pad, dil)
-            and _x3_planes(2, B, H, W, Cin, Cout, kh, kw, stride, pad, dil)):
-        xp = _x3_split(x.t, ldx, B * H * W, Cin)
+    if _conv_reads_x_planes(tape, w, B, H, W, Cin, Cout, kh, kw, stride, pad, dil):
+        pl = x._x3p
+        if pl is not None and pl.complete() and pl.rows == B * H * W and pl.C == Cin:
+            xp = pl.t
+        else:
+            xp = _x3_split(x.t, ldx, B * H * W, Cin)
+    elif x._x3p is not None:
+        raise RuntimeError("conv2d: the input carries producer planes this convolution does not read (x3_input_planes was asked for another layer)")
     if xp is not None or (tape.enabled and w.requires_grad and _x3_planes(3, B, H, W, Cin, Cout, kh, kw, stride, pad, dil)):
         wp = _weight_planes(w, 1)
         _register_weight_planes(w, 1)
@@ -794,8 +847,17 @@
     out = Var(y)
     if bwd_group is not None and tape.enabled:
         out._grad_dst = bwd_group[0].slice(bwd_group[1])
+    elif tape.enabled:
+        _want_dy_planes(out, x, w, bias, B, H, W, Cin, Cout, kh, kw, stride, pad, dil)
     tape.record(_conv2d_bwd, (x, w, bias, stride, pad, dil, xp, bwd_group), out)
     return out
+
+
+def _want_dy_planes(out: Var, x: Var, w, bias, B, H, W, Cin, Cout, kh, kw, stride, pad, dil):
+    if (w.requires_grad and x.needs_grad and not (x._t is None and x._lazy is not None) and _producer_planes()
+            and _x3_planes(1, B, H, W, Cin, Cout, kh, kw, stride, pad, dil) and _x3_planes(2, B, H, W, Cin, Cout, kh, kw, stride, pad, dil)):
+        Ho, Wo = out_size(H, kh, stride, pad, dil), out_size(W, kw, stride, pad, dil)
+        out._dy_planes = (B * Ho * Wo, Cout, bias is None)
 
 
 def _conv2d_bwd(tape: Tape, dy: torch.Tensor, x: Var, w, bias, stride, pad, dil, xp=None, bwd_group=None):
@@ -810,7 +872,13 @@
     dyp = None
     if (w.requires_grad and x.needs_grad and lazy_in is None and _x3_planes(1, B, H, W, Cin, Cout, kh, kw, stride, pad, dil)
             and _x3_planes(2, B, H, W, Cin, Cout, kh, kw, stride, pad, dil)):
-        dyp = _x3_split(dy, lddy, B * Ho * Wo, Cout)
+        pl = getattr(dy, "_pp_planes", None)
+        if pl is not None and pl.complete() and pl.rows == B * Ho * Wo and pl.C == Cout:
+            dyp = pl.t
+        else:
+            dyp = _x3_split(dy, lddy, B * Ho * Wo, Cout)
+    if dyp is None and getattr(dy, "_pp_planes_only", False):
+        raise RuntimeError("_conv2d_bwd: the gradient exists as bf16x3 planes only, and this backward does not read planes")
     big = _BIG_WGRAD_MAIN and 2.0 * B * Ho * Wo * Cin * Cout * kh * kw >= _BIG_WGRAD_FLOP
 
     def _issue_wgrad():
@@ -1168,7 +1236,8 @@
 def batch_norm_act(tape: Tape, x: Var, gamma, beta, running_mean, running_var, training: bool, act: int = ACT_NONE,
                    residual: Optional[Var] = None, eps: float = 1e-5, momentum: float = 0.1,
                    dst: Optional[torch.Tensor] = None, dropout_p: float = 0.0, lazy_ok: bool = False, single_consumer: bool = False,
-                   consumers: int = 0) -> Var:
+                   consumers: int = 0, planes: Optional["X3Planes"] = None, planes_c0: int = 0, planes_only: bool = False,
+                   owns_input: bool = False) -> Var:
     if (lazy_ok and _BN_ON_LOAD and training and tape.enabled and x._pending is not None and residual is None and dropout_p == 0.0
             and dst is None and shape_of(x)[3] % 4 == 0 and 4 * math.prod(shape_of(x)) >= _BN_ON_LOAD_MIN_BYTES):
         out = _bn_on_load(tape, x, gamma, beta, running_mean, running_var, act, eps, momentum)
@@ -1214,14 +1283,30 @@
             _dropout_counter[0] += 1
             dseed = (_dropout_counter[0] * 0x9E3779B97F4A7C15) & 0xFFFFFFFFFFFFFFFF
             sd = _dropout_seed_dev[0]
-        rc = L.pp_bn_train_fwd_fused(x.t.data_ptr(), ldx, M, C, gamma.data_ptr(), beta.data_ptr(), eps, momentum,
-                                     running_mean.data_ptr() if running_mean is not None else None,
-                                     running_var.data_ptr() if running_var is not None else None,
-                                     mean.data_ptr(), invstd.data_ptr(), rptr, ldr, act, float(dropout_p), dseed,
-                                     sd.data_ptr() if sd is not None else None, y.data_ptr(), ldy,
-                                     ws.data_ptr(), ws.numel(), sync.data_ptr(), sync.numel(), _stream())
+        if planes is not None and not (tape.enabled and _producer_planes() and planes.accepts(M, C, planes_c0)):
+            planes = None
+        if planes is not None:
+            rc = L.pp_bn_train_fwd_fused_planes(x.t.data_ptr(), ldx, M, C, gamma.data_ptr(), beta.data_ptr(), eps, momentum,
+                                                running_mean.data_ptr() if running_mean is not None else None,
+                                                running_var.data_ptr() if running_var is not None else None,
+                                                mean.data_ptr(), invstd.data_ptr(), rptr, ldr, act, float(dropout_p), dseed,
+                                                sd.data_ptr() if sd is not None else None, y.data_ptr(), ldy,
+                                                ws.data_ptr(), ws.numel(), sync.data_ptr(), sync.numel(),
+                                                planes.t.data_ptr(), planes.nbytes, planes.Kp, planes_c0, 0 if planes_only else 1, _stream())
+            planes.filled += C
+        else:
+            rc = L.pp_bn_train_fwd_fused(x.t.data_ptr(), ldx, M, C, gamma.data_ptr(), beta.data_ptr(), eps, momentum,
+                                         running_mean.data_ptr() if running_mean is not None else None,
+                                         running_var.data_ptr() if running_var is not None else None,
+                                         mean.data_ptr(), invstd.data_ptr(), rptr, ldr, act, float(dropout_p), dseed,
+                                         sd.data_ptr() if sd is not None else None, y.data_ptr(), ldy,
+                                         ws.data_ptr(), ws.numel(), sync.data_ptr(), sync.numel(), _stream())
         _lib.check(rc, "pp_bn_train_fwd_fused")
         out = Var(y)
+        if planes is not None and planes.complete():
+            out._x3p = planes
+        if owns_input and x._dy_planes is not None:
+            x._dy_planes = x._dy_planes[:3] + (True,)
         tape.record(_bn_bwd, (x, gamma, beta, mean, invstd, act, residual, out, 1.0 / (1.0 - dropout_p)), out)
         ncons = consumers if consumers > 0 else (1 if (lazy_ok or single_consumer) else 0)
         if ncons and dropout_p == 0.0 and dst is None and (residual is None or act == ACT_NONE):
@@ -1281,7 +1366,27 @@
         sync, ws = _bn_exchange(dev)
         remask = (act != ACT_NONE and residual is None and gscale == 1.0) or lazy_out
         flags = getattr(dy, "_pp_rowflags", None) if _SPARSE_ROWS else None
-        if flags is not None and flags.numel() == M:
+        want = x._dy_planes if (gd is None and x.grad is None and _producer_planes()) else None
+        pl = None
+        if want is not None and want[0] == M and want[1] == C and C % 4 == 0:
+            pl = X3Planes(M, C, dev)
+            only = bool(len(want) > 3 and want[3] and want[2])
+            args = (pl.t.data_ptr(), pl.nbytes, pl.Kp, 0, 0 if only else 1, _stream())
+            if flags is not None and flags.numel() == M:
+                rc = L.pp_bn_bwd_fused_sparse_planes(x.t.data_ptr(), ldx, dy.data_ptr(), lddy, None if remask else out.t.data_ptr(), ldya, act, M, C,
+                                                     mean.data_ptr(), invstd.data_ptr(), gamma.data_ptr(), dgamma.data_ptr(), dbeta.data_ptr(),
+                                                     dx.data_ptr(), lddx, dres.data_ptr() if dres is not None else None, C, float(gscale),
+                                                     beta.data_ptr(), ws.data_ptr(), ws.numel(), sync.data_ptr(), sync.numel(), flags.data_ptr(), *args)
+                tape._keepalive.append(flags)
+            else:
+                rc = L.pp_bn_bwd_fused_planes(x.t.data_ptr(), ldx, dy.data_ptr(), lddy, None if remask else out.t.data_ptr(), ldya, act, M, C,
+                                              mean.data_ptr(), invstd.data_ptr(), gamma.data_ptr(), dgamma.data_ptr(), dbeta.data_ptr(),
+                                              dx.data_ptr(), lddx, dres.data_ptr() if dres is not None else None, C, float(gscale),
+                                              beta.data_ptr(), ws.data_ptr(), ws.numel(), sync.data_ptr(), sync.numel(), *args)
+            pl.filled = C
+            dx._pp_planes = pl
+            dx._pp_planes_only = only
+        elif flags is not None and flags.numel() == M:
             rc = L.pp_bn_bwd_fused_sparse(x.t.data_ptr(), ldx, dy.data_ptr(), lddy, None if remask else out.t.data_ptr(), ldya, act, M, C,
                                         mean.data_ptr(), invstd.data_ptr(), gamma.data_ptr(), dgamma.data_ptr(), dbeta.data_ptr(),
                                         dx.data_ptr(), lddx, dres.data_ptr() if dres is not None else None, C, float(gscale),
@@ -1342,7 +1447,7 @@
 
 
 def bilinear(tape: Tape, x: Var, size, align_corners: bool, scale_factor: float = 0.0, out_nchw: bool = False,
-             dst: Optional[torch.Tensor] = None) -> Var:
+             dst: Optional[torch.Tensor] = None, planes: Optional["X3Planes"] = None, planes_c0: int = 0, planes_only: bool = False) -> Var:
     B, H, W, C, ldx = _geom(x.t)
     Ho, Wo = int(size[0]), int(size[1])
     dev = x.t.device
@@ -1352,10 +1457,22 @@
     else:
         y = dst if dst is not None else torch.empty((B, Ho, Wo, C), dtype=torch.float32, device=dev)
         _, _, _, _, ldy = _geom(y)
-    rc = _lib.lib().pp_bilinear_fwd(x.t.data_ptr(), ldx, B, H, W, C, y.data_ptr(), ldy, Ho, Wo, int(align_corners),
-                                    float(scale_factor), float(scale_factor), int(out_nchw), _stream())
+    if planes is not None and not (tape.enabled and _producer_planes() and not out_nchw and planes.accepts(B * Ho * Wo, C, planes_c0)):
+        if planes_only:
+            raise RuntimeError("bilinear: planes_only asked for operand planes this call cannot write")
+        planes = None
+    if planes is not None:
+        rc = _lib.lib().pp_bilinear_fwd_planes(x.t.data_ptr(), ldx, B, H, W, C, y.data_ptr(), ldy, Ho, Wo, int(align_corners),
+                                               float(scale_factor), float(scale_factor), planes.t.data_ptr(), planes.nbytes, planes.Kp,
+                                               planes_c0, 0 if planes_only else 1, _stream())
+        planes.filled += C
+    else:
+        rc = _lib.lib().pp_bilinear_fwd(x.t.data_ptr(), ldx, B, H, W, C, y.data_ptr(), ldy, Ho, Wo, int(align_corners),
+                                        float(scale_factor), float(scale_factor), int(out_nchw), _stream())
     _lib.check(rc, "pp_bilinear_fwd")
     out = Var(y)
+    if planes is not None and planes.complete():
+        out._x3p = planes
     tape.record(_bilinear_bwd, (x, (Ho, Wo), align_corners, scale_factor, out_nchw), out)
     return out
 
@@ -1568,7 +1685,7 @@
     _acc(x, dx)
 
 
-def concat_alias(tape: Tape, buf: torch.Tensor, parts: Sequence[Var]) -> Var:
+def concat_alias(tape: Tape, buf: torch.Tensor, parts: Sequence[Var], planes: Optional["X3Planes"] = None) -> Var:
     off = 0
     for p in parts:
         c = p.t.shape[3]
@@ -1576,6 +1693,8 @@
         off += c
     assert off == buf.shape[3]
     out = Var(buf)
+    if planes is not None and planes.complete() and planes.C == buf.shape[3]:
+        out._x3p = planes
     tape.record(_concat_bwd, (tuple(parts),), out)
     return out
 
diff --git a/pixelpick_amd/networks/backbones/resnet_backbone.py b/pixelpick_amd/networks/backbones/resnet_backbone.py
--- a/pixelpick_amd/networks/backbones/resnet_backbone.py
+++ b/pixelpick_amd/networks/backbones/resnet_backbone.py
@@ -6,7 +6,7 @@
 import torch.nn as nn
 
 from ... import engine as E
-from ..layers import BatchNorm2d, Conv2d, ReLU
+from ..layers import BatchNorm2d, Conv2d, ReLU, bn_act_into_conv
 
 
 class Bottleneck(nn.Module):
@@ -25,8 +25,8 @@
         self.stride = stride
 
     def run(self, tape, x):
-        out = self.bn1.run(tape, self.conv1.run(tape, x), E.ACT_RELU)
-        out = self.bn2.run(tape, self.conv2.run(tape, out), E.ACT_RELU)
+        out = bn_act_into_conv(tape, self.bn1, self.conv1.run(tape, x), E.ACT_RELU, self.conv2)
+        out = bn_act_into_conv(tape, self.bn2, self.conv2.run(tape, out), E.ACT_RELU, self.conv3)
         residual = x
         if self.downsample is not None:
             residual = self.downsample[1].run(tape, self.downsample[0].run(tape, x))
diff --git a/pixelpick_amd/networks/decoders.py b/pixelpick_amd/networks/decoders.py
--- a/pixelpick_amd/networks/decoders.py
+++ b/pixelpick_amd/networks/decoders.py
@@ -109,7 +109,10 @@
 
     def run(self, tape, x):
         s = self.segment_head
-        h = s[1].run(tape, s[0].run(tape, x), E.ACT_RELU, dropout=s[3])
-        emb = s[5].run(tape, s[4].run(tape, h), E.ACT_RELU, dropout=s[7])
+        own = {"owns_input": True} if E.producer_planes_on(tape) else {}
+        c1 = s[0].run(tape, x)
+        pl = E.x3_input_planes(tape, E.shape_of(c1), s[4].weight, s[4].bias, s[4].stride, s[4].padding, s[4].dilation)
+        h = s[1].run(tape, c1, E.ACT_RELU, dropout=s[3], **(dict(own, planes=pl) if pl is not None else own))
+        emb = s[5].run(tape, s[4].run(tape, h), E.ACT_RELU, dropout=s[7], **own)
         pred = self.classifier.run(tape, emb)
         return {"emb": emb, "pred": pred}
diff --git a/pixelpick_amd/networks/deeplab.py b/pixelpick_amd/networks/deeplab.py
--- a/pixelpick_amd/networks/deeplab.py
+++ b/pixelpick_amd/networks/deeplab.py
@@ -102,10 +102,17 @@
         a = self.aspp.run(tape, high)
         _, Hl, Wl, _ = low.t.shape
         cat_buf = torch.empty((B, Hl, Wl, 304), dtype=torch.float32, device=inputs.device)
-        up = E.bilinear(tape, a, (Hl, Wl), True, 0.0, dst=cat_buf[..., 0:256])
         llc = self.low_level_conv
-        low_ = llc[1].run(tape, llc[0].run(tape, low), E.ACT_RELU, dst=cat_buf[..., 256:304])
-        cat = E.concat_alias(tape, cat_buf, [up, low_])
+        head = self.seg_head.segment_head[0]
+        pl = E.x3_input_planes(tape, (B, Hl, Wl, 304), head.weight, head.bias, head.stride, head.padding, head.dilation)
+        if pl is not None:
+            low_ = llc[1].run(tape, llc[0].run(tape, low), E.ACT_RELU, dst=cat_buf[..., 256:304], planes=pl, planes_c0=256, planes_only=True)
+            only = pl.filled == 48
+            up = E.bilinear(tape, a, (Hl, Wl), True, 0.0, dst=cat_buf[..., 0:256], planes=pl if only else None, planes_only=only)
+        else:
+            up = E.bilinear(tape, a, (Hl, Wl), True, 0.0, dst=cat_buf[..., 0:256])
+            low_ = llc[1].run(tape, llc[0].run(tape, low), E.ACT_RELU, dst=cat_buf[..., 256:304])
+        cat = E.concat_alias(tape, cat_buf, [up, low_], planes=pl)
         outs = self.seg_head.run(tape, cat)
         if not upsample:
             return outs["pred"], outs["emb"]
diff --git a/pixelpick_amd/networks/layers.py b/pixelpick_amd/networks/layers.py
--- a/pixelpick_amd/networks/layers.py
+++ b/pixelpick_amd/networks/layers.py
@@ -113,7 +113,8 @@
             self._nbt_pending = 0
         super()._save_to_state_dict(destination, prefix, keep_vars)
 
-    def run(self, tape, x, act=E.ACT_NONE, residual=None, dst=None, dropout=None, lazy_ok=False, single_consumer=False, consumers=0):
+    def run(self, tape, x, act=E.ACT_NONE, residual=None, dst=None, dropout=None, lazy_ok=False, single_consumer=False, consumers=0,
+            planes=None, planes_c0=0, planes_only=False, owns_input=False):
         training = self.training
         if training:
             B, H, W, _ = E.shape_of(x)
@@ -123,13 +124,23 @@
         drop_p = dropout.p if (dropout is not None and dropout.training and dropout.p > 0.0) else 0.0
         return E.batch_norm_act(tape, x, self.weight, self.bias, self.running_mean, self.running_var, training, act,
                                 residual, self.eps, self.momentum, dst=dst, dropout_p=drop_p, lazy_ok=lazy_ok,
-                                single_consumer=single_consumer, consumers=consumers)
+                                single_consumer=single_consumer, consumers=consumers, planes=planes, planes_c0=planes_c0,
+                                planes_only=planes_only, owns_input=owns_input)
 
     def forward(self, x):
         raise RuntimeError("pixelpick_amd layers execute through run(tape, x)")
 
     def extra_repr(self):
         return f"{self.num_features}, eps={self.eps}, momentum={self.momentum}"
+
+
+def bn_act_into_conv(tape, bn: BatchNorm2d, x, act, conv: Conv2d):
+    if not E.producer_planes_on(tape):
+        return bn.run(tape, x, act)
+    pl = E.x3_input_planes(tape, E.shape_of(x), conv.weight, conv.bias, conv.stride, conv.padding, conv.dilation)
+    if pl is None:
+        return bn.run(tape, x, act, owns_input=True)
+    return bn.run(tape, x, act, owns_input=True, planes=pl, planes_only=True)
 
 
 class _Placeholder(nn.Module):
```

Measured after the change: 760.4 images/s (median of 6 runs). 1.5% higher.
